# p-mc-grath/DMMFODS

Measured on AMD Instinct MI355X. Metric: training images/sec at 1280x1920 RGB+LiDAR, higher is better.
Workload: dtype f16; 1 GPU; C2 d121 early-fusion 6ch b4 1280x1920; key=c2, per_gpu_batch=4, global_batch=4, height=1280, width=1920, storage_dtype=fp16, accumulate=fp32, parallelism=dp1, weights=random-init (reference init, seed 123)

## Files before the change

dmmfods_amd/_lib.py:

```python
import ctypes as C
import os

_HERE = os.path.dirname(os.path.abspath(__file__))
LIB_PATH = os.environ.get("DMM_LIB_PATH") or os.path.join(_HERE, "libdmmfods_hip.so")

DMM_F32, DMM_F16, DMM_BF16 = 0, 1, 2
LOSS_BCE, LOSS_FOCAL = 0, 1
T_CONV, T_CONVT, T_BN_WEIGHT, T_BN_BIAS, T_BN_MEAN, T_BN_VAR, T_BN_TRACKED = range(7)
ERR_INVALID, ERR_SHAPE, ERR_HIP, ERR_STATE, ERR_NO_DEVICE = -1, -2, -3, -4, -5


class ModelDesc(C.Structure):
    _fields_ = [
        ("growth_rate", C.c_int32), ("num_blocks", C.c_int32), ("block_config", C.c_int32 * 8),
        ("num_init_features", C.c_int32), ("bn_size", C.c_int32), ("num_classes", C.c_int32),
        ("concat_before_block_num", C.c_int32), ("stream_1_in_channels", C.c_int32),
        ("stream_2_in_channels", C.c_int32), ("batch", C.c_int32), ("height", C.c_int32), ("width", C.c_int32),
        ("dtype", C.c_int32), ("loss_scale", C.c_float), ("bn_momentum", C.c_float), ("bn_eps", C.c_float),
        ("iou_threshold", C.c_float), ("use_mfma", C.c_int32),
    ]


class ConvDesc(C.Structure):
    _fields_ = [(n, C.c_int32) for n in (
        "dtype", "use_mfma", "B", "H", "W", "Cin", "Cout", "R", "S", "stride", "pad", "transposed", "mode", "bn_relu")]


class GuardState(C.Structure):
    _fields_ = [("scale", C.c_float), ("grad_scale", C.c_float), ("sumsq", C.c_double), ("grad_norm", C.c_float),
                ("found_inf", C.c_int32), ("applied_steps", C.c_int64), ("skipped_steps", C.c_int64),
                ("growth_tracker", C.c_int32), ("step_size", C.c_float), ("bc2_sqrt", C.c_float), ("clip_coef", C.c_float),
                ("reserved", C.c_int32 * 2)]


assert C.sizeof(GuardState) == 64

ADAM_MAX_CLASSES = 16


class AdamSegment(C.Structure):
    _fields_ = [("begin", C.c_int64), ("count", C.c_int64), ("cls", C.c_int32)]


class AdamClass(C.Structure):
    _fields_ = [("lr", C.c_float), ("beta1", C.c_float), ("beta2", C.c_float), ("eps", C.c_float), ("weight_decay", C.c_float),
                ("decoupled", C.c_int32), ("t0", C.c_int64)]


assert C.sizeof(AdamSegment) == 24 and C.sizeof(AdamClass) == 32


class DmmError(RuntimeError):
    pass


_lib = None


def lib():
    global _lib
    if _lib is not None:
        return _lib
    if not os.path.exists(LIB_PATH):
        raise ImportError(
            f"{LIB_PATH} is missing: build it with `python -c 'import __graft_entry__ as g; g.build()'` "
            "(or `make -C dmmfods_amd/csrc`).  dmmfods_amd has no CPU fallback.")
    import torch
    tl = os.path.join(os.path.dirname(torch.__file__), "lib", "libamdhip64.so")
    if os.path.exists(tl):
        C.CDLL(tl, mode=C.RTLD_GLOBAL)
    L = C.CDLL(LIB_PATH)
    vp, i32, i64, f32, sz = C.c_void_p, C.c_int32, C.c_int64, C.c_float, C.c_size_t
    L.dmm_last_error.restype = C.c_char_p
    L.dmm_version.restype = C.c_int
    L.dmm_last_impl.restype = C.c_int
    L.dmm_impl_name.restype = C.c_char_p
    L.dmm_impl_name.argtypes = [C.c_int]
    L.dmm_impl_mask.restype = C.c_uint
    L.dmm_impl_mask.argtypes = [C.c_int]
    L.dmm_set_option.restype = C.c_int
    L.dmm_set_option.argtypes = [C.c_char_p, C.c_int]
    L.dmm_plan_create.argtypes = [C.POINTER(ModelDesc), C.POINTER(vp)]
    L.dmm_plan_destroy.argtypes = [vp]
    L.dmm_plan_destroy.restype = C.c_int
    L.dmm_plan_num_tensors.argtypes = [vp]
    L.dmm_plan_tensor_info.argtypes = [vp, C.c_int, C.POINTER(C.c_char_p), C.POINTER(i32), C.POINTER(i32),
                                       C.POINTER(i64 * 4), C.POINTER(i64)]
    L.dmm_plan_num_params.argtypes = [vp]
    L.dmm_plan_num_params.restype = i64
    L.dmm_plan_num_buffer_elems.argtypes = [vp]
    L.dmm_plan_num_buffer_elems.restype = i64
    L.dmm_plan_workspace_bytes.argtypes = [vp]
    L.dmm_plan_workspace_bytes.restype = sz
    L.dmm_plan_forward_flops.argtypes = [vp]
    L.dmm_plan_forward_flops.restype = C.c_double
    L.dmm_plan_bind.argtypes = [vp, vp, sz, vp, vp, vp]
    L.dmm_plan_forward.argtypes = [vp, vp, vp, vp, C.c_int, vp]
    L.dmm_plan_loss_backward.argtypes = [vp, vp, vp, vp, vp]
    L.dmm_plan_backward.argtypes = [vp, vp, vp]
    L.dmm_plan_loss_metrics.argtypes = [vp, vp, vp, vp, vp]
    L.dmm_plan_set_loss.argtypes = [vp, C.c_int, vp, vp, C.c_int]
    L.dmm_loss_forward.argtypes = [C.c_int, C.c_int, vp, vp, vp, vp, vp, vp, C.c_int, C.c_int, C.c_int, C.c_int, vp]
    L.dmm_plan_num_grad_buckets.argtypes = [vp]
    L.dmm_plan_num_graph_replays.argtypes = [vp, C.c_int]
    L.dmm_plan_num_graph_replays.restype = C.c_longlong
    L.dmm_plan_grad_bucket.argtypes = [vp, C.c_int, C.POINTER(i64), C.POINTER(i64)]
    L.dmm_plan_grad_bucket_wait.argtypes = [vp, C.c_int, vp]
    L.dmm_plan_profile_begin.argtypes = [vp, C.c_int]
    L.dmm_plan_profile_filter.restype = C.c_int
    L.dmm_plan_profile_filter.argtypes = [vp, C.c_char_p]
    L.dmm_plan_profile_num_ops.argtypes = [vp, C.c_int]
    L.dmm_plan_profile_op.argtypes = [vp, C.c_int, C.c_int, C.POINTER(C.c_char_p), C.POINTER(C.c_double), C.POINTER(C.c_double)]
    L.dmm_plan_profile_collect.argtypes = [vp, C.c_int, C.POINTER(C.c_double), C.c_int, C.POINTER(C.c_int)]
    L.dmm_adam_step.argtypes = [vp, vp, vp, vp, i64, f32, f32, f32, f32, f32, i64, f32, vp]
    L.dmm_grad_guard_scratch_bytes.argtypes = [i64]
    L.dmm_grad_guard_scratch_bytes.restype = sz
    L.dmm_guard_state_init.argtypes = [vp, f32, i64, i32, vp]
    L.dmm_adam_step_guarded.argtypes = [vp, vp, vp, vp, i64, f32, f32, f32, f32, f32, f32, f32, f32, i32, vp, vp, vp]
    L.dmm_adam_step_guarded_ranges.argtypes = [vp, vp, vp, vp, C.POINTER(i64), C.POINTER(i64), C.POINTER(i64), C.c_int,
                                               f32, f32, f32, f32, f32, f32, f32, f32, i32, vp, vp, vp]
    L.dmm_plan_set_encoder_frozen.argtypes = [vp, C.c_int]
    L.dmm_adam_table_bytes.argtypes = [C.c_int, i64]
    L.dmm_adam_table_bytes.restype = sz
    L.dmm_adam_table_init.argtypes = [vp, C.POINTER(AdamSegment), C.c_int, i64, C.c_int, vp]
    L.dmm_adam_step_segmented.argtypes = [vp, vp, vp, vp, i64, vp, C.c_int, C.POINTER(AdamClass), C.c_int, i64, f32, vp]
    L.dmm_adam_step_guarded_segmented.argtypes = [vp, vp, vp, vp, i64, vp, C.c_int, C.POINTER(AdamClass), C.c_int, f32, f32, f32, i32,
                                                  vp, vp, vp]
    L.dmm_grad_sumsq.argtypes = [vp, i64, i64, C.c_int, vp, vp]
    L.dmm_plan_set_dynamic_loss_scale.argtypes = [vp, vp]
    L.dmm_plan_set_grad_accumulate.argtypes = [vp, C.c_int]
    L.dmm_conv_scratch_bytes.argtypes = [C.POINTER(ConvDesc)]
    L.dmm_conv_scratch_bytes.restype = sz
    L.dmm_conv_forward.argtypes = [C.POINTER(ConvDesc), vp, vp, vp, vp, vp, vp, vp, vp]
    L.dmm_conv_wgrad.argtypes = [C.POINTER(ConvDesc), vp, vp, vp, vp, vp, vp, vp]
    L.dmm_conv_dgrad.argtypes = [C.POINTER(ConvDesc), vp, vp, vp, vp, vp, vp, vp, vp, vp]
    L.dmm_conv_wgrad_ex.argtypes = [C.POINTER(ConvDesc), vp, vp, vp, vp, vp, vp, vp, C.c_int, vp, vp, vp]
    L.dmm_conv_dgrad_ex.argtypes = [C.POINTER(ConvDesc), vp, vp, vp, vp, vp, vp, vp, vp, vp, C.c_int, vp, vp, vp]
    L.dmm_conv1x1_backward_fused.argtypes = [C.POINTER(ConvDesc), vp, vp, vp, vp, vp, vp, vp, vp, vp, C.c_int, vp, vp, vp, vp]
    L.dmm_conv5_wgrad_stats.argtypes = [C.POINTER(ConvDesc), vp, vp, vp, vp, vp, vp, vp, vp, vp]
    _lib = L
    return L


EXPORTS = [
    "dmm_last_error", "dmm_version", "dmm_set_option", "dmm_plan_create", "dmm_plan_destroy", "dmm_plan_num_tensors",
    "dmm_plan_tensor_info", "dmm_plan_num_params", "dmm_plan_num_buffer_elems", "dmm_plan_workspace_bytes",
    "dmm_plan_forward_flops", "dmm_plan_bind", "dmm_plan_forward", "dmm_plan_loss_backward", "dmm_plan_backward",
    "dmm_plan_loss_metrics", "dmm_plan_num_graph_replays", "dmm_plan_set_loss", "dmm_loss_forward", "dmm_plan_num_grad_buckets", "dmm_plan_grad_bucket",
    "dmm_plan_grad_bucket_wait", "dmm_plan_profile_begin", "dmm_plan_profile_filter", "dmm_plan_profile_num_ops", "dmm_plan_profile_op",
    "dmm_plan_profile_collect", "dmm_adam_step", "dmm_conv_scratch_bytes", "dmm_conv_forward", "dmm_conv_wgrad",
    "dmm_conv_dgrad", "dmm_conv_wgrad_ex", "dmm_conv_dgrad_ex", "dmm_conv1x1_backward_fused", "dmm_conv5_wgrad_stats", "dmm_last_impl", "dmm_impl_name", "dmm_impl_mask",
    "dmm_grad_guard_scratch_bytes", "dmm_guard_state_init", "dmm_adam_step_guarded", "dmm_grad_sumsq", "dmm_plan_set_dynamic_loss_scale",
    "dmm_plan_set_grad_accumulate", "dmm_plan_set_encoder_frozen", "dmm_adam_step_guarded_ranges",
    "dmm_adam_table_bytes", "dmm_adam_table_init", "dmm_adam_step_segmented", "dmm_adam_step_guarded_segmented",
]


def check(rc):
    if rc == 0:
        return
    msg = lib().dmm_last_error().decode(errors="replace")
    if rc == ERR_SHAPE:
        raise ValueError(msg)
    if rc == ERR_INVALID and "fusion" in msg:
        raise AttributeError(msg)
    if rc == ERR_INVALID:
        raise ValueError(msg)
    raise DmmError(f"dmm status {rc}: {msg}")


def last_impl():
    L = lib()
    return L.dmm_impl_name(L.dmm_last_impl()).decode()


def impls_since_reset(reset=True):
    L = lib()
    m = L.dmm_impl_mask(1 if reset else 0)
    return {L.dmm_impl_name(i).decode() for i in range(32) if (m >> i) & 1}


def stream_ptr():
    import torch
    return C.c_void_p(torch.cuda.current_stream().cuda_stream)
```

dmmfods_amd/csrc/bw1.hip:

```cpp
#include <algorithm>
#include <cstdio>
#include <cstdlib>
#include <type_traits>

#include "common.h"
#include "dispatch.h"
#include "gather.h"
#include "isa.h"
#include "pointwise.h"

namespace dmm {

#ifndef B1_DBG
#define B1_DBG 0
#endif
#ifndef B1_LATE_PREFETCH
#define B1_LATE_PREFETCH 0
#endif
#ifndef B1_RAW_BAR
#define B1_RAW_BAR 0
#endif
#ifndef B1_NT
#define B1_NT 0
#endif
#ifndef B1_GOLD_EARLY
#define B1_GOLD_EARLY 0
#endif
constexpr int B1_TM = 64;
constexpr int B1_NB = 128;
constexpr int B1_CT = 128;
constexpr int B1_IMG = B1_TM * 256;
constexpr int B1_W = 4 * B1_CT * 64;
constexpr int B1_STAGE = B1_TM * B1_CT * 4;
static_assert(B1_STAGE == 2 * B1_IMG, "staging aliases the operand images exactly");
constexpr int B1_LDS = 2 * B1_IMG + B1_W + 2 * B1_CT * 8 + 6 * B1_CT * 4;

__device__ __forceinline__ int b1_swz(int row, int slot) { return ((((slot >> 2) ^ (row & 3)) << 2) | ((slot & 3) ^ ((row >> 2) & 3))); }

template <typename T, int PQ, bool ACC_, bool PART>
__global__ __launch_bounds__(NTHREADS, 2) void bw1_kernel(const Bw1Args g) {
  constexpr bool ACC = ACC_ && !(B1_DBG & 32);
  constexpr bool UNC = std::is_same<T, f16>::value;
  static_assert(sizeof(T) == 2, "16-bit storage");
  typedef typename TT<T>::vec V;
  constexpr int SLOT = 8;
  constexpr int NL = B1_TM * 16 / NTHREADS;
  const ConvArgs& a = g.c;
  const Seg& sg = a.seg[0];

  extern __shared__ __attribute__((aligned(16))) unsigned char smem[];
  unsigned char* Ai = smem;
  unsigned char* Gi = smem + B1_IMG;
  unsigned char* Wi = smem + 2 * B1_IMG;
  double* red = (double*)(smem + 2 * B1_IMG + B1_W);
  float* kc = (float*)(smem + 2 * B1_IMG + B1_W + 2 * B1_CT * 8);

  const int tid = threadIdx.x, lane = tid & 63, wave = tid >> 6;
  const int r = lane & 31, h = lane >> 5;
  const int xcd = blockIdx.x & 7, q = blockIdx.x >> 3;
  const int ct = g.xcd_group ? q % g.nct : (int)(blockIdx.x % g.nct);
  const int split = g.xcd_group ? (q / g.nct) * 8 + xcd : (int)(blockIdx.x / g.nct);
  const int c0 = ct * B1_CT;
  const int t_beg = split * g.tiles_per_wg, t_end = min(g.ntiles, t_beg + g.tiles_per_wg);
  if (t_beg >= t_end) return;

  const int cs = tid & 15, p0 = tid >> 4;
  const int cx = c0 + cs * SLOT;
  const bool cvalid = cx < a.N;
  if (tid < B1_CT) {
    const int c = c0 + tid;
    const bool v = c < a.N;
    kc[tid] = v ? a.bscale[c] : 0.f; kc[B1_CT + tid] = v ? a.bshift[c] : 0.f;
    kc[2 * B1_CT + tid] = v ? a.bmean[c] : 0.f; kc[3 * B1_CT + tid] = v ? a.binvstd[c] : 0.f;
    kc[4 * B1_CT + tid] = PQ == 2 ? sg.q[tid] : 0.f; kc[5 * B1_CT + tid] = PQ == 2 ? sg.r[tid] : 0.f;
  }
  const unsigned char* xbase = (const unsigned char*)a.bx;
  const unsigned char* gbase = (const unsigned char*)sg.src;
  const unsigned char* ybase = (const unsigned char*)sg.src2;
  unsigned char* obase = (unsigned char*)a.out;
  const unsigned xcol = (unsigned)(cvalid ? cx : 0) * 2u, gcol = (unsigned)(cs * SLOT) * 2u;
  const unsigned xpitch = (unsigned)a.ldbx * 2u, gpitch = (unsigned)sg.ld * 2u, ypitch = (unsigned)sg.ld2 * 2u, opitch = (unsigned)a.ldo * 2u;
  const int lds0 = p0 * 256 + (b1_swz(p0, cs) << 4);

  {
    const T* wp = (const T*)a.wpack;
#pragma unroll
    for (int j = 0; j < B1_W / 16 / NTHREADS; ++j) {
      const int piece = tid + NTHREADS * j;
      const int chunk = piece >> 9, rowc = (piece >> 2) & 127, slot = piece & 3;
      const int c = c0 + rowc;
      V v;
#pragma unroll
      for (int e = 0; e < SLOT; ++e) v[e] = (T)0;
      if (c < a.Npad) v = *(const V*)(wp + ((size_t)chunk * a.Npad + c) * 32 + slot * SLOT);
      *(V*)(Wi + chunk * (B1_CT * 64) + rowc * 64 + ((slot ^ ((rowc >> 2) & 3)) << 4)) = v;
    }
  }
  if (tid < 2 * B1_CT) red[tid] = 0.0;
  __syncthreads();

  V rx[NL], rg[NL], ry[PQ == 2 ? NL : 1];
  unsigned okp = 0;
  auto issue = [&](int tile) {
    okp = 0;
#pragma unroll
    for (int i = 0; i < NL; ++i) {
      const int m = tile * B1_TM + p0 + 16 * i;
      if (m < a.M) okp |= 1u << i;
      const unsigned mm = (B1_DBG & 16) ? 0u : (unsigned)min(m, a.M - 1);
      if (B1_NT & 1) rx[i] = __builtin_nontemporal_load((const V*)(xbase + (size_t)(mm * xpitch + xcol)));
      else rx[i] = *(const V*)(xbase + (size_t)(mm * xpitch + xcol));
      rg[i] = *(const V*)(gbase + (size_t)(mm * gpitch + gcol));
      if constexpr (PQ == 2) ry[i] = *(const V*)(ybase + (size_t)(mm * ypitch + gcol));
    }
  };

  const int dpx = 32 * (wave & 1) + r;
  const int dgoff = dpx * 256;
  const int dcb = 64 * (wave >> 1);
  const int bsw = (r >> 2) & 3;
  const int tg = lane >> 4, ti = lane & 15, tq = ti >> 2, tp = ti & 3;
  const int arow = 8 * (tg >> 1) + tq;
  auto tr_off = [&](int px, int colbyte) { return px * 256 + ((b1_swz(px, colbyte >> 4) << 4) | (colbyte & 15)); };
  const int acolb = (32 * wave + 16 * (tg & 1) + 4 * tp) * 2;
  const int aoff1 = tr_off(arow, acolb);
  int goff1[4];
#pragma unroll
  for (int j = 0; j < 4; ++j) goff1[j] = tr_off(arow, (32 * j + 16 * (tg & 1) + 4 * tp) * 2);
  auto second = [](int off) { return (off ^ 16) + 4 * 256; };

  f32x16 accw[4];
#pragma unroll
  for (int j = 0; j < 4; ++j)
#pragma unroll
    for (int i = 0; i < 16; ++i) accw[j][i] = 0.f;

  issue(t_beg);
  for (int tile = t_beg; tile < t_end; ++tile) {
    V xraw[NL], gold[ACC ? NL : 1];
    const bool full = (tile + 1) * B1_TM <= a.M;
    const unsigned okt = okp;
    auto stage = [&](auto full_tag) {
      constexpr bool FULL = decltype(full_tag)::value;
      V z;
#pragma unroll
      for (int e = 0; e < SLOT; ++e) z[e] = (T)0;
      {
        SlotK<SLOT> kx;
        kx.k0 = load_fv<SLOT>(kc + cs * SLOT); kx.k1 = load_fv<SLOT>(kc + B1_CT + cs * SLOT); kx.k2 = 0.f; kx.k3 = 0.f;
#pragma unroll
        for (int i = 0; i < NL; ++i) {
          xraw[i] = rx[i];
          const bool v = FULL || ((okt >> i) & 1) != 0;
          const V av_ = bn_relu_slot(rx[i], kx);
          *(V*)(Ai + lds0 + 4096 * i) = v ? av_ : z;
        }
      }
      {
        SlotK<SLOT> kg;
        kg.k0 = 0.f; kg.k1 = 0.f; kg.k2 = 0.f; kg.k3 = 0.f;
        if (PQ == 2) { kg.k0 = load_fv<SLOT>(kc + 4 * B1_CT + cs * SLOT); kg.k1 = load_fv<SLOT>(kc + 5 * B1_CT + cs * SLOT); }
#pragma unroll
        for (int i = 0; i < NL; ++i) {
          const bool v = FULL || ((okt >> i) & 1) != 0;
          V gv = rg[i];
          if constexpr (PQ == 2) gv = eff_grad_slot(rg[i], ry[i], kg);
          *(V*)(Gi + lds0 + 4096 * i) = v ? gv : z;
        }
      }
    };
    if (UNC && full) stage(std::true_type()); else stage(std::false_type());
    __syncthreads();
#if !B1_LATE_PREFETCH
    if (tile + 1 < t_end) issue(tile + 1);
#endif
#if B1_GOLD_EARLY
    if constexpr (ACC) {
#pragma unroll
      for (int i = 0; i < NL; ++i) {
        const unsigned mm = (unsigned)min(tile * B1_TM + p0 + 16 * i, a.M - 1);
        gold[i] = *(const V*)(obase + (size_t)(mm * opitch + xcol));
      }
    }
#endif

    f32x16 accd[2];
#pragma unroll
    for (int t = 0; t < 2; ++t)
#pragma unroll
      for (int i = 0; i < 16; ++i) accd[t][i] = 0.f;
    if (!(B1_DBG & 4))
#pragma unroll
    for (int ch = 0; ch < 4; ++ch)
#pragma unroll
      for (int s = 0; s < 2; ++s) {
        const int slot = ch * 4 + 2 * s + h;
        const V av = *(const V*)(Gi + dgoff + (b1_swz(dpx, slot) << 4));
#pragma unroll
        for (int t = 0; t < 2; ++t) {
          const V bv = *(const V*)(Wi + ch * (B1_CT * 64) + (dcb + 32 * t + r) * 64 + (((2 * s + h) ^ bsw) << 4));
          accd[t] = mma16(av, bv, accd[t]);
        }
      }
    if (!(B1_DBG & 2))
#pragma unroll
    for (int ms = 0; ms < B1_TM / 16; ++ms) {
      const V af = frag16<T>(lds_tr16(Ai + aoff1 + ms * 4096), lds_tr16(Ai + second(aoff1) + ms * 4096));
#pragma unroll
      for (int j = 0; j < 4; ++j) {
        const V gf = frag16<T>(lds_tr16(Gi + goff1[j] + ms * 4096), lds_tr16(Gi + second(goff1[j]) + ms * 4096));
        accw[j] = mma16(gf, af, accw[j]);
      }
    }
#if !B1_GOLD_EARLY
    if constexpr (ACC) {
#pragma unroll
      for (int i = 0; i < NL; ++i) {
        const unsigned mm = (unsigned)min(tile * B1_TM + p0 + 16 * i, a.M - 1);
        if (B1_NT & 1) gold[i] = __builtin_nontemporal_load((const V*)(obase + (size_t)(mm * opitch + xcol)));
        else gold[i] = *(const V*)(obase + (size_t)(mm * opitch + xcol));
      }
    }
#endif
#if B1_LATE_PREFETCH
    if (tile + 1 < t_end) issue(tile + 1);
#endif
#if B1_RAW_BAR
    lds_barrier();
#else
    __syncthreads();
#endif
    if (B1_DBG & 8) {
      float sa = 0.f;
#pragma unroll
      for (int t = 0; t < 2; ++t)
#pragma unroll
        for (int i = 0; i < 16; ++i) sa += accd[t][i];
      if (sa == 1.2345e33f) obase[0] = 1;
    } else {
    float* Cs = (float*)smem;
#pragma unroll
    for (int t = 0; t < 2; ++t)
#pragma unroll
      for (int i = 0; i < 16; ++i) {
        const int row = 32 * (wave & 1) + (i & 3) + 8 * (i >> 2) + 4 * h;
        Cs[row * B1_CT + ((dcb + 32 * t + r) ^ (h << 5))] = accd[t][i];
      }
#if B1_RAW_BAR
    lds_barrier();
#else
    __syncthreads();
#endif
    float s1[SLOT], s2[SLOT];
#pragma unroll
    for (int e = 0; e < SLOT; ++e) { s1[e] = 0.f; s2[e] = 0.f; }
    auto finish = [&](auto full_tag) {
      constexpr bool FULL = decltype(full_tag)::value;
      float sc[SLOT], sh[SLOT], mu[UNC ? 1 : SLOT], is[UNC ? 1 : SLOT];
      load_f32s<SLOT>(kc + cs * SLOT, sc); load_f32s<SLOT>(kc + B1_CT + cs * SLOT, sh);
      if constexpr (!UNC) { load_f32s<SLOT>(kc + 2 * B1_CT + cs * SLOT, mu); load_f32s<SLOT>(kc + 3 * B1_CT + cs * SLOT, is); }
#pragma unroll
      for (int i = 0; i < NL; ++i) {
        if (!FULL && !((okt >> i) & 1)) continue;
        const int p = p0 + 16 * i;
        float av[SLOT];
#pragma unroll
        for (int e = 0; e < SLOT; e += 4) {
          const f32x4 t4 = *(const f32x4*)(Cs + p * B1_CT + ((cs * SLOT + e) ^ (((p >> 2) & 1) << 5)));
          av[e] = t4[0]; av[e + 1] = t4[1]; av[e + 2] = t4[2]; av[e + 3] = t4[3];
        }
        const unsigned m = (unsigned)(tile * B1_TM + p);
        if constexpr (UNC) {
          const V ov = bnbwd_slot<ACC>(av, xraw[i], gold[ACC ? i : 0], sc, sh, s1, s2);
          if (B1_NT & 2) __builtin_nontemporal_store(ov, (V*)(obase + (size_t)(m * opitch + xcol)));
          else if (!(B1_DBG & 64) || av[0] == 1.2345e33f) *(V*)(obase + (size_t)(m * opitch + xcol)) = ov;
        } else {
          float xf[SLOT], gf[SLOT];
          vec_to_f32<T>(xraw[i], xf);
          if constexpr (ACC) vec_to_f32<T>(gold[i], gf);
#pragma unroll
          for (int e = 0; e < SLOT; ++e) {
            const float dz = (fmaf(xf[e], sc[e], sh[e]) > 0.f) ? av[e] : 0.f;
            s1[e] += dz;
            s2[e] = fmaf(dz, (xf[e] - mu[e]) * is[e], s2[e]);
            gf[e] = (ACC ? gf[e] : 0.f) + sc[e] * dz;
          }
          if (!(B1_DBG & 64) || gf[0] == 1.2345e33f) *(V*)(obase + (size_t)(m * opitch + xcol)) = f32_to_vec<T>(gf);
        }
      }
    };
    if (cvalid) { if (UNC && full) finish(std::true_type()); else finish(std::false_type()); }
    fold_to_lds<16, SLOT, B1_CT>(s1, s2, red, cs, cvalid, lane);
    }
#if B1_RAW_BAR
    lds_barrier();
#else
    __syncthreads();
#endif
  }

  if (tid < B1_CT && c0 + tid < a.N) {
    const size_t rep = (size_t)(blockIdx.x & (STAT_REPS - 1)) * a.stat_stride;
    const double S1 = red[fold_slot<16, SLOT>(0, tid)];
    double S2 = red[fold_slot<16, SLOT>(1, tid)];
    if constexpr (UNC) S2 = (S2 - (double)kc[2 * B1_CT + tid] * S1) * (double)kc[3 * B1_CT + tid];
    atomic_add_f64(a.red1 + rep + c0 + tid, S1);
    atomic_add_f64(a.red2 + rep + c0 + tid, S2);
  }
  const int c = c0 + 32 * wave + r;
  if constexpr (PART) {
    float* slot = g.part + ((size_t)split * g.nct + ct) * B1_SLOT_FLOATS + (size_t)wave * (B1_NB * 32);
#pragma unroll
    for (int j = 0; j < 4; ++j)
#pragma unroll
      for (int i = 0; i < 16; ++i) {
        const int n = 32 * j + (i & 3) + 8 * (i >> 2) + 4 * h;
        slot[n * 32 + r] = accw[j][i];
      }
  } else if (!(B1_DBG & 1) && c < g.wC) {
    const size_t chunk = (size_t)(c0 / 32 + wave);
#pragma unroll
    for (int j = 0; j < 4; ++j)
#pragma unroll
      for (int i = 0; i < 16; ++i) {
        const int n = 32 * j + (i & 3) + 8 * (i >> 2) + 4 * h;
        atomic_add_f32(g.dpack + (chunk * g.dNpad + n) * 32 + r, accw[j][i]);
      }
  }
  if (B1_DBG & 1) {
    float s = 0.f;
#pragma unroll
    for (int j = 0; j < 4; ++j)
#pragma unroll
      for (int i = 0; i < 16; ++i) s += accw[j][i];
    if (s == 1.2345e33f) g.dpack[0] = s;
  }
}

template <typename T, int PQ, bool ACC, bool PART>
static hipError_t launch_bw1_t(const Bw1Args& g, int nwg, hipStream_t st) {
  return launch_lds<bw1_kernel<T, PQ, ACC, PART>>(B1_LDS, nwg, NTHREADS, B1_LDS, st, g);
}

bool bw1_eligible(const WgradArgs& w, const ConvArgs& d, int dtype, unsigned deny) {
  if (((deny >> IMPL_BW1) & 1u) || dtype == DT_F32 || w.nseg != 1 || d.nseg != 1 || d.pool2) return false;
  const Seg& wx = w.seg[0];
  const Seg& wg = w.dy;
  const Seg& dg = d.seg[0];
  if (wx.mode != G_PLAIN || wx.istride != 1 || wx.ntaps != 1 || wx.taps[0] != 0 || wx.scale == nullptr || wx.C % 32) return false;
  if (wg.mode != G_PLAIN || wg.istride != 1 || wg.ntaps != 1 || wg.taps[0] != 0 || wg.scale != nullptr || wg.C != B1_NB) return false;
  if (dg.mode != G_PLAIN || dg.istride != 1 || dg.ntaps != 1 || dg.taps[0] != 0 || dg.scale != nullptr || dg.C != B1_NB || dg.Cpad != B1_NB) return false;
  if (dg.src != wg.src || dg.ld != wg.ld || dg.q != wg.q || dg.src2 != wg.src2) return false;
  if (w.N != B1_NB || w.Npad != B1_NB || w.M != d.M || d.N != wx.C || d.Npad % 32) return false;
  if (d.bx != wx.src || d.ldbx != wx.ld || d.bscale != wx.scale || d.bshift != wx.shift) return false;
  if (d.out == nullptr || d.ostride != 1 || d.Hout != d.Ho || d.Wout != d.Wo || wx.Hs != d.Ho || wx.Ws != d.Wo) return false;
  const double span = 2.0 * (double)d.M;
  if (span * d.ldbx >= 4294967296.0 || span * d.ldo >= 4294967296.0 || span * dg.ld >= 4294967296.0 || span * dg.ld2 >= 4294967296.0) return false;
  return true;
}

Bw1Geom bw1_geometry(const ConvArgs& a) {
  Bw1Geom q;
  q.nct = (a.N + B1_CT - 1) / B1_CT;
  q.ntiles = (a.M + B1_TM - 1) / B1_TM;
  constexpr int cus = DESIGN_CUS;
  static const int per_cu = lab_int("DMM_BW1_PER_CU", 2);
  int nsplit = std::max(1, (per_cu * cus + q.nct - 1) / q.nct);
  nsplit = std::min(nsplit, std::max(1, q.ntiles / 4));
  q.tiles_per_wg = (q.ntiles + nsplit - 1) / nsplit;
  q.nsplit = (q.ntiles + q.tiles_per_wg - 1) / q.tiles_per_wg;
  q.xcd_group = (q.nct > 1 && q.nsplit >= 32 && q.tiles_per_wg >= 8) ? 1 : 0;
  q.nwg = q.xcd_group ? ((q.nsplit + 7) / 8) * 8 * q.nct : q.nsplit * q.nct;
  return q;
}

static bool g_bw1_part = !lab_flag("DMM_NO_BW1_PART");

static bool bw1_uses_part(const Bw1Args& g, const Bw1Geom& q) {
  return g_bw1_part && g.part != nullptr && q.nsplit * q.nct <= g.part_slots && q.nsplit > 1;
}

hipError_t launch_bw1(const Bw1Args& g0, int dtype, hipStream_t st) {
  Bw1Args g = g0;
  const ConvArgs& a = g.c;
  if (a.M <= 0) return hipSuccess;
  const Bw1Geom q = bw1_geometry(a);
  note_impl(IMPL_BW1);
  g.nct = q.nct; g.ntiles = q.ntiles; g.tiles_per_wg = q.tiles_per_wg; g.xcd_group = q.xcd_group; g.nsplit = q.nsplit;
  const int nwg = q.nwg;
  const int pq = a.seg[0].q ? 2 : 0;
  const bool acc = a.accumulate != 0;
  const bool part = bw1_uses_part(g, q);
#define B1_GO(T) \
  (part ? (pq ? (acc ? launch_bw1_t<T, 2, true, true>(g, nwg, st) : launch_bw1_t<T, 2, false, true>(g, nwg, st))     \
              : (acc ? launch_bw1_t<T, 0, true, true>(g, nwg, st) : launch_bw1_t<T, 0, false, true>(g, nwg, st)))    \
        : (pq ? (acc ? launch_bw1_t<T, 2, true, false>(g, nwg, st) : launch_bw1_t<T, 2, false, false>(g, nwg, st))   \
              : (acc ? launch_bw1_t<T, 0, true, false>(g, nwg, st) : launch_bw1_t<T, 0, false, false>(g, nwg, st))))
  if (dtype == DT_F16) return B1_GO(f16);
  return B1_GO(bf16);
#undef B1_GO
}

__global__ __launch_bounds__(256) void bw1_reduce_kernel(const float* __restrict__ part, float* __restrict__ dpack, int nct, int nsplit, int nfloats) {
  const int e = (blockIdx.x * 256 + threadIdx.x) * 4;
  if (e >= nct * B1_SLOT_FLOATS) return;
  f32x4 s = {0.f, 0.f, 0.f, 0.f};
  const float* p = part + e;
  const size_t pitch = (size_t)nct * B1_SLOT_FLOATS;
  int k = 0;
  for (; k + 16 <= nsplit; k += 16) {
    f32x4 v[16];
#pragma unroll
    for (int u = 0; u < 16; ++u) v[u] = __builtin_nontemporal_load((const f32x4*)(p + (size_t)(k + u) * pitch));
#pragma unroll
    for (int u = 0; u < 16; u += 4) s += (v[u] + v[u + 1]) + (v[u + 2] + v[u + 3]);
  }
  for (; k + 4 <= nsplit; k += 4) {
    const f32x4 v0 = *(const f32x4*)(p + (size_t)k * pitch), v1 = *(const f32x4*)(p + (size_t)(k + 1) * pitch);
    const f32x4 v2 = *(const f32x4*)(p + (size_t)(k + 2) * pitch), v3 = *(const f32x4*)(p + (size_t)(k + 3) * pitch);
    s += (v0 + v1) + (v2 + v3);
  }
  for (; k < nsplit; ++k) s += *(const f32x4*)(p + (size_t)k * pitch);
  if (e < nfloats) *(f32x4*)(dpack + e) = s;
}

hipError_t launch_bw1_reduce(const Bw1Args& g, hipStream_t st) {
  const ConvArgs& a = g.c;
  if (a.M <= 0) return hipSuccess;
  const Bw1Geom q = bw1_geometry(a);
  if (!bw1_uses_part(g, q)) return hipSuccess;
  const int nfloats = ((g.wC + 31) / 32) * g.dNpad * 32;
  const int nthreads = q.nct * B1_SLOT_FLOATS / 4;
  hipLaunchKernelGGL(bw1_reduce_kernel, dim3((nthreads + 255) / 256), dim3(256), 0, st, g.part, g.dpack, q.nct, q.nsplit, nfloats);
  return hipGetLastError();
}

}
```

dmmfods_amd/csrc/capi.cpp:

```cpp
#include <algorithm>
#include <atomic>
#include <cmath>
#include <cstdio>
#include <cstdlib>
#include <cstring>
#include <stdexcept>
#include <chrono>
#include <mutex>
#include <string>
#include <utility>
#include <vector>
#include <unistd.h>

#include "dispatch.h"
#include "plan.h"

using namespace dmm;

void plan_build_tables(dmm_plan* p);
void plan_bind(dmm_plan* p, void* ws);
void plan_size(dmm_plan* p);

static thread_local std::string g_err;
static int fail(int code, const std::string& msg) {
  g_err = msg;
  return code;
}
#define HIPCHK(expr)                                                                                   \
  do {                                                                                                 \
    hipError_t e__ = (expr);                                                                           \
    if (e__ != hipSuccess) return fail(DMM_ERR_HIP, std::string(#expr) + ": " + hipGetErrorString(e__)); \
  } while (0)

static bool g_overlap_wgrad = getenv("DMM_NO_OVERLAP") == nullptr;
static int g_graph = getenv("DMM_GRAPH") ? std::max(1, atoi(getenv("DMM_GRAPH"))) : 0;
static unsigned long long g_option_epoch = 1;
static int g_bucket_mb = getenv("DMM_GRAD_BUCKET_MB") ? atoi(getenv("DMM_GRAD_BUCKET_MB")) : 25;
static std::atomic<unsigned> g_family_off{lab_family_off()};
static unsigned plan_deny(const dmm_plan* p) { return (p->sw.no_hf ? 1u << IMPL_HF : 0u) | g_family_off; }

namespace {
struct DevicePool {
  std::mutex mu;
  hipStream_t side = nullptr, pack = nullptr, capture = nullptr;
  std::vector<hipEvent_t> free_plain, free_timing;
  long events_made = 0;
};
constexpr int MAX_DEVICES = 64;
DevicePool* g_pools[MAX_DEVICES] = {};
std::mutex g_pools_mu;

DevicePool* pool_of(int device) {
  if (device < 0 || device >= MAX_DEVICES) return nullptr;
  std::lock_guard<std::mutex> l(g_pools_mu);
  if (g_pools[device] == nullptr) g_pools[device] = new DevicePool();
  return g_pools[device];
}
hipError_t pool_streams(DevicePool* dp, bool want_capture) {
  std::lock_guard<std::mutex> l(dp->mu);
  if (dp->side == nullptr) {
    int lo = 0, hi = 0;
    hipError_t e = hipDeviceGetStreamPriorityRange(&lo, &hi);
    if (e != hipSuccess) return e;
    hipStream_t s = nullptr, k = nullptr;
    if ((e = hipStreamCreateWithPriority(&s, hipStreamNonBlocking, lo)) != hipSuccess) return e;
    if ((e = hipStreamCreateWithPriority(&k, hipStreamNonBlocking, lo)) != hipSuccess) return e;
    dp->side = s; dp->pack = k;
  }
  if (want_capture && dp->capture == nullptr) {
    hipStream_t c = nullptr;
    const hipError_t e = hipStreamCreateWithFlags(&c, hipStreamNonBlocking);
    if (e != hipSuccess) return e;
    dp->capture = c;
  }
  return hipSuccess;
}
hipEvent_t pool_event(DevicePool* dp, bool timing) {
  std::lock_guard<std::mutex> l(dp->mu);
  auto& fl = timing ? dp->free_timing : dp->free_plain;
  if (!fl.empty()) { hipEvent_t e = fl.back(); fl.pop_back(); return e; }
  hipEvent_t e = nullptr;
  const hipError_t rc = timing ? hipEventCreate(&e) : hipEventCreateWithFlags(&e, hipEventDisableTiming);
  if (rc != hipSuccess) return nullptr;
  ++dp->events_made;
  return e;
}
void pool_return(DevicePool* dp, std::vector<void*>& evs, bool timing) {
  std::lock_guard<std::mutex> l(dp->mu);
  auto& fl = timing ? dp->free_timing : dp->free_plain;
  for (void* e : evs) if (e) fl.push_back((hipEvent_t)e);
  evs.clear();
}
void trace_destroy(const char* what) {
  static const bool on = getenv("DMM_TRACE_DESTROY") != nullptr;
  if (!on) return;
  char buf[160];
  const int n = snprintf(buf, sizeof(buf), "[dmm] destroy: %s\n", what);
  if (n > 0) { ssize_t w = write(2, buf, (size_t)std::min<int>(n, (int)sizeof(buf) - 1)); (void)w; }
}
}

extern "C" {

const char* dmm_last_error(void) { return g_err.c_str(); }
int dmm_version(void) { return 101; }

static const char* const kImplNames[IMPL_COUNT] = {"auto", "generic", "thin", "conv3", "cvp", "halo", "wg3", "wg5", "wgp", "pig", "bw1", "hf", "cf", "wgpw", "cvw"};
static const struct { const char* option; int family; } kFamilyOptions[] = {
    {"thin_logits", IMPL_THIN}, {"conv3", IMPL_CONV3}, {"wg3", IMPL_WG3}, {"wgp", IMPL_WGP},
    {"wg5", IMPL_WG5},          {"cvp", IMPL_CVP},     {"bw1", IMPL_BW1}, {"pig", IMPL_PIG},
};

int dmm_set_option(const char* name, int value) {
  if (!name) return fail(DMM_ERR_INVALID, "null argument");
  ++g_option_epoch;
  if (std::string(name) == "overlap_wgrad") { g_overlap_wgrad = value != 0; return DMM_OK; }
  if (std::string(name) == "graph") { g_graph = value; return DMM_OK; }
  for (const auto& o : kFamilyOptions)
    if (std::string(name) == o.option) {
      if (value != 0) g_family_off &= ~(1u << o.family);
      else g_family_off |= 1u << o.family;
      return DMM_OK;
    }
  if (std::string(name) == "grad_bucket_mb") {
    if (value < 0) return fail(DMM_ERR_INVALID, "grad_bucket_mb must be >= 0");
    g_bucket_mb = value;
    return DMM_OK;
  }
  return fail(DMM_ERR_INVALID, std::string("unknown option ") + name);
}

int dmm_plan_create(const dmm_model_desc* desc, dmm_plan** out) {
  if (!desc || !out) return fail(DMM_ERR_INVALID, "null argument");
  if (desc->num_blocks < 2 || desc->num_blocks > 8) return fail(DMM_ERR_INVALID, "num_blocks must be in [2, 8]");
  if (desc->dtype != DMM_F32 && desc->dtype != DMM_F16 && desc->dtype != DMM_BF16)
    return fail(DMM_ERR_INVALID, "dtype must be DMM_F32, DMM_F16 or DMM_BF16");
  if (desc->dtype == DMM_BF16 && !desc->use_mfma) return fail(DMM_ERR_INVALID, "DMM_BF16 has no scalar check kernels: use_mfma must be 1");
  if (desc->batch < 1) return fail(DMM_ERR_INVALID, "batch must be >= 1");
  if (!(desc->loss_scale > 0)) return fail(DMM_ERR_INVALID, "loss_scale must be > 0");
  dmm_plan* p = new dmm_plan();
  p->desc = *desc;
  p->sw = PlanSwitches::from_environment();
  p->bucket_bytes = (size_t)g_bucket_mb << 20;
  p->deny = plan_deny(p);
  try {
    plan_build_tables(p);
  } catch (const std::domain_error& e) {
    delete p;
    return fail(DMM_ERR_SHAPE, e.what());
  } catch (const std::exception& e) {
    delete p;
    return fail(DMM_ERR_INVALID, e.what());
  }
  *out = p;
  return DMM_OK;
}

int dmm_plan_destroy(dmm_plan* plan) {
  if (!plan) return DMM_OK;
  trace_destroy("begin");
  std::string first_err;
  auto note = [&](hipError_t e, const char* what) {
    if (e != hipSuccess && first_err.empty()) first_err = std::string(what) + ": " + hipGetErrorString(e);
  };
  DevicePool* dp = plan->device >= 0 ? pool_of(plan->device) : nullptr;
  if (dp != nullptr) {
    int cur = -1;
    const bool switched = hipGetDevice(&cur) == hipSuccess && cur != plan->device && hipSetDevice(plan->device) == hipSuccess;
    if (plan->used_side) {
      trace_destroy("synchronise the side stream");
      note(hipStreamSynchronize(dp->side), "hipStreamSynchronize(side stream)");
      trace_destroy("synchronise the pack stream");
      note(hipStreamSynchronize(dp->pack), "hipStreamSynchronize(pack stream)");
    }
    if (plan->used_capture && dp->capture) {
      trace_destroy("synchronise the capture stream");
      note(hipStreamSynchronize(dp->capture), "hipStreamSynchronize(capture stream)");
    }
    trace_destroy("graphs");
    for (auto& gc : plan->graphs) {
      for (auto& e : gc.entries) note(hipGraphExecDestroy((hipGraphExec_t)e.exec), "hipGraphExecDestroy");
      gc.entries.clear();
    }
    trace_destroy("events back to the pool");
    pool_return(dp, plan->fork_events, false);
    pool_return(dp, plan->join_events, false);
    pool_return(dp, plan->bucket_events, false);
    for (auto& which : plan->prof_events)
      for (auto& pass : which) pool_return(dp, pass, true);
    if (switched) (void)hipSetDevice(cur);
  }
  trace_destroy("delete");
  delete plan;
  trace_destroy("done");
  return first_err.empty() ? DMM_OK : fail(DMM_ERR_HIP, "dmm_plan_destroy: " + first_err);
}

int dmm_plan_num_tensors(const dmm_plan* plan) { return plan ? (int)plan->tensors.size() : 0; }

int dmm_plan_tensor_info(const dmm_plan* plan, int index, const char** name, int32_t* kind, int32_t* ndim, int64_t shape[4],
                         int64_t* arena_offset) {
  if (!plan || index < 0 || index >= (int)plan->tensors.size()) return fail(DMM_ERR_INVALID, "tensor index out of range");
  const TensorInfo& t = plan->tensors[index];
  if (name) *name = t.name.c_str();
  if (kind) *kind = t.kind;
  if (ndim) *ndim = t.ndim;
  if (shape) for (int i = 0; i < 4; ++i) shape[i] = t.shape[i];
  if (arena_offset) *arena_offset = t.off;
  return DMM_OK;
}

int64_t dmm_plan_num_params(const dmm_plan* plan) { return plan ? plan->nparams : 0; }
int64_t dmm_plan_num_buffer_elems(const dmm_plan* plan) { return plan ? plan->nbuf : 0; }
size_t dmm_plan_workspace_bytes(const dmm_plan* plan) { return plan ? plan->zero_bytes + plan->zero_bwd_bytes + plan->main_bytes : 0; }
double dmm_plan_forward_flops(const dmm_plan* plan) { return plan ? plan->fwd_flops : 0; }

int dmm_plan_bind(dmm_plan* plan, void* workspace, size_t workspace_bytes, float* params, float* grads, float* buffers) {
  if (!plan || !workspace || !params || !grads || !buffers) return fail(DMM_ERR_INVALID, "null argument");
  if (workspace_bytes < dmm_plan_workspace_bytes(plan)) return fail(DMM_ERR_INVALID, "workspace too small");
  if ((uintptr_t)workspace % 256) return fail(DMM_ERR_INVALID, "workspace must be 256-byte aligned");
  int ndev = 0;
  if (hipGetDeviceCount(&ndev) != hipSuccess || ndev == 0) return fail(DMM_ERR_NO_DEVICE, "no HIP device");
  int dev = 0;
  HIPCHK(hipGetDevice(&dev));
  if (plan->device >= 0 && plan->device != dev) return fail(DMM_ERR_STATE, "the plan is bound to another device");
  if (dev >= MAX_DEVICES) return fail(DMM_ERR_INVALID, "device index out of range");
  plan->device = dev;
  plan->params = params;
  plan->grads = grads;
  plan->buffers = buffers;
  plan->graphs[0].epoch = plan->graphs[1].epoch = 0;
  plan->bound = false;
  plan->deny = plan_deny(plan);
  try {
    plan_bind(plan, workspace);
  } catch (const dmm::plan_sizing_error& e) {
    return fail(DMM_ERR_STATE, e.what());
  } catch (const std::exception& e) {
    return fail(DMM_ERR_INVALID, e.what());
  }
  HIPCHK(hipDeviceSynchronize());
  plan->bound = true;
  return DMM_OK;
}

static std::string family_check(const Op& o, unsigned ran) {
  if ((o.kind == OP_IGEMM ? o.c.M : o.w.M) <= 0) return std::string();
  const bool recorded_ran = (ran >> o.impl) & 1u;
  const bool generic_ran = (ran >> IMPL_GENERIC) & 1u;
  const bool wgp_remainder = o.kind == OP_WGRAD && o.impl == IMPL_WGP && o.w.nseg == 2 && o.w.nphase == 0;
  if (recorded_ran && (o.impl == IMPL_GENERIC || !generic_ran || wgp_remainder)) return std::string();
  std::string names;
  for (int f = 1; f < IMPL_COUNT; ++f)
    if ((ran >> f) & 1u) names += (names.empty() ? "" : "+") + std::string(dmm_impl_name(f));
  return std::string("launch '") + o.label + "': the plan recorded family " + dmm_impl_name(o.impl) + ", " + (names.empty() ? "none" : names) + " ran";
}

static int run_ops(dmm_plan* p, std::vector<Op>& ops, hipStream_t st, int prof_which = -1, size_t begin = 0, size_t end = 0, bool capturing = false) {
  if (end == 0 || end > ops.size()) end = ops.size();
  const size_t ev_offset = 0;
  const int dt = p->desc.dtype;
  const bool mfma = p->desc.use_mfma != 0;
  std::vector<void*>* evs = nullptr;
  if (prof_which >= 0 && p->prof_max_passes > 0 && p->prof_pass[prof_which] < p->prof_max_passes) {
    auto& sets = p->prof_events[prof_which];
    const int pass = p->prof_pass[prof_which]++;
    if ((int)sets.size() <= pass) sets.resize(pass + 1);
    evs = &sets[pass];
    const size_t need = 2 * (ops.size() + ev_offset);
    DevicePool* pdp = pool_of(p->device);
    while (evs->size() < need) {
      hipEvent_t e = pdp ? pool_event(pdp, true) : nullptr;
      if (e == nullptr) return fail(DMM_ERR_HIP, "hipEventCreate failed");
      evs->push_back((void*)e);
    }
  }
  const bool accumulate = p->grad_accumulate;
  const std::string& filt = p->prof_filter;
  auto selected = [&](const Op& o) { return evs != nullptr && (filt.empty() || strncmp(o.label, filt.c_str(), filt.size()) == 0); };
  const bool overlap = g_overlap_wgrad && !capturing && (evs == nullptr || !filt.empty());
  constexpr int nside = 1;
  size_t nfork = 0;
  bool forked = false;
  DevicePool* dp = pool_of(p->device);
  hipStream_t side_st = nullptr, pack_st = nullptr;
  if (overlap) {
    if (dp == nullptr || pool_streams(dp, false) != hipSuccess) return fail(DMM_ERR_HIP, "side stream");
    side_st = dp->side; pack_st = dp->pack;
    while ((int)p->join_events.size() < nside + 1) {
      hipEvent_t je = pool_event(dp, false);
      if (je == nullptr) return fail(DMM_ERR_HIP, "hipEventCreate failed");
      p->join_events.push_back((void*)je);
    }
    p->used_side = true;
  }
  bool pack_pending = false;
  auto join_pack = [&]() {
    if (pack_pending) {
      hipStreamWaitEvent(st, (hipEvent_t)p->join_events[nside], 0);
      pack_pending = false;
    }
  };
  auto join_side = [&]() {
    if (forked) {
      for (int k = 0; k < nside; ++k) {
        hipEventRecord((hipEvent_t)p->join_events[k], side_st);
        hipStreamWaitEvent(st, (hipEvent_t)p->join_events[k], 0);
      }
      forked = false;
    }
  };
  auto join = [&]() { join_side(); join_pack(); };
  static const bool host_prof = lab_flag("DMM_HOST_PROF");
  static double hp_launch[32] = {0}, hp_fork[32] = {0};
  static long hp_n[32] = {0}, hp_lists = 0;
  auto now = [] { return std::chrono::duration<double, std::micro>(std::chrono::steady_clock::now().time_since_epoch()).count(); };
  for (size_t i = begin; i < end; ++i) {
    Op& o = ops[i];
    hipError_t e = hipSuccess;
    const double hp_t0 = host_prof ? now() : 0.0;
    double hp_t1 = hp_t0;
    hipStream_t lst = st;
    if (overlap && o.leaf == 3 && forked) {
      lst = side_st;
    } else if (overlap && !o.chain && (o.kind == OP_WGRAD || o.leaf)) {
      if (nfork >= p->fork_events.size()) {
        hipEvent_t fe = pool_event(dp, false);
        if (fe == nullptr) { join(); return fail(DMM_ERR_HIP, "hipEventCreate failed"); }
        p->fork_events.push_back((void*)fe);
      }
      lst = o.leaf == 2 ? pack_st : side_st;
      hipEvent_t fe = (hipEvent_t)p->fork_events[nfork++];
      hipEventRecord(fe, st);
      hipStreamWaitEvent(lst, fe, 0);
      if (o.leaf == 2) pack_pending = true; else forked = true;
      if (host_prof) hp_t1 = now();
    }
    const bool sel = selected(o);
    if (sel) hipEventRecord((hipEvent_t)(*evs)[2 * (ev_offset + i)], lst);
    const bool fam_check = (o.kind == OP_IGEMM || o.kind == OP_WGRAD) && o.impl != IMPL_AUTO;
    const unsigned mask_before = g_impl_mask;
    if (fam_check) g_impl_mask = 0;
    switch (o.kind) {
      case OP_MEMSET: if (!(accumulate && o.ms.p == (void*)p->grads)) e = hipMemsetAsync(o.ms.p, 0, o.ms.bytes, lst); break;
      case OP_COPY: e = hipMemcpyAsync(o.cp.dst, o.cp.src, o.cp.bytes, hipMemcpyDeviceToDevice, lst); break;
      case OP_CONVERT: e = launch_convert_input(o.cv, dt, lst); break;
      case OP_IGEMM: e = launch_igemm(o.c, dt, o.epi, mfma, lst, o.impl); break;
      case OP_WGRAD: e = launch_wgrad(o.w, dt, mfma, lst, o.impl); break;
      case OP_BW1: e = launch_bw1(o.b1, dt, lst); break;
      case OP_BW1RED: e = launch_bw1_reduce(o.b1, lst); break;
      case OP_RAWFIN: e = launch_wg5_rawfin(o.rf, lst); break;
      case OP_FIN64: e = launch_wg5_fin64(o.f64, lst); break;
      case OP_JOIN: if (o.epi == 1) join_pack(); else join_side(); break;
      case OP_BNFIN: e = launch_bn_finalize(o.bf, lst); break;
      case OP_BNBWD:
        if (accumulate) { BnBwdFinalizeArgs bb = o.bb; bb.accumulate = 1; e = launch_bn_bwd_finalize(bb, lst); }
        else e = launch_bn_bwd_finalize(o.bb, lst);
        break;
      case OP_POOL: e = launch_maxpool_fwd(o.mp, dt, lst); break;
      case OP_POOLBWD: e = launch_maxpool_bwd(o.mpb, dt, lst); break;
      case OP_BCE: e = launch_bce_metrics(o.bce, dt, lst); break;
      case OP_PACK: e = launch_pack(o.pk.descs, o.pk.prefix, o.pk.ndesc, o.pk.total_rows, dt, lst, o.pk.tdescs, o.pk.tiles, o.pk.nt1, o.pk.nt9); break;
      case OP_APPLYCORR: e = launch_apply_corr(o.ac, dt, lst); break;
      case OP_UNPACK: e = launch_unpack(o.pk.descs, o.pk.prefix, o.pk.ndesc, o.pk.total_rows, dt, o.pk.grad_scale, lst, o.pk.tdescs, o.pk.tiles, o.pk.nt1, o.pk.nt9, accumulate); break;
      default: join(); return fail(DMM_ERR_STATE, "unknown op");
    }
    if (host_prof && o.kind < 32) { const double t2 = now(); hp_fork[o.kind] += hp_t1 - hp_t0; hp_launch[o.kind] += t2 - hp_t1; hp_n[o.kind]++; }
    if (e != hipSuccess) join();
    if (e != hipSuccess && fam_check) g_impl_mask |= mask_before;
    if (e != hipSuccess) return fail(DMM_ERR_HIP, "op " + std::to_string(i) + " kind " + std::to_string(o.kind) + ": " + hipGetErrorString(e));
    if (fam_check) {
      const unsigned ran = g_impl_mask;
      g_impl_mask = mask_before | ran;
      const std::string why = family_check(o, ran);
      if (!why.empty()) { join(); return fail(DMM_ERR_STATE, why); }
    }
    if (sel) hipEventRecord((hipEvent_t)(*evs)[2 * (ev_offset + i) + 1], lst);
    if (pack_pending && o.leaf == 2) hipEventRecord((hipEvent_t)p->join_events[nside], lst);
    if (o.signal >= 0 && !capturing) {
      while ((int)p->bucket_events.size() <= o.signal) {
        hipEvent_t be = dp ? pool_event(dp, false) : nullptr;
        if (be == nullptr) { join(); return fail(DMM_ERR_HIP, "hipEventCreate failed"); }
        p->bucket_events.push_back((void*)be);
      }
      hipEventRecord((hipEvent_t)p->bucket_events[o.signal], lst);
    }
  }
  join();
  if (host_prof && ++hp_lists == 40) {
    double tot = 0;
    for (int k = 0; k < 32; ++k) tot += hp_launch[k] + hp_fork[k];
    fprintf(stderr, "[host] 40 lists: %.2f ms of enqueue calls per list pair\n", tot / 20 / 1e3);
    for (int k = 0; k < 32; ++k)
      if (hp_n[k]) fprintf(stderr, "[host] op kind %2d: %6ld calls per pair, launch %.2f us each, fork events %.2f us each\n", k, hp_n[k] / 20,
                           hp_launch[k] / hp_n[k], hp_fork[k] / hp_n[k]);
  }
  return DMM_OK;
}

static int record_bucket_events(dmm_plan* p, const std::vector<Op>& ops, hipStream_t st) {
  for (const Op& o : ops) {
    if (o.signal < 0) continue;
    while ((int)p->bucket_events.size() <= o.signal) {
      DevicePool* dp = pool_of(p->device);
      hipEvent_t be = dp ? pool_event(dp, false) : nullptr;
      if (be == nullptr) return fail(DMM_ERR_HIP, "hipEventCreate failed");
      p->bucket_events.push_back((void*)be);
    }
    HIPCHK(hipEventRecord((hipEvent_t)p->bucket_events[o.signal], st));
  }
  return DMM_OK;
}

static int launch_list(dmm_plan* p, int which, std::vector<Op>& ops, size_t seg_begin, size_t seg_end, hipStream_t st) {
  dmm_plan::GraphCache& gc = p->graphs[which];
  const bool profiling = p->prof_max_passes > 0 && p->prof_pass[which] < p->prof_max_passes;
  if (gc.epoch != g_option_epoch) {
    for (auto& e : gc.entries) hipGraphExecDestroy((hipGraphExec_t)e.exec);
    gc.entries.clear();
    gc.nseen = 0;
    gc.epoch = g_option_epoch;
  }
  const bool want = g_graph && !(g_graph == 2 && which == 1) && !p->graph_failed && !profiling && !(which == 1 && p->dp_used) && seg_end > seg_begin + 8;
  if (!want) return run_ops(p, ops, st, which);
  if (gc.entries.empty() && gc.nseen > 0) {
    DevicePool* dp = pool_of(p->device);
    if (dp == nullptr || pool_streams(dp, true) != hipSuccess) return fail(DMM_ERR_HIP, "capture stream");
    hipStream_t cs = dp->capture;
    p->used_capture = true;
    hipGraph_t graph = nullptr;
    hipGraphExec_t exec = nullptr;
    bool ok = hipStreamBeginCapture(cs, hipStreamCaptureModeThreadLocal) == hipSuccess;
    if (ok) {
      const int rc = run_ops(p, ops, cs, -1, seg_begin, seg_end, true);
      const bool ended = hipStreamEndCapture(cs, &graph) == hipSuccess && graph != nullptr;
      ok = rc == DMM_OK && ended;
      if (ok) ok = hipGraphInstantiate(&exec, graph, nullptr, nullptr, 0) == hipSuccess;
      if (graph) hipGraphDestroy(graph);
    }
    gc.captures++;
    static const bool gtrace = lab_flag("DMM_GRAPH_TRACE");
    if (gtrace) fprintf(stderr, "[dmm] graph capture of list %d, launches [%zu, %zu): %s\n", which, seg_begin, seg_end, ok ? "ok" : "FAILED");
    if (!ok) {
      (void)hipGetLastError();
      p->graph_failed = true;
    } else {
      dmm_plan::GraphEntry e;
      for (int i = 0; i < 4; ++i) e.key[i] = nullptr;
      e.exec = (void*)exec; e.stamp = 0;
      gc.entries.push_back(e);
    }
  }
  gc.nseen = 1;
  if (gc.entries.empty()) return run_ops(p, ops, st, which);
  int rc = seg_begin > 0 ? run_ops(p, ops, st, -1, 0, seg_begin) : DMM_OK;
  if (rc) return rc;
  HIPCHK(hipGraphLaunch((hipGraphExec_t)gc.entries[0].exec, st));
  p->graph_replays[which]++;
  if (seg_end < ops.size()) { rc = run_ops(p, ops, st, -1, seg_end, ops.size()); if (rc) return rc; }
  return which == 1 ? record_bucket_events(p, ops, st) : DMM_OK;
}

int dmm_plan_forward(dmm_plan* plan, const float* stream_1, const float* stream_2, float* logits_out, int training, void* stream) {
  if (!plan || !plan->bound) return fail(DMM_ERR_STATE, "plan not bound");
  if (!stream_1 || !logits_out) return fail(DMM_ERR_INVALID, "null argument");
  if (plan->desc.stream_2_in_channels > 0 && !stream_2) return fail(DMM_ERR_INVALID, "stream_2 required");
  std::vector<Op>& ops = training ? plan->fwd_train : plan->fwd_eval;
  for (int idx : (training ? plan->convert_ops_train : plan->convert_ops_eval)) {
    Op& o = ops[idx];
    if (o.epi == 0) { o.cv.src1 = stream_1; o.cv.src2 = nullptr; }
    else if (o.epi == 1) { o.cv.src1 = stream_1; o.cv.src2 = stream_2; }
    else { o.cv.src1 = stream_2; o.cv.src2 = nullptr; }
  }
  ops[training ? plan->logits_op_train : plan->logits_op_eval].c.logits = logits_out;
  if (!training) return run_ops(plan, ops, (hipStream_t)stream, -1);
  size_t seg_begin = 0;
  for (size_t i = 0; i < ops.size(); ++i) if (ops[i].kind == OP_JOIN) seg_begin = i + 1;
  if (seg_begin == 0) for (int idx : plan->convert_ops_train) seg_begin = std::max(seg_begin, (size_t)idx + 1);
  return launch_list(plan, 0, ops, seg_begin, (size_t)plan->logits_op_train, (hipStream_t)stream);
}

static void set_loss_fields(const dmm_plan* plan, BceArgs& a) {
  a.kind = plan->loss_kind;
  for (int i = 0; i < 8; ++i) { a.alpha[i] = plan->loss_alpha[i]; a.gamma[i] = plan->loss_gamma[i]; }
}

int dmm_plan_set_loss(dmm_plan* plan, int kind, const float* alpha, const float* gamma, int nclass) {
  if (!plan) return fail(DMM_ERR_INVALID, "null plan");
  if (kind != DMM_LOSS_BCE && kind != DMM_LOSS_FOCAL) return fail(DMM_ERR_INVALID, "loss kind must be DMM_LOSS_BCE or DMM_LOSS_FOCAL");
  if (kind == DMM_LOSS_FOCAL) {
    if (!alpha || !gamma || nclass != plan->desc.num_classes) return fail(DMM_ERR_INVALID, "focal loss needs num_classes alpha / gamma values");
    for (int i = 0; i < nclass; ++i) { plan->loss_alpha[i] = alpha[i]; plan->loss_gamma[i] = gamma[i]; }
  }
  plan->loss_kind = kind;
  return DMM_OK;
}

int dmm_loss_forward(int kind, int from_prob, const float* alpha, const float* gamma, const float* input, const float* target,
                     float* loss_out, float* dinput_out, int batch, int nclass, int height, int width, void* stream) {
  if (!input || !target || (!loss_out && !dinput_out)) return fail(DMM_ERR_INVALID, "null argument");
  if (kind != DMM_LOSS_BCE && kind != DMM_LOSS_FOCAL) return fail(DMM_ERR_INVALID, "loss kind must be DMM_LOSS_BCE or DMM_LOSS_FOCAL");
  if (nclass < 1 || nclass > 8 || batch < 1 || height < 1 || width < 1) return fail(DMM_ERR_INVALID, "1..8 classes (dim 1) supported");
  if (kind == DMM_LOSS_FOCAL && (!alpha || !gamma)) return fail(DMM_ERR_INVALID, "focal loss needs alpha / gamma");
  BceArgs a;
  memset(&a, 0, sizeof(a));
  a.logits = input; a.target = target; a.loss_out = loss_out; a.dx_out = dinput_out;
  a.B = batch; a.NC = nclass; a.H = height; a.W = width;
  a.thr = 0.f; a.loss_scale = 1.f; a.kind = kind; a.from_prob = from_prob ? 1 : 0;
  for (int i = 0; i < nclass; ++i) { a.alpha[i] = alpha ? alpha[i] : 1.f; a.gamma[i] = gamma ? gamma[i] : 2.f; }
  HIPCHK(launch_bce_metrics(a, DT_F32, (hipStream_t)stream));
  return DMM_OK;
}

int dmm_plan_loss_backward(dmm_plan* plan, const float* logits, const float* target, double* metrics_out, void* stream) {
  if (!plan || !plan->bound) return fail(DMM_ERR_STATE, "plan not bound");
  if (!logits || !target) return fail(DMM_ERR_INVALID, "null argument");
  Op& b = plan->bwd[plan->bce_op];
  b.bce.logits = logits;
  b.bce.target = target;
  set_loss_fields(plan, b.bce);
  b.bce.dyn_scale = plan->dyn_scale;
  int rc = launch_list(plan, 1, plan->bwd, (size_t)plan->bce_op + 1, plan->bwd.size(), (hipStream_t)stream);
  if (rc) return rc;
  if (metrics_out) HIPCHK(hipMemcpyAsync(metrics_out, plan->metrics, plan->metrics_bytes, hipMemcpyDeviceToDevice, (hipStream_t)stream));
  return DMM_OK;
}

int dmm_plan_backward(dmm_plan* plan, const float* dlogits, void* stream) {
  if (!plan || !plan->bound) return fail(DMM_ERR_STATE, "plan not bound");
  if (!dlogits) return fail(DMM_ERR_INVALID, "null argument");
  hipStream_t st = (hipStream_t)stream;
  const BceArgs& b = plan->bwd[plan->bce_op].bce;
  ConvertArgs cv;
  memset(&cv, 0, sizeof(cv));
  cv.src1 = dlogits; cv.C1 = b.NC; cv.dst = b.dlogits; cv.B = b.B; cv.H = b.H; cv.W = b.W;
  cv.scale = plan->desc.loss_scale;
  cv.dyn_scale = plan->dyn_scale;
  int rc = run_ops(plan, plan->bwd, st, -1, 0, (size_t)plan->bce_op);
  if (rc) return rc;
  HIPCHK(launch_convert_input(cv, plan->desc.dtype, st));
  return run_ops(plan, plan->bwd, st, -1, (size_t)plan->bce_op + 1, 0);
}

long long dmm_plan_num_graph_replays(const dmm_plan* plan, int which) {
  return (plan && which >= 0 && which <= 1) ? plan->graph_replays[which] : 0;
}

int dmm_plan_num_grad_buckets(const dmm_plan* plan) { return plan ? (int)plan->buckets.size() : 0; }

int dmm_plan_grad_bucket(const dmm_plan* plan, int index, int64_t* offset, int64_t* count) {
  if (!plan || index < 0 || index >= (int)plan->buckets.size()) return fail(DMM_ERR_INVALID, "bucket index out of range");
  if (offset) *offset = plan->buckets[index].off;
  if (count) *count = plan->buckets[index].n;
  return DMM_OK;
}

int dmm_plan_grad_bucket_wait(dmm_plan* plan, int index, void* stream) {
  if (!plan || index < 0 || index >= (int)plan->buckets.size()) return fail(DMM_ERR_INVALID, "bucket index out of range");
  const GradBucket& b = plan->buckets[index];
  plan->dp_used = true;
  for (int ev : {b.ev_main, b.ev_side}) {
    if (ev < 0) continue;
    if (ev >= (int)plan->bucket_events.size()) return fail(DMM_ERR_STATE, "no backward pass has been enqueued on this plan yet");
    HIPCHK(hipStreamWaitEvent((hipStream_t)stream, (hipEvent_t)plan->bucket_events[ev], 0));
  }
  return DMM_OK;
}

int dmm_plan_profile_begin(dmm_plan* plan, int max_passes) {
  if (!plan) return fail(DMM_ERR_INVALID, "null plan");
  plan->prof_max_passes = max_passes;
  plan->prof_pass[0] = plan->prof_pass[1] = 0;
  return DMM_OK;
}

int dmm_plan_profile_filter(dmm_plan* plan, const char* label_prefix) {
  if (!plan) return fail(DMM_ERR_INVALID, "null plan");
  plan->prof_filter = label_prefix ? label_prefix : "";
  return DMM_OK;
}

int dmm_plan_profile_num_ops(const dmm_plan* plan, int which) {
  if (!plan || which < 0 || which > 1) return 0;
  return (int)(which == 0 ? plan->fwd_train.size() : plan->bwd.size());
}

int dmm_plan_profile_op(const dmm_plan* plan, int which, int index, const char** label, double* flops, double* bytes) {
  if (!plan || which < 0 || which > 1) return fail(DMM_ERR_INVALID, "bad argument");
  const std::vector<Op>& ops = which == 0 ? plan->fwd_train : plan->bwd;
  if (index < 0 || index >= (int)ops.size()) return fail(DMM_ERR_INVALID, "op index out of range");
  if (label) *label = ops[index].label;
  if (flops) *flops = ops[index].flops;
  if (bytes) *bytes = ops[index].bytes;
  return DMM_OK;
}

int dmm_plan_profile_collect(dmm_plan* plan, int which, double* ms_sum, int n, int* passes) {
  if (!plan || which < 0 || which > 1 || !ms_sum) return fail(DMM_ERR_INVALID, "bad argument");
  const int nops = dmm_plan_profile_num_ops(plan, which);
  if (n < nops) return fail(DMM_ERR_INVALID, "buffer too small");
  for (int i = 0; i < nops; ++i) ms_sum[i] = 0;
  int np = 0;
  for (auto& evs : plan->prof_events[which]) {
    if ((int)evs.size() < 2 * nops || np >= plan->prof_pass[which]) continue;
    const std::vector<Op>& ops = which == 0 ? plan->fwd_train : plan->bwd;
    const std::string& filt = plan->prof_filter;
    for (int i = 0; i < nops; ++i) {
      if (!filt.empty() && strncmp(ops[i].label, filt.c_str(), filt.size()) != 0) continue;
      float ms = 0;
      if (hipEventElapsedTime(&ms, (hipEvent_t)evs[2 * i], (hipEvent_t)evs[2 * i + 1]) != hipSuccess) return fail(DMM_ERR_HIP, "hipEventElapsedTime failed");
      ms_sum[i] += ms;
    }
    ++np;
  }
  if (passes) *passes = np;
  return DMM_OK;
}

int dmm_plan_loss_metrics(dmm_plan* plan, const float* logits, const float* target, double* metrics_out, void* stream) {
  if (!plan || !plan->bound) return fail(DMM_ERR_STATE, "plan not bound");
  if (!logits || !target || !metrics_out) return fail(DMM_ERR_INVALID, "null argument");
  hipStream_t st = (hipStream_t)stream;
  HIPCHK(hipMemsetAsync(plan->metrics, 0, plan->metrics_bytes, st));
  Op o = plan->bce_only;
  o.bce.logits = logits;
  o.bce.target = target;
  set_loss_fields(plan, o.bce);
  HIPCHK(launch_bce_metrics(o.bce, plan->desc.dtype, st));
  HIPCHK(hipMemcpyAsync(metrics_out, plan->metrics, plan->metrics_bytes, hipMemcpyDeviceToDevice, st));
  return DMM_OK;
}

int dmm_adam_step(float* params, const float* grads, float* exp_avg, float* exp_avg_sq, int64_t n, float lr, float beta1, float beta2,
                  float eps, float weight_decay, int64_t step, float grad_scale, void* stream) {
  if (!params || !grads || !exp_avg || !exp_avg_sq || n < 0 || step < 1) return fail(DMM_ERR_INVALID, "bad Adam argument");
  AdamArgs a;
  a.p = params; a.g = grads; a.m = exp_avg; a.v = exp_avg_sq; a.n = (size_t)n;
  a.beta1 = beta1; a.beta2 = beta2; a.eps = eps; a.weight_decay = weight_decay;
  const double bc1 = 1.0 - std::pow((double)beta1, (double)step), bc2 = 1.0 - std::pow((double)beta2, (double)step);
  a.step_size = (float)(lr / bc1);
  a.bc2_sqrt = (float)std::sqrt(bc2);
  a.grad_scale = grad_scale;
  HIPCHK(launch_adam(a, (hipStream_t)stream));
  return DMM_OK;
}

int dmm_plan_set_dynamic_loss_scale(dmm_plan* plan, const float* scale_dev) {
  if (!plan) return fail(DMM_ERR_INVALID, "null plan");
  if (((uintptr_t)scale_dev & 3) != 0) return fail(DMM_ERR_INVALID, "dynamic loss scale pointer must be 4-byte aligned");
  plan->dyn_scale = scale_dev;
  if (plan->bound && plan->bce_op >= 0) plan->bwd[plan->bce_op].bce.dyn_scale = scale_dev;
  return DMM_OK;
}

int dmm_plan_set_grad_accumulate(dmm_plan* plan, int accumulate) {
  if (!plan) return fail(DMM_ERR_INVALID, "null plan");
  const bool on = accumulate != 0;
  if (on == plan->grad_accumulate) return DMM_OK;
  plan->grad_accumulate = on;
  plan->graphs[1].epoch = 0;
  return DMM_OK;
}

int dmm_plan_set_encoder_frozen(dmm_plan* plan, int frozen) {
  if (!plan) return fail(DMM_ERR_INVALID, "null plan");
  if (plan->bound) return fail(DMM_ERR_STATE, "dmm_plan_set_encoder_frozen: the plan is bound (set the mode between dmm_plan_create and dmm_plan_bind)");
  const bool on = frozen != 0;
  if (on == plan->encoder_frozen) return DMM_OK;
  plan->encoder_frozen = on;
  plan->deny = plan_deny(plan);
  try {
    plan_size(plan);
  } catch (const std::exception& e) {
    plan->encoder_frozen = !on;
    try { plan_size(plan); } catch (...) {}
    return fail(DMM_ERR_INVALID, e.what());
  }
  return DMM_OK;
}

size_t dmm_grad_guard_scratch_bytes(int64_t n) {
  (void)n;
  return (size_t)GUARD_PARTIALS * sizeof(double);
}

int dmm_guard_state_init(dmm_guard_state* dev, float init_scale, int64_t applied_steps, int32_t growth_tracker, void* stream) {
  if (!dev) return fail(DMM_ERR_INVALID, "null guard state");
  if (((uintptr_t)dev & 7) != 0) return fail(DMM_ERR_INVALID, "guard state must be 8-byte aligned");
  if (!(init_scale > 0.f) || !std::isfinite(init_scale)) return fail(DMM_ERR_INVALID, "init_scale must be a finite number > 0");
  if (applied_steps < 0 || growth_tracker < 0) return fail(DMM_ERR_INVALID, "applied_steps and growth_tracker must be >= 0");
  HIPCHK(launch_guard_init(dev, init_scale, applied_steps, growth_tracker, (hipStream_t)stream));
  return DMM_OK;
}

int dmm_grad_sumsq(const float* grads, int64_t offset, int64_t count, int accumulate, void* scratch, void* stream) {
  if (!grads || !scratch) return fail(DMM_ERR_INVALID, "null argument");
  if (offset < 0 || count < 0) return fail(DMM_ERR_INVALID, "offset and count must be >= 0");
  if ((((uintptr_t)grads) & 3) != 0 || (((uintptr_t)scratch) & 7) != 0) return fail(DMM_ERR_INVALID, "misaligned gradient or scratch pointer");
  GradSumsqArgs r;
  r.g = grads + offset; r.n = (size_t)count; r.partials = (double*)scratch; r.accumulate = accumulate ? 1 : 0;
  HIPCHK(launch_grad_sumsq(r, (hipStream_t)stream));
  return DMM_OK;
}

int dmm_adam_step_guarded(float* params, const float* grads, float* exp_avg, float* exp_avg_sq, int64_t n, float lr, float beta1,
                          float beta2, float eps, float weight_decay, float max_norm, float growth_factor, float backoff_factor,
                          int32_t growth_interval, dmm_guard_state* state, void* scratch, void* stream) {
  if (!params || !grads || !exp_avg || !exp_avg_sq || !state || !scratch) return fail(DMM_ERR_INVALID, "null argument of the guarded Adam step");
  if (n < 0) return fail(DMM_ERR_INVALID, "n must be >= 0");
  if ((((uintptr_t)grads) & 3) != 0 || (((uintptr_t)state) & 7) != 0 || (((uintptr_t)scratch) & 7) != 0)
    return fail(DMM_ERR_INVALID, "misaligned gradient, state or scratch pointer");
  if (!(growth_factor >= 1.f) || !std::isfinite(growth_factor)) return fail(DMM_ERR_INVALID, "growth_factor must be a finite number >= 1");
  if (!(backoff_factor > 0.f) || !(backoff_factor <= 1.f)) return fail(DMM_ERR_INVALID, "backoff_factor must lie in (0, 1]");
  if (growth_interval < 0) return fail(DMM_ERR_INVALID, "growth_interval must be >= 0");
  if (std::isnan(max_norm)) return fail(DMM_ERR_INVALID, "max_norm is NaN");
  if (!(beta1 >= 0.f && beta1 < 1.f) || !(beta2 >= 0.f && beta2 < 1.f)) return fail(DMM_ERR_INVALID, "betas must lie in [0, 1)");
  hipStream_t st = (hipStream_t)stream;
  GradSumsqArgs r;
  r.g = grads; r.n = (size_t)n; r.partials = (double*)scratch; r.accumulate = 0;
  HIPCHK(launch_grad_sumsq(r, st));
  GuardFinalizeArgs f;
  f.partials = (const double*)scratch; f.state = state; f.lr = lr; f.beta1 = beta1; f.beta2 = beta2; f.max_norm = max_norm;
  f.growth_factor = growth_factor; f.backoff_factor = backoff_factor; f.growth_interval = growth_interval;
  HIPCHK(launch_guard_finalize(f, st));
  AdamArgs a;
  a.p = params; a.g = grads; a.m = exp_avg; a.v = exp_avg_sq; a.n = (size_t)n;
  a.beta1 = beta1; a.beta2 = beta2; a.eps = eps; a.weight_decay = weight_decay;
  a.step_size = 0.f; a.bc2_sqrt = 1.f; a.grad_scale = 0.f;
  HIPCHK(launch_adam_guarded(a, state, st));
  return DMM_OK;
}

int dmm_adam_step_guarded_ranges(float* params, const float* grads, float* exp_avg, float* exp_avg_sq, const int64_t* offsets,
                                 const int64_t* counts, const int64_t* t0, int nranges, float lr, float beta1, float beta2, float eps,
                                 float weight_decay, float max_norm, float growth_factor, float backoff_factor, int32_t growth_interval,
                                 dmm_guard_state* state, void* scratch, void* stream) {
  if (!params || !grads || !exp_avg || !exp_avg_sq || !offsets || !counts || !t0 || !state || !scratch)
    return fail(DMM_ERR_INVALID, "null argument of the guarded Adam step over ranges");
  if (nranges < 1) return fail(DMM_ERR_INVALID, "nranges must be >= 1");
  if ((((uintptr_t)grads) & 3) != 0 || (((uintptr_t)state) & 7) != 0 || (((uintptr_t)scratch) & 7) != 0)
    return fail(DMM_ERR_INVALID, "misaligned gradient, state or scratch pointer");
  for (int i = 0; i < nranges; ++i) {
    if (offsets[i] < 0 || counts[i] < 0) return fail(DMM_ERR_INVALID, "range " + std::to_string(i) + ": offset and count must be >= 0");
    if (t0[i] < 0) return fail(DMM_ERR_INVALID, "range " + std::to_string(i) + ": t0 must be >= 0");
    if (offsets[i] > INT64_MAX - counts[i]) return fail(DMM_ERR_INVALID, "range " + std::to_string(i) + ": offset + count overflows");
    for (int k = 0; k < i; ++k)
      if (offsets[i] < offsets[k] + counts[k] && offsets[k] < offsets[i] + counts[i])
        return fail(DMM_ERR_INVALID, "ranges " + std::to_string(k) + " and " + std::to_string(i) + " overlap");
  }
  if (!(growth_factor >= 1.f) || !std::isfinite(growth_factor)) return fail(DMM_ERR_INVALID, "growth_factor must be a finite number >= 1");
  if (!(backoff_factor > 0.f) || !(backoff_factor <= 1.f)) return fail(DMM_ERR_INVALID, "backoff_factor must lie in (0, 1]");
  if (growth_interval < 0) return fail(DMM_ERR_INVALID, "growth_interval must be >= 0");
  if (std::isnan(max_norm)) return fail(DMM_ERR_INVALID, "max_norm is NaN");
  if (!(beta1 >= 0.f && beta1 < 1.f) || !(beta2 >= 0.f && beta2 < 1.f)) return fail(DMM_ERR_INVALID, "betas must lie in [0, 1)");
  hipStream_t st = (hipStream_t)stream;
  for (int i = 0; i < nranges; ++i) {
    GradSumsqArgs r;
    r.g = grads + offsets[i]; r.n = (size_t)counts[i]; r.partials = (double*)scratch; r.accumulate = i > 0 ? 1 : 0;
    HIPCHK(launch_grad_sumsq(r, st));
  }
  GuardFinalizeArgs f;
  f.partials = (const double*)scratch; f.state = state; f.lr = lr; f.beta1 = beta1; f.beta2 = beta2; f.max_norm = max_norm;
  f.growth_factor = growth_factor; f.backoff_factor = backoff_factor; f.growth_interval = growth_interval;
  HIPCHK(launch_guard_finalize(f, st));
  for (int i = 0; i < nranges; ++i) {
    AdamArgs a;
    a.p = params + offsets[i]; a.g = grads + offsets[i]; a.m = exp_avg + offsets[i]; a.v = exp_avg_sq + offsets[i]; a.n = (size_t)counts[i];
    a.beta1 = beta1; a.beta2 = beta2; a.eps = eps; a.weight_decay = weight_decay;
    a.step_size = 0.f; a.bc2_sqrt = 1.f; a.grad_scale = 0.f;
    if (t0[i] == 0) HIPCHK(launch_adam_guarded(a, state, st));
    else HIPCHK(launch_adam_guarded_from(a, state, lr, t0[i], st));
  }
  return DMM_OK;
}

namespace {
hipError_t upload(void* dst, const void* src, size_t bytes, hipStream_t st);
struct AdamTableHost {
  int nsegs = 0, nclasses = 0;
  int64_t n = 0;
  std::vector<std::pair<int64_t, int64_t>> runs;
};
std::mutex g_adam_tables_mu;
std::vector<std::pair<const void*, AdamTableHost>> g_adam_tables;

size_t adam_table_chunks(int64_t n) { return (size_t)((n + ADAM_SEG_CHUNK - 1) / ADAM_SEG_CHUNK); }

bool bad_scalar(float x) { return std::isnan(x) || x < 0.f; }

int adam_seg_check(const char* who, const float* params, const float* grads, const float* exp_avg, const float* exp_avg_sq, int64_t n,
                   const void* table_dev, int nsegs, const dmm_adam_class* classes, int nclasses, AdamTableHost* host) {
  const std::string w(who);
  if (!params || !grads || !exp_avg || !exp_avg_sq || !table_dev || !classes) return fail(DMM_ERR_INVALID, w + ": null argument");
  if ((((uintptr_t)params | (uintptr_t)grads | (uintptr_t)exp_avg | (uintptr_t)exp_avg_sq) & 3) != 0 || ((uintptr_t)table_dev & 7) != 0)
    return fail(DMM_ERR_INVALID, w + ": misaligned arena (4 bytes) or table (8 bytes) pointer");
  if (n < 1) return fail(DMM_ERR_INVALID, w + ": n must be >= 1");
  if (nsegs < 1) return fail(DMM_ERR_INVALID, w + ": nsegs must be >= 1");
  if (nclasses < 1 || nclasses > ADAM_MAX_CLASSES)
    return fail(DMM_ERR_INVALID, w + ": nclasses must lie in [1, " + std::to_string(ADAM_MAX_CLASSES) + "]");
  for (int c = 0; c < nclasses; ++c) {
    const dmm_adam_class& k = classes[c];
    const std::string cw = w + ": class " + std::to_string(c) + ": ";
    if (!(k.beta1 >= 0.f && k.beta1 < 1.f) || !(k.beta2 >= 0.f && k.beta2 < 1.f)) return fail(DMM_ERR_INVALID, cw + "betas must lie in [0, 1)");
    if (bad_scalar(k.lr)) return fail(DMM_ERR_INVALID, cw + "lr must be >= 0 and not NaN");
    if (bad_scalar(k.eps)) return fail(DMM_ERR_INVALID, cw + "eps must be >= 0 and not NaN");
    if (bad_scalar(k.weight_decay)) return fail(DMM_ERR_INVALID, cw + "weight_decay must be >= 0 and not NaN");
    if (k.t0 < 0) return fail(DMM_ERR_INVALID, cw + "t0 must be >= 0");
  }
  std::lock_guard<std::mutex> l(g_adam_tables_mu);
  for (const auto& e : g_adam_tables)
    if (e.first == table_dev) {
      if (e.second.nsegs != nsegs || e.second.n != n)
        return fail(DMM_ERR_INVALID, w + ": table_dev was initialised for nsegs = " + std::to_string(e.second.nsegs) + ", n = " + std::to_string(e.second.n));
      if (e.second.nclasses != nclasses)
        return fail(DMM_ERR_INVALID, w + ": table_dev was initialised for nclasses = " + std::to_string(e.second.nclasses));
      *host = e.second;
      return DMM_OK;
    }
  return fail(DMM_ERR_INVALID, w + ": table_dev was not initialised by dmm_adam_table_init");
}

void adam_seg_args(AdamSegArgs& a, float* params, const float* grads, float* exp_avg, float* exp_avg_sq, int64_t n, const void* table_dev,
                   int nsegs, const dmm_adam_class* classes, int nclasses) {
  a.p = params; a.g = grads; a.m = exp_avg; a.v = exp_avg_sq; a.n = (size_t)n;
  a.segs = (const AdamSegDev*)table_dev;
  a.first = (const int*)((const uint8_t*)table_dev + (size_t)nsegs * sizeof(AdamSegDev));
  a.nsegs = nsegs; a.nchunks = (int)adam_table_chunks(n); a.nclasses = nclasses;
  a.vec_ok = (((uintptr_t)params | (uintptr_t)grads | (uintptr_t)exp_avg | (uintptr_t)exp_avg_sq) & 15) == 0 ? 1 : 0;
  a.grad_scale = 0.f; a.state = nullptr;
  for (int c = 0; c < ADAM_MAX_CLASSES; ++c) {
    AdamSegClass& k = a.cls[c];
    k = AdamSegClass{};
    k.bc2_sqrt = 1.f;
    if (c >= nclasses) continue;
    const dmm_adam_class& s = classes[c];
    k.lr = s.lr; k.beta1 = s.beta1; k.beta2 = s.beta2; k.eps = s.eps; k.t0 = s.t0;
    k.decoupled = s.decoupled != 0 ? 1 : 0;
    k.weight_decay = k.decoupled ? 0.f : s.weight_decay;
    k.decay = k.decoupled ? (float)(1.0 - (double)s.lr * (double)s.weight_decay) : 1.f;
  }
}
}

size_t dmm_adam_table_bytes(int nsegs, int64_t n) {
  if (nsegs < 1 || n < 1 || n > (int64_t)INT32_MAX * ADAM_SEG_CHUNK) return 0;
  return (size_t)nsegs * sizeof(AdamSegDev) + adam_table_chunks(n) * sizeof(int);
}

int dmm_adam_table_init(void* table_dev, const dmm_adam_segment* segs, int nsegs, int64_t n, int nclasses, void* stream) {
  if (!table_dev || !segs) return fail(DMM_ERR_INVALID, "dmm_adam_table_init: null argument");
  if (((uintptr_t)table_dev & 7) != 0) return fail(DMM_ERR_INVALID, "dmm_adam_table_init: misaligned table pointer (8 bytes)");
  if (nsegs < 1) return fail(DMM_ERR_INVALID, "dmm_adam_table_init: nsegs must be >= 1");
  if (n < 1 || n > (int64_t)INT32_MAX * ADAM_SEG_CHUNK) return fail(DMM_ERR_INVALID, "dmm_adam_table_init: n must be >= 1 (and below 2^41)");
  if (nclasses < 1 || nclasses > ADAM_MAX_CLASSES)
    return fail(DMM_ERR_INVALID, "dmm_adam_table_init: nclasses must lie in [1, " + std::to_string(ADAM_MAX_CLASSES) + "]");
  for (int i = 0; i < nsegs; ++i) {
    const dmm_adam_segment& s = segs[i];
    const std::string w = "dmm_adam_table_init: segment " + std::to_string(i);
    if (s.count < 1) return fail(DMM_ERR_INVALID, w + ": count must be >= 1");
    if (s.begin < 0 || s.begin >= n || s.count > n - s.begin) return fail(DMM_ERR_INVALID, w + " lies outside [0, n)");
    if (s.cls < 0 || s.cls >= nclasses) return fail(DMM_ERR_INVALID, w + ": cls outside [0, nclasses)");
    if (i > 0 && s.begin < segs[i - 1].begin + segs[i - 1].count)
      return fail(DMM_ERR_INVALID, w + " is unsorted or overlaps segment " + std::to_string(i - 1));
  }
  const size_t nchunks = adam_table_chunks(n), bytes = dmm_adam_table_bytes(nsegs, n);
  std::vector<uint8_t> buf(bytes);
  AdamSegDev* sd = (AdamSegDev*)buf.data();
  int* first = (int*)(buf.data() + (size_t)nsegs * sizeof(AdamSegDev));
  AdamTableHost host;
  host.nsegs = nsegs; host.nclasses = nclasses; host.n = n;
  for (int i = 0; i < nsegs; ++i) {
    sd[i].begin = segs[i].begin; sd[i].end = segs[i].begin + segs[i].count; sd[i].cls = segs[i].cls; sd[i].pad = 0;
    if (!host.runs.empty() && host.runs.back().first + host.runs.back().second == segs[i].begin) host.runs.back().second += segs[i].count;
    else host.runs.emplace_back(segs[i].begin, segs[i].count);
  }
  int s = 0;
  for (size_t ch = 0; ch < nchunks; ++ch) {
    while (s < nsegs && sd[s].end <= (long long)(ch * ADAM_SEG_CHUNK)) ++s;
    first[ch] = s;
  }
  HIPCHK(upload(table_dev, buf.data(), bytes, (hipStream_t)stream));
  std::lock_guard<std::mutex> l(g_adam_tables_mu);
  for (auto& e : g_adam_tables)
    if (e.first == table_dev) { e.second = std::move(host); return DMM_OK; }
  g_adam_tables.emplace_back(table_dev, std::move(host));
  return DMM_OK;
}

int dmm_adam_step_segmented(float* params, const float* grads, float* exp_avg, float* exp_avg_sq, int64_t n, const void* table_dev,
                            int nsegs, const dmm_adam_class* classes, int nclasses, int64_t step, float grad_scale, void* stream) {
  if (step < 1) return fail(DMM_ERR_INVALID, "dmm_adam_step_segmented: step must be >= 1");
  AdamTableHost host;
  if (int rc = adam_seg_check("dmm_adam_step_segmented", params, grads, exp_avg, exp_avg_sq, n, table_dev, nsegs, classes, nclasses, &host)) return rc;
  AdamSegArgs a;
  adam_seg_args(a, params, grads, exp_avg, exp_avg_sq, n, table_dev, nsegs, classes, nclasses);
  a.grad_scale = grad_scale;
  for (int c = 0; c < nclasses; ++c) {
    AdamSegClass& k = a.cls[c];
    const int64_t t = step - k.t0;
    k.active = t >= 1 ? 1 : 0;
    if (!k.active) continue;
    const double bc1 = 1.0 - std::pow((double)k.beta1, (double)t), bc2 = 1.0 - std::pow((double)k.beta2, (double)t);
    k.step_size = (float)(k.lr / bc1);
    k.bc2_sqrt = (float)std::sqrt(bc2);
  }
  HIPCHK(launch_adam_segmented(a, (hipStream_t)stream));
  return DMM_OK;
}

int dmm_adam_step_guarded_segmented(float* params, const float* grads, float* exp_avg, float* exp_avg_sq, int64_t n,
                                    const void* table_dev, int nsegs, const dmm_adam_class* classes, int nclasses, float max_norm,
                                    float growth_factor, float backoff_factor, int32_t growth_interval, dmm_guard_state* state,
                                    void* scratch, void* stream) {
  const char* who = "dmm_adam_step_guarded_segmented";
  if (!state || !scratch) return fail(DMM_ERR_INVALID, std::string(who) + ": null state or scratch");
  if ((((uintptr_t)state) & 7) != 0 || (((uintptr_t)scratch) & 7) != 0) return fail(DMM_ERR_INVALID, std::string(who) + ": misaligned state or scratch pointer");
  if (!(growth_factor >= 1.f) || !std::isfinite(growth_factor)) return fail(DMM_ERR_INVALID, "growth_factor must be a finite number >= 1");
  if (!(backoff_factor > 0.f) || !(backoff_factor <= 1.f)) return fail(DMM_ERR_INVALID, "backoff_factor must lie in (0, 1]");
  if (growth_interval < 0) return fail(DMM_ERR_INVALID, "growth_interval must be >= 0");
  if (std::isnan(max_norm)) return fail(DMM_ERR_INVALID, "max_norm is NaN");
  AdamTableHost host;
  if (int rc = adam_seg_check(who, params, grads, exp_avg, exp_avg_sq, n, table_dev, nsegs, classes, nclasses, &host)) return rc;
  hipStream_t st = (hipStream_t)stream;
  for (size_t i = 0; i < host.runs.size(); ++i) {
    GradSumsqArgs r;
    r.g = grads + host.runs[i].first; r.n = (size_t)host.runs[i].second; r.partials = (double*)scratch; r.accumulate = i > 0 ? 1 : 0;
    HIPCHK(launch_grad_sumsq(r, st));
  }
  GuardFinalizeArgs f;
  f.partials = (const double*)scratch; f.state = state; f.lr = classes[0].lr; f.beta1 = classes[0].beta1; f.beta2 = classes[0].beta2;
  f.max_norm = max_norm; f.growth_factor = growth_factor; f.backoff_factor = backoff_factor; f.growth_interval = growth_interval;
  HIPCHK(launch_guard_finalize(f, st));
  AdamSegArgs a;
  adam_seg_args(a, params, grads, exp_avg, exp_avg_sq, n, table_dev, nsegs, classes, nclasses);
  a.state = state;
  HIPCHK(launch_adam_segmented(a, st));
  return DMM_OK;
}

namespace {
hipError_t upload(void* dst, const void* src, size_t bytes, hipStream_t st) {
  const hipError_t e = hipStreamSynchronize(st);
  return e != hipSuccess ? e : hipMemcpy(dst, src, bytes, hipMemcpyHostToDevice);
}
struct OneConv {
  int esz, SLOT, BK;
  int Ho, Wo, Hout, Wout, ostride, istride;
  std::vector<std::vector<Tap>> phase_taps;
  std::vector<std::pair<int, int>> phase_xy;
  int Cst;
};
int rup(int v, int m) { return (v + m - 1) / m * m; }

bool geometry(const dmm_conv_desc* d, OneConv& g) {
  g.esz = (int)dtype_size(d->dtype);
  g.SLOT = 16 / g.esz;
  g.BK = 4 * g.SLOT;
  g.Cst = d->Cin;
  g.ostride = 1;
  g.istride = 1;
  if (d->Cin % 8 || d->Cout % 8 == 7) return false;
  if (d->transposed) {
    g.Ho = d->H; g.Wo = d->W; g.Hout = 2 * d->H; g.Wout = 2 * d->W; g.ostride = 2;
    for (int py = 0; py < 2; ++py)
      for (int px = 0; px < 2; ++px) { g.phase_taps.push_back(taps_convT_phase(py, px)); g.phase_xy.push_back({py, px}); }
    return true;
  }
  if (d->mode == 2) { g.Ho = d->H / 2; g.Wo = d->W / 2; g.phase_taps.push_back(taps_conv(1, 1, 0)); }
  else if (d->mode == 1) { g.Ho = 2 * d->H; g.Wo = 2 * d->W; g.phase_taps.push_back(taps_conv(d->R, d->S, d->pad)); }
  else {
    g.Ho = (d->H + 2 * d->pad - d->R) / d->stride + 1;
    g.Wo = (d->W + 2 * d->pad - d->S) / d->stride + 1;
    g.istride = d->stride;
    g.phase_taps.push_back(taps_conv(d->R, d->S, d->pad));
  }
  g.Hout = g.Ho; g.Wout = g.Wo;
  g.phase_xy.push_back({0, 0});
  return true;
}

struct Scratch {
  uint8_t* base;
  size_t off = 0;
  void* take(size_t bytes) {
    off = (off + 255) / 256 * 256;
    void* p = base ? base + off : nullptr;
    off += bytes;
    return p;
  }
};

size_t layout_fwd(const dmm_conv_desc* d, const OneConv& g, uint8_t* scratch, const float* w, float* dw, std::vector<PackDesc>& packs,
                  PackDesc** dev_descs, int** dev_prefix, std::vector<int>& prefix, int& total_rows) {
  Scratch S{scratch};
  *dev_descs = (PackDesc*)S.take(8 * sizeof(PackDesc));
  *dev_prefix = (int*)S.take(8 * sizeof(int));
  total_rows = 0;
  const long long RS = (long long)d->R * d->S;
  for (size_t ph = 0; ph < g.phase_taps.size(); ++ph) {
    PackDesc pd;
    memset(&pd, 0, sizeof(pd));
    pd.w = w; pd.gw = dw;
    pd.N = d->Cout; pd.Npad = rup(d->Cout, 32); pd.nseg = 1;
    if (!d->transposed) { pd.sn = d->Cin * RS; pd.sk = RS; } else { pd.sn = RS; pd.sk = (long long)d->Cout * RS; }
    pd.st = 1;
    fill_pack_seg(pd.seg[0], g.phase_taps[ph], d->Cin, g.Cst, 0, g.BK);
    const size_t elems = (size_t)pd.seg[0].nchunks * pd.Npad * g.BK;
    pd.dst = S.take(elems * g.esz);
    pd.dpack = (float*)S.take(elems * sizeof(float));
    prefix.push_back(total_rows);
    total_rows += pd.seg[0].nchunks * pd.Npad;
    packs.push_back(pd);
  }
  return S.off;
}
}

size_t dmm_conv_scratch_bytes(const dmm_conv_desc* d) {
  OneConv g;
  if (!d || !geometry(d, g)) return 0;
  std::vector<PackDesc> packs;
  std::vector<int> prefix;
  PackDesc* dd; int* dp; int tr;
  size_t fwd = layout_fwd(d, g, nullptr, nullptr, nullptr, packs, &dd, &dp, prefix, tr);
  const size_t dg = (size_t)((d->R * d->S * rup(d->Cout, 8) + g.BK - 1) / g.BK + 16) * rup(d->Cin, 128) * g.BK * g.esz;
  return fwd + dg + 2 * dg + (size_t)rup(d->Cout, 8) * 8 + 8192 + (size_t)W5_SBUF64_FLOATS * sizeof(float);
}

static void fill_one_seg(Seg& s, const dmm_conv_desc* d, const OneConv& g, const void* x, const float* scale, const float* shift,
                         const std::vector<Tap>& taps) {
  memset(&s, 0, sizeof(s));
  s.src = x; s.ld = g.Cst; s.Hs = d->H; s.Ws = d->W; s.C = g.Cst; s.Cpad = g.Cst;
  s.mode = d->transposed ? 0 : d->mode;
  s.istride = g.istride;
  if (d->bn_relu) { s.scale = scale; s.shift = shift; }
  fill_seg_taps(s, taps, g.BK);
}

int dmm_last_impl(void) { return g_last_impl; }
unsigned dmm_impl_mask(int reset) { const unsigned m = g_impl_mask; if (reset) g_impl_mask = 0; return m; }
const char* dmm_impl_name(int impl) { return impl >= 0 && impl < IMPL_COUNT ? kImplNames[impl] : "?"; }

int dmm_conv_forward(const dmm_conv_desc* d, const void* x, const float* w, const float* scale, const float* shift, void* y,
                     double* stats, void* scratch, void* stream) {
  OneConv g;
  if (!d || !geometry(d, g)) return fail(DMM_ERR_INVALID, "unsupported conv descriptor");
  hipStream_t st = (hipStream_t)stream;
  std::vector<PackDesc> packs;
  std::vector<int> prefix;
  PackDesc* dd; int* dp; int total_rows;
  layout_fwd(d, g, (uint8_t*)scratch, w, nullptr, packs, &dd, &dp, prefix, total_rows);
  HIPCHK(upload(dd, packs.data(), packs.size() * sizeof(PackDesc), st));
  HIPCHK(upload(dp, prefix.data(), prefix.size() * sizeof(int), st));
  HIPCHK(hipStreamSynchronize(st));
  HIPCHK(launch_pack(dd, dp, (int)packs.size(), total_rows, d->dtype, st));
  if (stats) HIPCHK(hipMemsetAsync(stats, 0, 2 * d->Cout * sizeof(double), st));
  for (size_t ph = 0; ph < packs.size(); ++ph) {
    ConvArgs a;
    memset(&a, 0, sizeof(a));
    a.nseg = 1;
    fill_one_seg(a.seg[0], d, g, x, scale, shift, g.phase_taps[ph]);
    a.B = d->B; a.Ho = g.Ho; a.Wo = g.Wo; a.M = d->B * g.Ho * g.Wo;
    a.wpack = packs[ph].dst; a.N = d->Cout; a.Npad = packs[ph].Npad;
    a.out = y; a.ldo = d->Cout; a.Hout = g.Hout; a.Wout = g.Wout; a.ostride = g.ostride;
    a.py = g.phase_xy[ph].first; a.px = g.phase_xy[ph].second;
    if (stats) { a.stat_sum = stats; a.stat_sq = stats + d->Cout; }
    HIPCHK(launch_igemm(a, d->dtype, EPI_STORE, d->use_mfma != 0, st, IMPL_AUTO, g_family_off));
  }
  return DMM_OK;
}

static void set_eff_grad(Seg& s, const void* yfwd, int ldy, const float* q, const float* r, const float* zeros) {
  if (q == nullptr) return;
  s.src2 = yfwd; s.ld2 = ldy; s.q = q; s.r = r; s.ql = zeros; s.rl = zeros;
}

static PackDesc dgrad_pack_desc(const dmm_conv_desc* d, const OneConv& g, const std::vector<Tap>& taps, const float* w, int npad) {
  PackDesc pd;
  memset(&pd, 0, sizeof(pd));
  const long long RS = (long long)d->R * d->S;
  pd.w = w;
  pd.N = d->Cin; pd.Npad = npad; pd.nseg = 1;
  if (!d->transposed) { pd.sn = RS; pd.sk = d->Cin * RS; } else { pd.sn = (long long)d->Cout * RS; pd.sk = RS; }
  pd.st = 1;
  fill_pack_seg(pd.seg[0], taps, d->Cout, rup(d->Cout, 8), 0, g.BK);
  return pd;
}

int dmm_conv_wgrad_ex(const dmm_conv_desc* d, const void* x, const void* dy, const float* scale, const float* shift, const void* yfwd,
                      const float* q, const float* r, int transposed_form, float* dw, void* scratch, void* stream) {
  OneConv g;
  if (!d || !geometry(d, g)) return fail(DMM_ERR_INVALID, "unsupported conv descriptor");
  if ((q != nullptr) != (r != nullptr) || (q != nullptr && yfwd == nullptr)) return fail(DMM_ERR_INVALID, "q, r and yfwd come together");
  hipStream_t st = (hipStream_t)stream;
  const size_t wn = (size_t)d->Cin * d->Cout * d->R * d->S;
  if (transposed_form) {
    if (d->transposed || d->mode != 0 || d->stride != 1 || d->R * d->S <= 1 || !d->bn_relu)
      return fail(DMM_ERR_INVALID, "the transposed form serves unit-stride multi-tap convolutions behind BN+ReLU");
    const std::vector<Tap> taps = taps_conv_dgrad(d->R, d->S, d->pad);
    const int cs = g.Cst;
    const int npad = rup(cs, cs >= 384 || cs % 128 == 0 ? 128 : (cs >= 64 ? 64 : 32));
    Scratch S{(uint8_t*)scratch};
    PackDesc* dd = (PackDesc*)S.take(sizeof(PackDesc));
    int* dp = (int*)S.take(sizeof(int));
    float* zeros = (float*)S.take((size_t)rup(d->Cout, 8) * sizeof(float) + 64);
    PackDesc pd = dgrad_pack_desc(d, g, taps, dw, npad);
    const size_t elems = (size_t)pd.seg[0].nchunks * pd.Npad * g.BK;
    pd.dpack = (float*)S.take(elems * sizeof(float));
    pd.gw = dw;
    if (S.off > dmm_conv_scratch_bytes(d)) return fail(DMM_ERR_INVALID, "scratch too small");
    HIPCHK(hipMemsetAsync(scratch, 0, S.off, st));
    int zero = 0;
    HIPCHK(upload(dd, &pd, sizeof(pd), st));
    HIPCHK(upload(dp, &zero, sizeof(int), st));
    HIPCHK(hipStreamSynchronize(st));
    WgradArgs a;
    memset(&a, 0, sizeof(a));
    a.nseg = 1;
    Seg& sq = a.seg[0];
    sq.src = dy; sq.ld = d->Cout; sq.Hs = g.Hout; sq.Ws = g.Wout; sq.C = rup(d->Cout, 8); sq.Cpad = sq.C; sq.mode = G_PLAIN; sq.istride = 1;
    set_eff_grad(sq, yfwd, d->Cout, q, r, zeros);
    fill_seg_taps(sq, taps, g.BK);
    a.B = d->B; a.Ho = g.Ho; a.Wo = g.Wo; a.M = d->B * g.Ho * g.Wo;
    fill_one_seg(a.dy, d, g, x, scale, shift, taps_conv(1, 1, 0));
    a.dy.istride = 1;
    a.N = g.Cst; a.Npad = pd.Npad;
    a.dpack = (float*)pd.dpack;
    void* part = nullptr;
    Resolved wg3;
    const unsigned deny = g_family_off;
    if (d->use_mfma && !((deny >> IMPL_WG3) & 1u) && wg3_resolve(a, d->dtype, wg3)) {
      HIPCHK(hipMallocAsync(&part, (size_t)W3_MAX_SLOTS * W3_SLOT_FLOATS * sizeof(float), st));
      a.part = (float*)part;
      a.part_slots = W3_MAX_SLOTS;
    }
    const hipError_t e1 = launch_wgrad(a, d->dtype, d->use_mfma != 0, st, IMPL_AUTO, deny);
    if (part != nullptr) hipFreeAsync(part, st);
    HIPCHK(e1);
    HIPCHK(hipMemsetAsync(dw, 0, wn * sizeof(float), st));
    HIPCHK(launch_unpack(dd, dp, 1, pd.seg[0].nchunks * pd.Npad, d->dtype, 1.0f, st));
    return DMM_OK;
  }
  std::vector<PackDesc> packs;
  std::vector<int> prefix;
  PackDesc* dd; int* dp; int total_rows;
  const size_t used = layout_fwd(d, g, (uint8_t*)scratch, dw , dw, packs, &dd, &dp, prefix, total_rows);
  Scratch S{(uint8_t*)scratch, used};
  float* zeros = (float*)S.take((size_t)rup(d->Cout, 8) * sizeof(float) + 64);
  if (S.off > dmm_conv_scratch_bytes(d)) return fail(DMM_ERR_INVALID, "scratch too small");
  HIPCHK(hipMemsetAsync(scratch, 0, S.off, st));
  HIPCHK(upload(dd, packs.data(), packs.size() * sizeof(PackDesc), st));
  HIPCHK(upload(dp, prefix.data(), prefix.size() * sizeof(int), st));
  HIPCHK(hipStreamSynchronize(st));
  for (size_t ph = 0; ph < packs.size(); ++ph) {
    WgradArgs a;
    memset(&a, 0, sizeof(a));
    a.nseg = 1;
    fill_one_seg(a.seg[0], d, g, x, scale, shift, g.phase_taps[ph]);
    a.B = d->B; a.Ho = g.Ho; a.Wo = g.Wo; a.M = d->B * g.Ho * g.Wo;
    a.dy.src = dy; a.dy.ld = d->Cout; a.dy.Hs = g.Hout; a.dy.Ws = g.Wout; a.dy.C = rup(d->Cout, 8); a.dy.Cpad = a.dy.C;
    a.dy.mode = G_PLAIN; a.dy.istride = g.ostride; a.dy.ntaps = 1; a.dy.nchunks = 1;
    a.dy.taps[0] = (short)((g.phase_xy[ph].first & 0xff) | ((g.phase_xy[ph].second & 0xff) << 8));
    set_eff_grad(a.dy, yfwd, d->Cout, q, r, zeros);
    a.N = d->Cout; a.Npad = packs[ph].Npad;
    a.dpack = (float*)packs[ph].dpack;
    HIPCHK(launch_wgrad(a, d->dtype, d->use_mfma != 0, st, IMPL_AUTO, g_family_off));
  }
  HIPCHK(hipMemsetAsync(dw, 0, wn * sizeof(float), st));
  HIPCHK(launch_unpack(dd, dp, (int)packs.size(), total_rows, d->dtype, 1.0f, st));
  return DMM_OK;
}

int dmm_conv5_wgrad_stats(const dmm_conv_desc* d, const void* x, const void* dy, const float* w, const float* scale, const float* shift,
                          float* dw, double* red, void* scratch, void* stream) {
  OneConv g;
  if (!d || !geometry(d, g)) return fail(DMM_ERR_INVALID, "unsupported conv descriptor");
  if (d->transposed || d->mode != 0 || d->stride != 1 || d->R != 5 || d->S != 5 || d->pad != 2 || !d->bn_relu || d->Cin != 64 || d->Cout > 4 ||
      d->dtype == DMM_F32 || !d->use_mfma)
    return fail(DMM_ERR_INVALID, "serves the 5x5 convolution of 64 channels onto <= 4 behind BN+ReLU in 16-bit storage");
  hipStream_t st = (hipStream_t)stream;
  const size_t wn = (size_t)d->Cin * d->Cout * 25;
  const std::vector<Tap> taps = taps_conv_dgrad(5, 5, 2);
  Scratch S{(uint8_t*)scratch};
  PackDesc* dd = (PackDesc*)S.take(sizeof(PackDesc));
  int* dp = (int*)S.take(sizeof(int));
  PackDesc pd = dgrad_pack_desc(d, g, taps, dw, 64);
  const size_t elems = (size_t)pd.seg[0].nchunks * pd.Npad * g.BK;
  pd.dpack = (float*)S.take(elems * sizeof(float));
  pd.gw = dw;
  float* sbuf = (float*)S.take((size_t)W5_SBUF64_FLOATS * sizeof(float));
  if (S.off > dmm_conv_scratch_bytes(d)) return fail(DMM_ERR_INVALID, "scratch too small");
  HIPCHK(hipMemsetAsync(scratch, 0, S.off, st));
  HIPCHK(hipMemsetAsync(red, 0, 2 * (size_t)d->Cin * sizeof(double), st));
  int zero = 0;
  HIPCHK(upload(dd, &pd, sizeof(pd), st));
  HIPCHK(upload(dp, &zero, sizeof(int), st));
  HIPCHK(hipStreamSynchronize(st));
  WgradArgs a;
  memset(&a, 0, sizeof(a));
  a.nseg = 1;
  Seg& sq = a.seg[0];
  sq.src = dy; sq.ld = d->Cout; sq.Hs = g.Hout; sq.Ws = g.Wout; sq.C = rup(d->Cout, 8); sq.Cpad = sq.C; sq.mode = G_PLAIN; sq.istride = 1;
  fill_seg_taps(sq, taps, g.BK);
  a.B = d->B; a.Ho = g.Ho; a.Wo = g.Wo; a.M = d->B * g.Ho * g.Wo;
  fill_one_seg(a.dy, d, g, x, scale, shift, taps_conv(1, 1, 0));
  a.dy.istride = 1;
  a.N = g.Cst; a.Npad = pd.Npad;
  a.dpack = (float*)pd.dpack;
  a.sbuf = sbuf;
  a.t_mean = shift + d->Cin; a.t_invstd = shift + 2 * d->Cin;
  HIPCHK(launch_wgrad(a, d->dtype, true, st, IMPL_AUTO, g_family_off));
  if (g_last_impl != IMPL_WG5) return fail(DMM_ERR_STATE, "the factor form is wg5.hip's");
  Fin64Args f;
  memset(&f, 0, sizeof(f));
  f.sbuf = sbuf; f.dpack = a.dpack; f.Npad = a.Npad;
  f.w = w; f.Kin = d->Cin; f.nreal = d->Cout; f.dtype = d->dtype;
  for (int t = 0; t < 25; ++t) f.tapw[t] = (unsigned char)(pd.seg[0].tapw[t] & 0xff);
  f.scale = scale; f.shift = shift; f.mean = shift + d->Cin; f.invstd = shift + 2 * d->Cin;
  f.red1 = red; f.red2 = red + d->Cin;
  HIPCHK(launch_wg5_fin64(f, st));
  HIPCHK(hipMemsetAsync(dw, 0, wn * sizeof(float), st));
  HIPCHK(launch_unpack(dd, dp, 1, pd.seg[0].nchunks * pd.Npad, d->dtype, 1.0f, st));
  return DMM_OK;
}

int dmm_conv_wgrad(const dmm_conv_desc* d, const void* x, const void* dy, const float* scale, const float* shift, float* dw, void* scratch,
                   void* stream) {
  return dmm_conv_wgrad_ex(d, x, dy, scale, shift, nullptr, nullptr, nullptr, 0, dw, scratch, stream);
}

static int build_dgrad(const dmm_conv_desc* d, const OneConv& g, const void* x, const void* dy, const float* w, const float* scale,
                       const float* shift, const void* yfwd, const float* q, const float* r, void* gx, int accumulate, double* red,
                       Scratch& S, int npad, ConvArgs& a, hipStream_t st) {
  std::vector<Tap> taps;
  int istride = 1, rH = d->H, rW = d->W, pool2 = 0, ostride = 1;
  if (d->transposed) { taps = taps_convT_dgrad(); istride = 2; }
  else if (d->mode == 2) { taps = taps_conv(1, 1, 0); rH = d->H / 2; rW = d->W / 2; pool2 = 1; ostride = 2; }
  else if (d->mode == 1) { taps = taps_up2_merged_dgrad(); istride = 2; }
  else taps = taps_conv_dgrad(d->R, d->S, d->pad);
  PackDesc* dd = (PackDesc*)S.take(sizeof(PackDesc));
  int* dp = (int*)S.take(sizeof(int));
  float* zeros = (float*)S.take((size_t)rup(d->Cout, 8) * sizeof(float) + 64);
  PackDesc pd = dgrad_pack_desc(d, g, taps, w, npad);
  pd.dst = S.take((size_t)pd.seg[0].nchunks * pd.Npad * g.BK * g.esz);
  if (S.off > dmm_conv_scratch_bytes(d)) return fail(DMM_ERR_INVALID, "scratch too small");
  int zero = 0;
  HIPCHK(hipMemsetAsync(zeros, 0, (size_t)rup(d->Cout, 8) * sizeof(float) + 64, st));
  HIPCHK(upload(dd, &pd, sizeof(pd), st));
  HIPCHK(upload(dp, &zero, sizeof(int), st));
  HIPCHK(hipStreamSynchronize(st));
  HIPCHK(launch_pack(dd, dp, 1, pd.seg[0].nchunks * pd.Npad, d->dtype, st));
  HIPCHK(hipMemsetAsync(red, 0, 2 * d->Cin * sizeof(double), st));
  memset(&a, 0, sizeof(a));
  a.nseg = 1;
  Seg& s = a.seg[0];
  const int kc = rup(d->Cout, 8);
  s.src = dy; s.ld = d->Cout; s.Hs = g.Hout; s.Ws = g.Wout; s.C = kc; s.Cpad = kc; s.mode = G_PLAIN; s.istride = istride;
  set_eff_grad(s, yfwd, d->Cout, q, r, zeros);
  fill_seg_taps(s, taps, g.BK);
  a.B = d->B; a.Ho = rH; a.Wo = rW; a.M = d->B * rH * rW;
  a.wpack = pd.dst; a.N = d->Cin; a.Npad = pd.Npad;
  a.out = gx; a.ldo = d->Cin; a.Hout = d->H; a.Wout = d->W; a.ostride = ostride;
  a.bx = x; a.ldbx = d->Cin; a.bscale = scale; a.bshift = shift;
  a.bmean = shift + d->Cin; a.binvstd = shift + 2 * d->Cin;
  a.red1 = red; a.red2 = red + d->Cin;
  a.accumulate = accumulate ? 1 : 0; a.pool2 = pool2;
  return DMM_OK;
}

int dmm_conv_dgrad_ex(const dmm_conv_desc* d, const void* x, const void* dy, const float* w, const float* scale, const float* shift,
                      const void* yfwd, const float* q, const float* r, void* gx, int accumulate, double* red, void* scratch,
                      void* stream) {
  OneConv g;
  if (!d || !geometry(d, g) || !d->bn_relu) return fail(DMM_ERR_INVALID, "unsupported conv descriptor (dgrad needs bn_relu)");
  if (d->mode == 0 && !d->transposed && d->stride != 1) return fail(DMM_ERR_INVALID, "strided conv dgrad is not on the hot path");
  if ((q != nullptr) != (r != nullptr) || (q != nullptr && yfwd == nullptr)) return fail(DMM_ERR_INVALID, "q, r and yfwd come together");
  hipStream_t st = (hipStream_t)stream;
  Scratch S{(uint8_t*)scratch};
  ConvArgs a;
  const int cs = g.Cst;
  const int npad = rup(cs, cs >= 384 || cs % 128 == 0 ? 128 : (cs >= 64 ? 64 : 32));
  const int rc = build_dgrad(d, g, x, dy, w, scale, shift, yfwd, q, r, gx, accumulate, red, S, npad, a, st);
  if (rc) return rc;
  HIPCHK(launch_igemm(a, d->dtype, EPI_BNBWD, d->use_mfma != 0, st, IMPL_AUTO, g_family_off));
  return DMM_OK;
}

int dmm_conv_dgrad(const dmm_conv_desc* d, const void* x, const void* dy, const float* w, const float* scale, const float* shift, void* gx,
                   double* red, void* scratch, void* stream) {
  return dmm_conv_dgrad_ex(d, x, dy, w, scale, shift, nullptr, nullptr, nullptr, gx, 0, red, scratch, stream);
}

int dmm_conv1x1_backward_fused(const dmm_conv_desc* d, const void* x, const void* dy, const float* w, const float* scale,
                               const float* shift, const void* yfwd, const float* q, const float* r, void* gx, int accumulate,
                               float* dw, double* red, void* scratch, void* stream) {
  OneConv g;
  if (!d || !geometry(d, g) || !d->bn_relu || d->R != 1 || d->S != 1 || d->stride != 1 || d->transposed || d->mode != 0)
    return fail(DMM_ERR_INVALID, "the fused backward serves 1x1 unit-stride convolutions behind BN+ReLU");
  if ((q != nullptr) != (r != nullptr) || (q != nullptr && yfwd == nullptr)) return fail(DMM_ERR_INVALID, "q, r and yfwd come together");
  hipStream_t st = (hipStream_t)stream;
  std::vector<PackDesc> packs;
  std::vector<int> prefix;
  PackDesc* dd; int* dp; int total_rows;
  const size_t used = layout_fwd(d, g, (uint8_t*)scratch, dw, dw, packs, &dd, &dp, prefix, total_rows);
  HIPCHK(hipMemsetAsync(scratch, 0, used, st));
  HIPCHK(upload(dd, packs.data(), packs.size() * sizeof(PackDesc), st));
  HIPCHK(upload(dp, prefix.data(), prefix.size() * sizeof(int), st));
  Scratch S{(uint8_t*)scratch, used};
  Bw1Args b;
  memset(&b, 0, sizeof(b));
  const int cs = g.Cst;
  const int npad = rup(cs, cs >= 384 || cs % 128 == 0 ? 128 : (cs >= 64 ? 64 : 32));
  const int rc = build_dgrad(d, g, x, dy, w, scale, shift, yfwd, q, r, gx, accumulate, red, S, npad, b.c, st);
  if (rc) return rc;
  WgradArgs wa;
  memset(&wa, 0, sizeof(wa));
  wa.nseg = 1;
  fill_one_seg(wa.seg[0], d, g, x, scale, shift, g.phase_taps[0]);
  wa.B = d->B; wa.Ho = g.Ho; wa.Wo = g.Wo; wa.M = d->B * g.Ho * g.Wo;
  wa.dy = b.c.seg[0];
  wa.N = d->Cout; wa.Npad = packs[0].Npad;
  wa.dpack = (float*)packs[0].dpack;
  if (!bw1_eligible(wa, b.c, d->dtype, g_family_off)) return fail(DMM_ERR_INVALID, "not a pair bw1.hip fuses (16-bit storage, 128 output channels, Cin % 32 == 0)");
  b.dpack = wa.dpack; b.dNpad = wa.Npad; b.wC = wa.seg[0].C;
  {
    const Bw1Geom q = bw1_geometry(b.c);
    b.part_slots = q.nsplit * q.nct;
    void* part = nullptr;
    HIPCHK(hipMallocAsync(&part, (size_t)b.part_slots * B1_SLOT_FLOATS * sizeof(float), st));
    b.part = (float*)part;
    const hipError_t e1 = launch_bw1(b, d->dtype, st);
    const hipError_t e2 = e1 == hipSuccess ? launch_bw1_reduce(b, st) : e1;
    hipFreeAsync(part, st);
    HIPCHK(e2);
  }
  const size_t wn = (size_t)d->Cin * d->Cout;
  HIPCHK(hipMemsetAsync(dw, 0, wn * sizeof(float), st));
  HIPCHK(launch_unpack(dd, dp, (int)packs.size(), total_rows, d->dtype, 1.0f, st));
  return DMM_OK;
}

}
```

dmmfods_amd/csrc/plan.h:

```cpp
#pragma once
#include <cstring>
#include <stdexcept>
#include <string>
#include <vector>

#include "../../include/dmmfods_hip.h"
#include "common.h"
#include "pointwise.h"

namespace dmm {

struct plan_sizing_error : std::runtime_error { using std::runtime_error::runtime_error; };

struct TensorInfo {
  std::string name;
  int kind, ndim;
  int64_t shape[4];
  int64_t off;
};

struct Tap {
  int dy, dx;
  unsigned tapw;
};

std::vector<Tap> taps_conv(int R, int S, int pad);
std::vector<Tap> taps_conv_dgrad(int R, int S, int pad);
std::vector<Tap> taps_convT_phase(int py, int px);
std::vector<Tap> taps_convT_dgrad();
std::vector<Tap> taps_up2_merged_dgrad();
std::vector<Tap> taps_up2_phase(int e, int f);
std::vector<Tap> taps_conv_phase_s2(int e, int f);
void fill_seg_taps(Seg& s, const std::vector<Tap>& taps, int BK);
void fill_pack_seg(PackSeg& p, const std::vector<Tap>& taps, int Creal, int Cpad, int koff, int BK);

enum OpKind { OP_MEMSET = 0, OP_CONVERT, OP_IGEMM, OP_WGRAD, OP_BNFIN, OP_BNBWD, OP_POOL, OP_POOLBWD, OP_BCE, OP_PACK, OP_UNPACK,
              OP_COPY, OP_APPLYCORR, OP_BW1, OP_JOIN, OP_BW1RED, OP_RAWFIN, OP_FIN64 };

struct MemsetArgs { void* p; size_t bytes; };
struct CopyArgs { void* dst; const void* src; size_t bytes; };
struct PackArgs {
  const PackDesc* descs; const int* prefix; int ndesc, total_rows; float grad_scale;
  const PackDesc* tdescs; const PackTile* tiles; int nt1, nt9;
};

struct Op {
  int kind;
  int epi;
  int leaf;
  int chain;
  int signal;
  int impl;
  double flops;
  double bytes;
  char label[56];
  union {
    MemsetArgs ms;
    CopyArgs cp;
    ConvertArgs cv;
    ConvArgs c;
    WgradArgs w;
    BnFinalizeArgs bf;
    BnBwdFinalizeArgs bb;
    MaxpoolArgs mp;
    MaxpoolBwdArgs mpb;
    BceArgs bce;
    PackArgs pk;
    ApplyCorrArgs ac;
    Bw1Args b1;
    RawFinArgs rf;
    Fin64Args f64;
  };
  Op() { memset(static_cast<void*>(this), 0, sizeof(*this)); signal = -1; impl = IMPL_AUTO; }
};

}

struct GradBucket {
  int64_t off = 0, n = 0;
  int ev_main = -1, ev_side = -1;
  int ready = -1;
};

struct PlanSwitches {
  bool no_pack_tiles = false, no_hf = false, no_c3_merge = false, no_cvp_merge = false, no_wgp_merge = false, no_two_pass = false,
       no_eff_compact = false, no_s2_interleave = false, no_raw_stats = false, no_r1_stats = false;
  int pack_cut = 0;
  static PlanSwitches from_environment();
};

struct dmm_plan {
  dmm_model_desc desc;
  PlanSwitches sw;
  unsigned deny = 0;
  std::vector<dmm::TensorInfo> tensors;
  int64_t nparams = 0, nbuf = 0;
  size_t zero_bytes = 0, zero_bwd_bytes = 0, main_bytes = 0;
  double fwd_flops = 0;
  bool bound = false;
  void* ws = nullptr;
  float *params = nullptr, *grads = nullptr, *buffers = nullptr;
  std::vector<dmm::Op> fwd_train, fwd_eval, bwd;
  std::vector<int> convert_ops_train, convert_ops_eval;
  int logits_op_train = -1, logits_op_eval = -1;
  int bce_op = -1, bce_only_valid = 0;
  dmm::Op bce_only;
  int loss_kind = 0;
  float loss_alpha[8] = {1, 1, 1, 1, 1, 1, 1, 1}, loss_gamma[8] = {2, 2, 2, 2, 2, 2, 2, 2};
  bool grad_accumulate = false;
  bool encoder_frozen = false;
  const float* dyn_scale = nullptr;
  double* metrics = nullptr;
  size_t metrics_bytes = 0;
  std::vector<dmm::PackDesc> packs;
  std::vector<int> pack_prefix;
  std::vector<dmm::PackDesc> unpacks;
  std::vector<int> unpack_prefix;
  std::vector<dmm::PackTile> pack_tiles, unpack_tiles;
  size_t bucket_bytes = 0;
  std::vector<GradBucket> buckets;
  std::vector<void*> bucket_events;
  int prof_max_passes = 0;
  int prof_pass[2] = {0, 0};
  std::vector<std::vector<void*>> prof_events[2];
  std::string prof_filter;
  int device = -1;
  bool used_side = false, used_capture = false;
  std::vector<void*> join_events;
  std::vector<void*> fork_events;
  struct GraphEntry { const void* key[4]; void* exec; unsigned long long stamp; };
  struct GraphCache {
    std::vector<GraphEntry> entries;
    const void* seen[4][4] = {};
    int nseen = 0;
    int captures = 0;
    unsigned long long epoch = 0;
  };
  GraphCache graphs[2];
  bool graph_failed = false;
  bool dp_used = false;
  unsigned long long graph_clock = 0;
  long long graph_replays[2] = {0, 0};
};
```

dmmfods_amd/csrc/pointwise.h:

```cpp
#pragma once
#include "../../include/dmmfods_hip.h"
#include "common.h"

namespace dmm {

struct ConvertArgs {
  const float* src1;
  const float* src2;
  int C1, C2;
  void* dst;
  int B, H, W;
  double* stat_sum;
  double* stat_sq;
  float scale;
  const float* dyn_scale;
};

struct BnFinalizeArgs {
  const double* sum;
  const double* sq;
  int stat_stride;
  double count;
  double count_unbiased;
  const float* gamma;
  const float* beta;
  float* running_mean;
  float* running_var;
  float* scale;
  float* shift;
  float* mean;
  float* invstd;
  int C;
  int training;
  float momentum, eps;
};

struct BnBwdFinalizeArgs {
  const double* red1;
  const double* red2;
  int stat_stride;
  const float* mean;
  const float* invstd;
  const float* scale;
  float* dgamma;
  float* dbeta;
  double* qd;
  double* rd;
  float* q;
  float* r;
  float* ql;
  float* rl;
  double count;
  float grad_scale;
  int C;
  int accumulate;
};

struct MaxpoolArgs {
  const void* y0;
  int ld0, H0, W0, B, C;
  const float* scale;
  const float* shift;
  void* out;
  int ldo, Hp, Wp;
  unsigned char* argmax;
  double* stat_sum;
  double* stat_sq;
  int stat_stride;
};

struct MaxpoolBwdArgs {
  const void* y0;
  int ld0, H0, W0, B, C;
  const float* scale;
  const float* shift;
  const void* gpool;
  const void* xpool;
  const float* q;
  const float* r;
  const float* ql;
  const float* rl;
  const float* mean;
  const float* invstd;
  int ldg, Hp, Wp;
  const unsigned char* argmax;
  void* gy0;
  double* red1;
  double* red2;
  int stat_stride;
};

struct BceArgs {
  const float* logits;
  const float* target;
  void* dlogits;
  double* out;
  int B, NC, H, W;
  float thr, loss_scale;
  int kind, from_prob;
  float alpha[8], gamma[8];
  float* loss_out;
  float* dx_out;
  int metrics;
  const float* dyn_scale;
};

struct ApplyCorrArgs {
  void* g;
  const void* y;
  const float* q;
  const float* r;
  const float* ql;
  const float* rl;
  size_t npix;
  int C, ldg, ldy;
};

struct AdamArgs {
  float* p;
  const float* g;
  float* m;
  float* v;
  size_t n;
  float beta1, beta2, eps, weight_decay, step_size, bc2_sqrt, grad_scale;
};

constexpr int GUARD_PARTIALS = 512;
struct GradSumsqArgs {
  const float* g;
  size_t n;
  double* partials;
  int accumulate;
};
constexpr int ADAM_MAX_CLASSES = DMM_ADAM_MAX_CLASSES;
constexpr int ADAM_SEG_CHUNK = 1024;
constexpr int ADAM_SEG_MAX_GRID = 2048;
struct AdamSegDev {
  long long begin, end;
  int cls, pad;
};
struct AdamSegClass {
  float lr, beta1, beta2, eps;
  float weight_decay;
  float decay;
  float step_size, bc2_sqrt;
  long long t0;
  int decoupled;
  int active;
};
struct AdamSegArgs {
  float* p;
  const float* g;
  float* m;
  float* v;
  size_t n;
  const AdamSegDev* segs;
  const int* first;
  int nsegs, nchunks, nclasses;
  int vec_ok;
  float grad_scale;
  const dmm_guard_state* state;
  AdamSegClass cls[ADAM_MAX_CLASSES];
};
struct GuardFinalizeArgs {
  const double* partials;
  dmm_guard_state* state;
  float lr, beta1, beta2;
  float max_norm;
  float growth_factor, backoff_factor;
  int growth_interval;
};

struct PackSeg {
  int Creal, Cpad, ntaps, nchunks, koff;
  unsigned tapw[MAX_TAPS];
};

struct PackDesc {
  const float* w;
  void* dst;
  float* gw;
  const float* dpack;
  int N, Npad, nseg;
  int shared_master;
  long long sn, sk, st;
  PackSeg seg[2];
  int rs;
  int tiled;
};
struct PackTile { int desc, nsib, n0, cg; };

struct Bw1Args {
  ConvArgs c;
  float* dpack;
  int dNpad, wC;
  float* part;
  int part_slots;
  int nct, ntiles, tiles_per_wg, xcd_group, nsplit;
};
struct Bw1Geom { int nct, ntiles, tiles_per_wg, nsplit, xcd_group, nwg; };
Bw1Geom bw1_geometry(const ConvArgs& a);
constexpr int B1_SLOT_FLOATS = 4 * 128 * 32;
bool bw1_eligible(const WgradArgs& w, const ConvArgs& d, int dtype, unsigned deny);
hipError_t launch_bw1(const Bw1Args& g, int dtype, hipStream_t st);
hipError_t launch_bw1_reduce(const Bw1Args& g, hipStream_t st);
hipError_t launch_igemm(const ConvArgs& a, int dtype, int epi, bool mfma, hipStream_t st, int impl = IMPL_AUTO, unsigned deny = 0);
hipError_t launch_wgrad(WgradArgs a, int dtype, bool mfma, hipStream_t st, int impl = IMPL_AUTO, unsigned deny = 0);
int igemm_pick(const ConvArgs& a, int dtype, int epi, bool mfma, unsigned deny);
int wgrad_pick(const WgradArgs& a, int dtype, bool mfma, unsigned deny);
hipError_t launch_wg5_rawfin(const RawFinArgs& a, hipStream_t st);
hipError_t launch_wg5_fin64(const Fin64Args& a, hipStream_t st);
hipError_t launch_convert_input(const ConvertArgs& a, int dtype, hipStream_t st);
hipError_t launch_bn_finalize(const BnFinalizeArgs& a, hipStream_t st);
hipError_t launch_bn_bwd_finalize(const BnBwdFinalizeArgs& a, hipStream_t st);
hipError_t launch_maxpool_fwd(const MaxpoolArgs& a, int dtype, hipStream_t st);
hipError_t launch_maxpool_bwd(const MaxpoolBwdArgs& a, int dtype, hipStream_t st);
hipError_t launch_bce_metrics(const BceArgs& a, int dtype, hipStream_t st);
hipError_t launch_adam(const AdamArgs& a, hipStream_t st);
hipError_t launch_grad_sumsq(const GradSumsqArgs& a, hipStream_t st);
hipError_t launch_guard_finalize(const GuardFinalizeArgs& a, hipStream_t st);
hipError_t launch_adam_guarded(const AdamArgs& a, const dmm_guard_state* state, hipStream_t st);
hipError_t launch_adam_guarded_from(const AdamArgs& a, const dmm_guard_state* state, float lr, int64_t t0, hipStream_t st);
hipError_t launch_adam_segmented(const AdamSegArgs& a, hipStream_t st);
hipError_t launch_guard_init(dmm_guard_state* dev, float scale, int64_t applied, int32_t tracker, hipStream_t st);
hipError_t launch_apply_corr(const ApplyCorrArgs& a, int dtype, hipStream_t st);
hipError_t launch_pack(const PackDesc* descs_dev, const int* prefix_dev, int ndesc, int total_rows, int dtype, hipStream_t st,
                       const PackDesc* tile_descs = nullptr, const PackTile* tiles_dev = nullptr, int nt1 = 0, int nt9 = 0);
hipError_t launch_unpack(const PackDesc* descs_dev, const int* prefix_dev, int ndesc, int total_rows, int dtype, float grad_scale,
                         hipStream_t st, const PackDesc* tile_descs = nullptr, const PackTile* tiles_dev = nullptr, int nt1 = 0, int nt9 = 0,
                         bool accumulate = false);

#if defined(__HIPCC__)
template <bool COH>
__device__ __forceinline__ double stat_load(const double* p) {
  if constexpr (COH) return __hip_atomic_load(p, __ATOMIC_RELAXED, __HIP_MEMORY_SCOPE_AGENT);
  else return *p;
}

template <bool COH>
__device__ __forceinline__ void bn_finalize_channel(const BnFinalizeArgs& a, int c) {
  float mean, var;
  if (a.training) {
    double su = stat_load<COH>(a.sum + c), sq = stat_load<COH>(a.sq + c);
    if (a.stat_stride)
      for (int k = 1; k < STAT_REPS; ++k) { su += stat_load<COH>(a.sum + c + (size_t)k * a.stat_stride); sq += stat_load<COH>(a.sq + c + (size_t)k * a.stat_stride); }
    const double m = su / a.count;
    double v = sq / a.count - m * m;
    if (v < 0) v = 0;
    mean = (float)m;
    var = (float)v;
    const double unb = a.count_unbiased > 1 ? v * (a.count_unbiased / (a.count_unbiased - 1.0)) : v;
    a.running_mean[c] = (1.f - a.momentum) * a.running_mean[c] + a.momentum * mean;
    a.running_var[c] = (1.f - a.momentum) * a.running_var[c] + a.momentum * (float)unb;
  } else {
    mean = a.running_mean[c];
    var = a.running_var[c];
  }
  const float invstd = 1.0f / sqrtf(var + a.eps);
  const float s = a.gamma[c] * invstd;
  a.scale[c] = s;
  a.shift[c] = a.beta[c] - mean * s;
  a.mean[c] = mean;
  a.invstd[c] = invstd;
}

template <bool COH>
__device__ __forceinline__ void bn_bwd_finalize_channel(const BnBwdFinalizeArgs& a, int c) {
  double S1 = stat_load<COH>(a.red1 + c), S2 = stat_load<COH>(a.red2 + c);
  if (a.stat_stride)
    for (int k = 1; k < STAT_REPS; ++k) { S1 += stat_load<COH>(a.red1 + c + (size_t)k * a.stat_stride); S2 += stat_load<COH>(a.red2 + c + (size_t)k * a.stat_stride); }
  const double mu = a.mean[c], is = a.invstd[c];
  const double dotp = S2;
  const float dg = (float)(dotp * a.grad_scale), db = (float)(S1 * a.grad_scale);
  if (a.accumulate) {
    a.dgamma[c] += dg;
    a.dbeta[c] += db;
  } else {
    a.dgamma[c] = dg;
    a.dbeta[c] = db;
  }
  if (a.qd != nullptr) {
    const double s = a.scale[c];
    const double c1 = S1 / a.count, c2 = dotp / a.count;
    const double q = a.qd[c] + (-s * c1 + s * c2 * mu * is);
    const double r = a.rd[c] + (-s * c2 * is);
    a.qd[c] = q;
    a.rd[c] = r;
    const float qh = (float)q, rh = (float)r;
    a.q[c] = qh; a.ql[c] = (float)(q - (double)qh);
    a.r[c] = rh; a.rl[c] = (float)(r - (double)rh);
  }
}

#endif

}
```

dmmfods_amd/csrc/wg3.hip:

```cpp
#include <algorithm>
#include <cmath>
#include <cstdlib>

#include "common.h"
#include "dispatch.h"
#include "gather.h"
#include "isa.h"
#include "pointwise.h"

#ifndef WG3_DBG
#define WG3_DBG 0
#endif
namespace dmm {

constexpr int W3_TH = 8, W3_TW = 16, W3_HH = 10, W3_HW = 18;
constexpr int W3_CA = 128, W3_CY = 32;
constexpr int W3_A_BYTES = BM * W3_CA * 2;
constexpr int W3_Y_BYTES = W3_HH * W3_HW * W3_CY * 2;
constexpr int W3_IMG = W3_A_BYTES + W3_Y_BYTES;
constexpr int W3_LDS = 2 * W3_IMG;
constexpr int W3_NT = 512;

struct Wg3Args {
  WgradArgs w;
  int tiles_y, tiles_x, ntiles, tiles_per_wg;
  float* part;
};

template <typename T, int NA, int NY, int PQ, int MODE>
__device__ __forceinline__ void w3_sync(typename TT<T>::vec (&ra)[NA], typename TT<T>::vec (&ry)[NY], typename TT<T>::vec (&ry2)[PQ == 2 ? NY : 1]) {
  static_assert(NA == 8 && NY == 3, "DMM_V8 / DMM_V3 below");
  if constexpr (PQ == 2) {
    if constexpr (MODE == 2) DMM_VM_HOLD(DMM_V8(ra), DMM_V3(ry), DMM_V3(ry2));
    else DMM_VM_WAIT(MODE == 0 ? NA + 2 * NY : 0, DMM_V8(ra), DMM_V3(ry), DMM_V3(ry2));
  } else {
    if constexpr (MODE == 2) DMM_VM_HOLD(DMM_V8(ra), DMM_V3(ry));
    else DMM_VM_WAIT(MODE == 0 ? NA + NY : 0, DMM_V8(ra), DMM_V3(ry));
  }
}

template <typename T, int PQ>
__global__ __launch_bounds__(W3_NT, 1) void wg3_kernel(const Wg3Args g) {
  static_assert(sizeof(T) == 2, "16-bit storage");
  typedef typename TT<T>::vec V;
  constexpr int SLOT = 8;
  constexpr int NL = 256;
  constexpr int NA = BM * (W3_CA / SLOT) / NL;
  constexpr int NY = (W3_HH * W3_HW * (W3_CY / SLOT) + NL - 1) / NL;
  const WgradArgs& a = g.w;
  const Seg& sy_ = a.seg[0];
  const Seg& sa = a.dy;

  extern __shared__ __attribute__((aligned(16))) unsigned char smem[];
  const int tid = threadIdx.x, lane = tid & 63, wave = tid >> 6;
  const int t_beg = blockIdx.x * g.tiles_per_wg, t_end = min(g.ntiles, t_beg + g.tiles_per_wg);
  if (t_beg >= t_end) return;
  const int nt = t_end - t_beg;

  if (wave >= 4) {
    const int lt = tid - NL;
    const int ca = lt & 15, pa0 = lt >> 4;
    const int cy = lt & 3, hy0 = lt >> 2;
    SlotK<SLOT> ka, ky;
    ka.k0 = load_fv<SLOT>(sa.scale + ca * SLOT); ka.k1 = load_fv<SLOT>(sa.shift + ca * SLOT); ka.k2 = 0.f; ka.k3 = 0.f;
    ky.k0 = 0.f; ky.k1 = 0.f; ky.k2 = 0.f; ky.k3 = 0.f;
    if (PQ == 2) { ky.k0 = load_fv<SLOT>(sy_.q + cy * SLOT); ky.k1 = load_fv<SLOT>(sy_.r + cy * SLOT); }
    const T* asrc = (const T*)sa.src + ca * SLOT;
    const T* ysrc = (const T*)sy_.src + cy * SLOT;
    const T* ysrc2 = (const T*)sy_.src2 + cy * SLOT;
    int hyy[NY], hxx[NY];
#pragma unroll
    for (int i = 0; i < NY; ++i) {
      const int hp = min(hy0 + 64 * i, W3_HH * W3_HW - 1);
      hyy[i] = hp / W3_HW - 1; hxx[i] = hp % W3_HW - 1;
    }
    struct LSet {
      V ra[NA], ry[NY], ry2[PQ == 2 ? NY : 1];
      unsigned oka, oky;
    };
    const int tiles_img = g.tiles_y * g.tiles_x;
    int cb = t_beg / tiles_img, cty, ctx, cleft = nt;
    { const int tr = t_beg - cb * tiles_img; cty = tr / g.tiles_x; ctx = tr - cty * g.tiles_x; }
    auto issue = [&](LSet& R) {
      const int y0 = cty * W3_TH, x0 = ctx * W3_TW;
      R.oka = 0; R.oky = 0;
      const int xa = x0 + pa0;
      const size_t arow = (size_t)cb * sa.Hs;
#pragma unroll
      for (int i = 0; i < NA; ++i) {
        const int y = y0 + i;
        if (y < a.Ho && xa < a.Wo) R.oka |= 1u << i;
        const size_t pix = (arow + min(y, sa.Hs - 1)) * sa.Ws + min(xa, sa.Ws - 1);
        if (!(WG3_DBG & 4)) gload16(R.ra[i], asrc + pix * sa.ld);
      }
      const size_t yrow = (size_t)cb * sy_.Hs;
#pragma unroll
      for (int i = 0; i < NY; ++i) {
        const int y = y0 + hyy[i], x = x0 + hxx[i];
        if (hy0 + 64 * i < W3_HH * W3_HW && (unsigned)y < (unsigned)sy_.Hs && (unsigned)x < (unsigned)sy_.Ws) R.oky |= 1u << i;
        const size_t pix = (yrow + min(max(y, 0), sy_.Hs - 1)) * sy_.Ws + min(max(x, 0), sy_.Ws - 1);
        if (!(WG3_DBG & 4)) gload16(R.ry[i], ysrc + pix * sy_.ld);
        if constexpr (PQ == 2) { if (!(WG3_DBG & 4)) gload16(R.ry2[i], ysrc2 + pix * sy_.ld2); }
      }
      if (--cleft > 0) {
        if (++ctx == g.tiles_x) { ctx = 0; if (++cty == g.tiles_y) { cty = 0; ++cb; } }
      }
    };
    auto store = [&](LSet& R, int set, bool wait = true) {
      if (wait && !(WG3_DBG & 4)) w3_sync<T, NA, NY, PQ, 0>(R.ra, R.ry, R.ry2);
      unsigned char* As = smem + set * W3_IMG;
      unsigned char* Ys = As + W3_A_BYTES;
      V z;
#pragma unroll
      for (int e = 0; e < SLOT; ++e) z[e] = (T)0;
#pragma unroll
      for (int i = 0; i < NA; ++i) {
        const int p = pa0 + 16 * i;
        const V v = bn_relu_slot(R.ra[i], ka);
        *(V*)(As + p * 256 + ((ca * 16) ^ ((p & 3) << 6))) = ((R.oka >> i) & 1) ? v : z;
      }
#pragma unroll
      for (int i = 0; i < NY; ++i) {
        const int hp = hy0 + 64 * i;
        if (hp < W3_HH * W3_HW) {
          V v = R.ry[i];
          if constexpr (PQ == 2) v = eff_grad_slot(R.ry[i], R.ry2[i], ky);
          *(V*)(Ys + hp * 64 + cy * 16) = ((R.oky >> i) & 1) ? v : z;
        }
      }
    };
#pragma unroll
    for (int e = 0; e < SLOT; ++e) {
      asm volatile("" : "+v"(ka.k0[e]), "+v"(ka.k1[e]));
      if constexpr (PQ == 2) asm volatile("" : "+v"(ky.k0[e]), "+v"(ky.k1[e]));
    }
    LSet R0, R1;
    issue(R0);
    issue(R1);
    for (int k = 0; k + 1 < nt; k += 2) {
      store(R0, 0);
      lds_barrier();
      issue(R0);
      store(R1, 1);
      lds_barrier();
      issue(R1);
    }
    if (!(WG3_DBG & 4)) {
      w3_sync<T, NA, NY, PQ, 1>(R0.ra, R0.ry, R0.ry2);
      w3_sync<T, NA, NY, PQ, 2>(R1.ra, R1.ry, R1.ry2);
    }
    if (nt & 1) {
      store(R0, 0, false);
      lds_barrier();
    }
    return;
  }

  f32x16 acc[9];
#pragma unroll
  for (int t = 0; t < 9; ++t)
#pragma unroll
    for (int i = 0; i < 16; ++i) acc[t][i] = 0.f;

  const int tg = lane >> 4, ti = lane & 15, tq = ti >> 2, tp = ti & 3;
  const int acol = ((32 * wave + 16 * (tg & 1) + 4 * tp) * 2) ^ (tq << 6);
  const int arow = 8 * (tg >> 1) + tq;
  const int ycol = (16 * (tg & 1) + 4 * tp) * 2;
  int yoff[9];
#pragma unroll
  for (int t = 0; t < 9; ++t) {
    const int tw = sy_.taps[t];
    const int dy = (int)(signed char)(tw & 0xff), dx = (int)(signed char)((tw >> 8) & 0xff);
    yoff[t] = ((1 + dy) * W3_HW + (arow + 1 + dx)) * 64 + ycol;
  }
  for (int k = 0; k < nt; ++k) {
    lds_barrier();
    const unsigned char* As = smem + (k & 1) * W3_IMG;
    const unsigned char* Ys = As + W3_A_BYTES;
    if (!(WG3_DBG & 2)) {
#pragma unroll 2
      for (int ms = 0; ms < W3_TH; ++ms) {
        const unsigned char* ap = As + (16 * ms + arow) * 256 + acol;
        const V af = frag16<T>(lds_tr16(ap), lds_tr16(ap + 4 * 256));
        const unsigned char* yp = Ys + ms * (W3_HW * 64);
#pragma unroll
        for (int t = 0; t < 9; ++t) {
          const V bf = frag16<T>(lds_tr16(yp + yoff[t]), lds_tr16(yp + yoff[t] + 4 * 64));
          acc[t] = mma16(af, bf, acc[t]);
        }
      }
    }
  }

  const int r = lane & 31, h = lane >> 5;
  if (g.part != nullptr) {
    f32x4* slot = (f32x4*)(g.part + (size_t)blockIdx.x * W3_SLOT_FLOATS);
#pragma unroll
    for (int t = 0; t < 9; ++t)
#pragma unroll
      for (int j = 0; j < 4; ++j) {
        const f32x4 v = {acc[t][4 * j], acc[t][4 * j + 1], acc[t][4 * j + 2], acc[t][4 * j + 3]};
        if (!(WG3_DBG & 1) || v[0] == 1.2345e33f) slot[((t * 4 + wave) * 4 + j) * 64 + lane] = v;
      }
  } else {
#pragma unroll
    for (int t = 0; t < 9; ++t)
#pragma unroll
      for (int i = 0; i < 16; ++i) {
        const int c = 32 * wave + (i & 3) + 8 * (i >> 2) + 4 * h;
        if (!(WG3_DBG & 1) || acc[t][i] == 1.2345e33f) atomic_add_f32(a.dpack + ((size_t)t * a.Npad + c) * 32 + r, acc[t][i]);
      }
  }
}

constexpr int W3_RG = 8;
__global__ __launch_bounds__(256) void wg3_reduce_kernel(const float* __restrict__ part, float* __restrict__ dpack, int nslots) {
  __shared__ f32x4 red[W3_RG][32];
  const int o = threadIdx.x & 31, sg = threadIdx.x >> 5;
  const int f = blockIdx.x * 32 + o;
  const float* p = part + (size_t)f * 4;
  f32x4 s = {0.f, 0.f, 0.f, 0.f};
  int k = sg;
  for (; k + 3 * W3_RG < nslots; k += 4 * W3_RG) {
    const f32x4 v0 = __builtin_nontemporal_load((const f32x4*)(p + (size_t)k * W3_SLOT_FLOATS));
    const f32x4 v1 = __builtin_nontemporal_load((const f32x4*)(p + (size_t)(k + W3_RG) * W3_SLOT_FLOATS));
    const f32x4 v2 = __builtin_nontemporal_load((const f32x4*)(p + (size_t)(k + 2 * W3_RG) * W3_SLOT_FLOATS));
    const f32x4 v3 = __builtin_nontemporal_load((const f32x4*)(p + (size_t)(k + 3 * W3_RG) * W3_SLOT_FLOATS));
    s += (v0 + v1) + (v2 + v3);
  }
  for (; k < nslots; k += W3_RG) s += __builtin_nontemporal_load((const f32x4*)(p + (size_t)k * W3_SLOT_FLOATS));
  red[sg][o] = s;
  __syncthreads();
  if (sg == 0) {
    f32x4 t4 = red[0][o];
#pragma unroll
    for (int g2 = 1; g2 < W3_RG; ++g2) t4 += red[g2][o];
    const int l = f & 63, j = (f >> 6) & 3, w = (f >> 8) & 3, t = f >> 10;
    float* d = dpack + ((size_t)t * W3_CA + 32 * w + 8 * j + 4 * (l >> 5)) * 32 + (l & 31);
#pragma unroll
    for (int q = 0; q < 4; ++q) d[q * 32] += t4[q];
  }
}

struct Wg3Launch {
  Wg3Args g;
  LdsLauncher<Wg3Args> run;
};

bool wg3_resolve(const WgradArgs& a, int dtype, Resolved& r) {
  if (dtype == DT_F32 || a.nseg != 1) return false;
  const Seg& q = a.seg[0];
  const Seg& p = a.dy;
  if (q.mode != G_PLAIN || q.istride != 1 || q.ntaps != 9 || q.C != W3_CY || q.Cpad != W3_CY || q.Hs != a.Ho || q.Ws != a.Wo || q.scale != nullptr)
    return false;
  if (p.mode != G_PLAIN || p.istride != 1 || p.ntaps != 1 || p.taps[0] != 0 || p.C != W3_CA || p.Hs != a.Ho || p.Ws != a.Wo || p.scale == nullptr)
    return false;
  if (a.N != W3_CA || a.Npad != W3_CA) return false;
  bool seen[9] = {false, false, false, false, false, false, false, false, false};
  for (int t = 0; t < 9; ++t) {
    const int dy = (int)(signed char)(q.taps[t] & 0xff), dx = (int)(signed char)((q.taps[t] >> 8) & 0xff);
    if (dy < -1 || dy > 1 || dx < -1 || dx > 1 || seen[(dy + 1) * 3 + dx + 1]) return false;
    seen[(dy + 1) * 3 + dx + 1] = true;
  }
  Wg3Launch& l = r.put<Wg3Launch>();
  Wg3Args& g = l.g;
  g.w = a;
  g.tiles_y = (a.Ho + W3_TH - 1) / W3_TH;
  g.tiles_x = (a.Wo + W3_TW - 1) / W3_TW;
  g.ntiles = a.B * g.tiles_y * g.tiles_x;
  if (dtype == DT_F16) l.run = q.q ? launch_lds<wg3_kernel<f16, 2>, Wg3Args> : launch_lds<wg3_kernel<f16, 0>, Wg3Args>;
  else l.run = q.q ? launch_lds<wg3_kernel<bf16, 2>, Wg3Args> : launch_lds<wg3_kernel<bf16, 0>, Wg3Args>;
  return true;
}

hipError_t wg3_launch(const Resolved& r, hipStream_t st) {
  const Wg3Launch& l = r.get<Wg3Launch>();
  Wg3Args g = l.g;
  const WgradArgs& a = g.w;
  static const int cus = device_cus();
  static const bool use_slots = lab_int("DMM_WG3_SLOTS", 1) != 0;
  static const int wgs_cap = lab_int("DMM_WG3_WGS", 0);
  g.part = (use_slots && a.part != nullptr) ? a.part : nullptr;
  int nwg = g.part ? std::min(cus, a.part_slots) : (int)std::lround(std::sqrt(12.0 * g.ntiles));
  if (wgs_cap > 0) nwg = std::min(nwg, wgs_cap);
  nwg = std::max(1, std::min(std::min(nwg, cus), g.ntiles));
  g.tiles_per_wg = (g.ntiles + nwg - 1) / nwg;
  nwg = (g.ntiles + g.tiles_per_wg - 1) / g.tiles_per_wg;
  hipError_t e = l.run(W3_LDS, nwg, W3_NT, W3_LDS, st, g);
  if (e == hipSuccess && g.part != nullptr) {
    hipLaunchKernelGGL(wg3_reduce_kernel, dim3(W3_SLOT_FLOATS / 4 / 32), dim3(256), 0, st, g.part, g.w.dpack, nwg);
    e = hipGetLastError();
  }
  return e;
}

}
```

include/dmmfods_hip.h:

```cpp
#ifndef DMMFODS_HIP_H
#define DMMFODS_HIP_H
#include <stddef.h>
#include <stdint.h>

#ifdef __cplusplus
extern "C" {
#endif

typedef enum {
  DMM_OK = 0,
  DMM_ERR_INVALID = -1,
  DMM_ERR_SHAPE = -2,
  DMM_ERR_HIP = -3,
  DMM_ERR_STATE = -4,
  DMM_ERR_NO_DEVICE = -5
} dmm_status;

enum { DMM_F32 = 0, DMM_F16 = 1, DMM_BF16 = 2 };

enum { DMM_T_CONV = 0, DMM_T_CONVT = 1, DMM_T_BN_WEIGHT = 2, DMM_T_BN_BIAS = 3, DMM_T_BN_MEAN = 4, DMM_T_BN_VAR = 5,
       DMM_T_BN_TRACKED = 6 };

typedef struct {
  int32_t growth_rate;
  int32_t num_blocks;
  int32_t block_config[8];
  int32_t num_init_features;
  int32_t bn_size;
  int32_t num_classes;
  int32_t concat_before_block_num;
  int32_t stream_1_in_channels;
  int32_t stream_2_in_channels;
  int32_t batch, height, width;
  int32_t dtype;
  float loss_scale;
  float bn_momentum, bn_eps;
  float iou_threshold;
  int32_t use_mfma;
} dmm_model_desc;

typedef struct dmm_plan dmm_plan;

const char* dmm_last_error(void);
int dmm_version(void);
int dmm_set_option(const char* name, int value);

int dmm_plan_create(const dmm_model_desc* desc, dmm_plan** out);
int dmm_plan_destroy(dmm_plan* plan);

int dmm_plan_num_tensors(const dmm_plan* plan);
int dmm_plan_tensor_info(const dmm_plan* plan, int index, const char** name, int32_t* kind, int32_t* ndim,
                         int64_t shape[4], int64_t* arena_offset);
int64_t dmm_plan_num_params(const dmm_plan* plan);
int64_t dmm_plan_num_buffer_elems(const dmm_plan* plan);
size_t dmm_plan_workspace_bytes(const dmm_plan* plan);
double dmm_plan_forward_flops(const dmm_plan* plan);

int dmm_plan_bind(dmm_plan* plan, void* workspace, size_t workspace_bytes, float* params, float* grads, float* buffers);

int dmm_plan_forward(dmm_plan* plan, const float* stream_1, const float* stream_2, float* logits_out, int training,
                     void* stream);

int dmm_plan_loss_backward(dmm_plan* plan, const float* logits, const float* target, double* metrics_out, void* stream);

enum { DMM_LOSS_BCE = 0, DMM_LOSS_FOCAL = 1 };
int dmm_plan_set_loss(dmm_plan* plan, int kind, const float* alpha, const float* gamma, int nclass);

int dmm_loss_forward(int kind, int from_prob, const float* alpha, const float* gamma, const float* input, const float* target,
                     float* loss_out, float* dinput_out, int batch, int nclass, int height, int width, void* stream);

int dmm_plan_backward(dmm_plan* plan, const float* dlogits, void* stream);

int dmm_plan_set_grad_accumulate(dmm_plan* plan, int accumulate);

int dmm_plan_set_encoder_frozen(dmm_plan* plan, int frozen);

int dmm_plan_num_grad_buckets(const dmm_plan* plan);
int dmm_plan_grad_bucket(const dmm_plan* plan, int index, int64_t* offset, int64_t* count);
int dmm_plan_grad_bucket_wait(dmm_plan* plan, int index, void* stream);

int dmm_plan_profile_begin(dmm_plan* plan, int max_passes);
int dmm_plan_profile_filter(dmm_plan* plan, const char* label_prefix);
int dmm_plan_profile_num_ops(const dmm_plan* plan, int which);
int dmm_plan_profile_op(const dmm_plan* plan, int which, int index, const char** label, double* flops, double* bytes);
int dmm_plan_profile_collect(dmm_plan* plan, int which, double* ms_sum, int n, int* passes);

int dmm_plan_loss_metrics(dmm_plan* plan, const float* logits, const float* target, double* metrics_out, void* stream);

long long dmm_plan_num_graph_replays(const dmm_plan* plan, int which);

int dmm_adam_step(float* params, const float* grads, float* exp_avg, float* exp_avg_sq, int64_t n, float lr, float beta1,
                  float beta2, float eps, float weight_decay, int64_t step, float grad_scale, void* stream);

typedef struct dmm_guard_state {
  float scale;
  float grad_scale;
  double sumsq;
  float grad_norm;
  int32_t found_inf;
  int64_t applied_steps;
  int64_t skipped_steps;
  int32_t growth_tracker;
  float step_size;
  float bc2_sqrt;
  float clip_coef;
  int32_t reserved[2];
} dmm_guard_state;

size_t dmm_grad_guard_scratch_bytes(int64_t n);
int dmm_guard_state_init(dmm_guard_state* dev, float init_scale, int64_t applied_steps, int32_t growth_tracker, void* stream);
int dmm_adam_step_guarded(float* params, const float* grads, float* exp_avg, float* exp_avg_sq, int64_t n, float lr, float beta1,
                          float beta2, float eps, float weight_decay, float max_norm, float growth_factor, float backoff_factor,
                          int32_t growth_interval, dmm_guard_state* state, void* scratch, void* stream);
int dmm_adam_step_guarded_ranges(float* params, const float* grads, float* exp_avg, float* exp_avg_sq, const int64_t* offsets,
                                 const int64_t* counts, const int64_t* t0, int nranges, float lr, float beta1, float beta2, float eps,
                                 float weight_decay, float max_norm, float growth_factor, float backoff_factor, int32_t growth_interval,
                                 dmm_guard_state* state, void* scratch, void* stream);
int dmm_grad_sumsq(const float* grads, int64_t offset, int64_t count, int accumulate, void* scratch, void* stream);
#define DMM_ADAM_MAX_CLASSES 16
typedef struct dmm_adam_segment {
  int64_t begin, count;
  int32_t cls;
} dmm_adam_segment;
typedef struct dmm_adam_class {
  float lr, beta1, beta2, eps, weight_decay;
  int32_t decoupled;
  int64_t t0;
} dmm_adam_class;
size_t dmm_adam_table_bytes(int nsegs, int64_t n);
int dmm_adam_table_init(void* table_dev, const dmm_adam_segment* segs, int nsegs, int64_t n, int nclasses, void* stream);
int dmm_adam_step_segmented(float* params, const float* grads, float* exp_avg, float* exp_avg_sq, int64_t n, const void* table_dev,
                            int nsegs, const dmm_adam_class* classes, int nclasses, int64_t step, float grad_scale, void* stream);
int dmm_adam_step_guarded_segmented(float* params, const float* grads, float* exp_avg, float* exp_avg_sq, int64_t n,
                                    const void* table_dev, int nsegs, const dmm_adam_class* classes, int nclasses, float max_norm,
                                    float growth_factor, float backoff_factor, int32_t growth_interval, dmm_guard_state* state,
                                    void* scratch, void* stream);
int dmm_plan_set_dynamic_loss_scale(dmm_plan* plan, const float* scale_dev);

typedef struct {
  int32_t dtype, use_mfma;
  int32_t B, H, W;
  int32_t Cin, Cout;
  int32_t R, S, stride, pad;
  int32_t transposed;
  int32_t mode;
  int32_t bn_relu;
} dmm_conv_desc;

size_t dmm_conv_scratch_bytes(const dmm_conv_desc* d);
int dmm_conv_forward(const dmm_conv_desc* d, const void* x, const float* w, const float* scale, const float* shift, void* y,
                     double* stats, void* scratch, void* stream);
int dmm_conv_wgrad(const dmm_conv_desc* d, const void* x, const void* dy, const float* scale, const float* shift, float* dw,
                   void* scratch, void* stream);
int dmm_conv_dgrad(const dmm_conv_desc* d, const void* x, const void* dy, const float* w, const float* scale, const float* shift,
                   void* gx, double* red, void* scratch, void* stream);


int dmm_conv_wgrad_ex(const dmm_conv_desc* d, const void* x, const void* dy, const float* scale, const float* shift, const void* yfwd,
                      const float* q, const float* r, int transposed_form, float* dw, void* scratch, void* stream);
int dmm_conv_dgrad_ex(const dmm_conv_desc* d, const void* x, const void* dy, const float* w, const float* scale, const float* shift,
                      const void* yfwd, const float* q, const float* r, void* gx, int accumulate, double* red, void* scratch,
                      void* stream);
int dmm_conv5_wgrad_stats(const dmm_conv_desc* d, const void* x, const void* dy, const float* w, const float* scale, const float* shift,
                          float* dw, double* red, void* scratch, void* stream);
int dmm_conv1x1_backward_fused(const dmm_conv_desc* d, const void* x, const void* dy, const float* w, const float* scale,
                               const float* shift, const void* yfwd, const float* q, const float* r, void* gx, int accumulate,
                               float* dw, double* red, void* scratch, void* stream);

int dmm_last_impl(void);
const char* dmm_impl_name(int impl);
unsigned dmm_impl_mask(int reset);

#ifdef __cplusplus
}
#endif
#endif
```

Measured before the change: 160.1 img/s.

## Batch consecutive WG3 weight-gradient and BW1 reduce launches into grouped kernels

Adds grouped kernels that take a table of several WG3 weight-gradient convolutions, or several BW1 split-reduce jobs, and run them in one launch. A shared tile budget is split across members in proportion to their tile counts. The backward op runner gathers eligible ops, flushes them at dependency points and issues them as one grouped launch plus one grouped reduce. This is on by default on the main stream. It cuts per-kernel launch overhead and small-kernel underutilisation, at the cost of more complex scheduling and changed overlap with the side stream.

```diff
diff --git a/dmmfods_amd/_lib.py b/dmmfods_amd/_lib.py
--- a/dmmfods_amd/_lib.py
+++ b/dmmfods_amd/_lib.py
@@ -138,6 +138,10 @@
     L.dmm_conv_dgrad_ex.argtypes = [C.POINTER(ConvDesc), vp, vp, vp, vp, vp, vp, vp, vp, vp, C.c_int, vp, vp, vp]
     L.dmm_conv1x1_backward_fused.argtypes = [C.POINTER(ConvDesc), vp, vp, vp, vp, vp, vp, vp, vp, vp, C.c_int, vp, vp, vp, vp]
     L.dmm_conv5_wgrad_stats.argtypes = [C.POINTER(ConvDesc), vp, vp, vp, vp, vp, vp, vp, vp, vp]
+    L.dmm_plan_wgrad_batch_counts.argtypes = [vp, C.POINTER(C.c_longlong * 4)]
+    L.dmm_conv_wgrad_grouped.argtypes = [C.POINTER(ConvDesc), C.c_int, vp, vp, vp, vp, vp, vp, vp, vp, vp, C.c_int, C.POINTER(C.c_int), vp]
+    L.dmm_bw1_reduce_grouped.argtypes = [C.c_int, vp, vp, C.POINTER(C.c_int), C.POINTER(C.c_int), C.POINTER(C.c_int), C.c_int,
+                                         C.POINTER(C.c_int), vp]
     _lib = L
     return L
 
@@ -153,6 +157,7 @@
     "dmm_grad_guard_scratch_bytes", "dmm_guard_state_init", "dmm_adam_step_guarded", "dmm_grad_sumsq", "dmm_plan_set_dynamic_loss_scale",
     "dmm_plan_set_grad_accumulate", "dmm_plan_set_encoder_frozen", "dmm_adam_step_guarded_ranges",
     "dmm_adam_table_bytes", "dmm_adam_table_init", "dmm_adam_step_segmented", "dmm_adam_step_guarded_segmented",
+    "dmm_plan_wgrad_batch_counts", "dmm_conv_wgrad_grouped", "dmm_bw1_reduce_grouped",
 ]
 
 
diff --git a/dmmfods_amd/csrc/bw1.hip b/dmmfods_amd/csrc/bw1.hip
--- a/dmmfods_amd/csrc/bw1.hip
+++ b/dmmfods_amd/csrc/bw1.hip
@@ -1,5 +1,6 @@
 #include <algorithm>
 #include <cstdio>
+#include <cstring>
 #include <cstdlib>
 #include <type_traits>
 
@@ -401,7 +402,7 @@
 #undef B1_GO
 }
 
-__global__ __launch_bounds__(256) void bw1_reduce_kernel(const float* __restrict__ part, float* __restrict__ dpack, int nct, int nsplit, int nfloats) {
+__device__ __forceinline__ void bw1_reduce_slots(const float* __restrict__ part, float* __restrict__ dpack, int nct, int nsplit, int nfloats) {
   const int e = (blockIdx.x * 256 + threadIdx.x) * 4;
   if (e >= nct * B1_SLOT_FLOATS) return;
   f32x4 s = {0.f, 0.f, 0.f, 0.f};
@@ -423,15 +424,55 @@
   for (; k < nsplit; ++k) s += *(const f32x4*)(p + (size_t)k * pitch);
   if (e < nfloats) *(f32x4*)(dpack + e) = s;
 }
+__global__ __launch_bounds__(256) void bw1_reduce_kernel(const float* __restrict__ part, float* __restrict__ dpack, int nct, int nsplit, int nfloats) {
+  bw1_reduce_slots(part, dpack, nct, nsplit, nfloats);
+}
+struct Bw1RedGroupArgs { Bw1RedMember m[B1_RED_GROUP_MAX]; };
+static_assert(sizeof(Bw1RedMember) % 8 == 0, "members are read with aligned scalar loads");
+__global__ __launch_bounds__(256) void bw1_reduce_group_kernel(const Bw1RedGroupArgs g) {
+  const Bw1RedMember& m = g.m[blockIdx.y];
+  bw1_reduce_slots(m.part, m.dpack, m.nct, m.nsplit, m.nfloats);
+}
+
+static bool bw1_reduce_member(const Bw1Args& g, Bw1RedMember& m) {
+  const ConvArgs& a = g.c;
+  if (a.M <= 0) return false;
+  const Bw1Geom q = bw1_geometry(a);
+  if (!bw1_uses_part(g, q)) return false;
+  m.part = g.part; m.dpack = g.dpack; m.nct = q.nct; m.nsplit = q.nsplit;
+  m.nfloats = ((g.wC + 31) / 32) * g.dNpad * 32;
+  return true;
+}
+
+hipError_t launch_bw1_reduce_member(const Bw1RedMember& m, hipStream_t st) {
+  const int nthreads = m.nct * B1_SLOT_FLOATS / 4;
+  hipLaunchKernelGGL(bw1_reduce_kernel, dim3((nthreads + 255) / 256), dim3(256), 0, st, m.part, m.dpack, m.nct, m.nsplit, m.nfloats);
+  return hipGetLastError();
+}
 
 hipError_t launch_bw1_reduce(const Bw1Args& g, hipStream_t st) {
-  const ConvArgs& a = g.c;
-  if (a.M <= 0) return hipSuccess;
-  const Bw1Geom q = bw1_geometry(a);
-  if (!bw1_uses_part(g, q)) return hipSuccess;
-  const int nfloats = ((g.wC + 31) / 32) * g.dNpad * 32;
-  const int nthreads = q.nct * B1_SLOT_FLOATS / 4;
-  hipLaunchKernelGGL(bw1_reduce_kernel, dim3((nthreads + 255) / 256), dim3(256), 0, st, g.part, g.dpack, q.nct, q.nsplit, nfloats);
+  Bw1RedMember m;
+  if (!bw1_reduce_member(g, m)) return hipSuccess;
+  return launch_bw1_reduce_member(m, st);
+}
+
+bool bw1_reduce_group_add(Bw1RedGroup& G, const Bw1Args& g) {
+  Bw1RedMember m;
+  if (!bw1_reduce_member(g, m)) return true;
+  if (G.n >= B1_RED_GROUP_MAX) return false;
+  G.m[G.n++] = m;
+  return true;
+}
+
+hipError_t bw1_reduce_group_launch(Bw1RedGroup& G, hipStream_t st) {
+  if (G.n <= 0) return hipSuccess;
+  Bw1RedGroupArgs a;
+  memset(&a, 0, sizeof(a));
+  int nct = 0;
+  for (int i = 0; i < G.n; ++i) { a.m[i] = G.m[i]; nct = std::max(nct, G.m[i].nct); }
+  const int n = G.n;
+  G.n = 0;
+  hipLaunchKernelGGL(bw1_reduce_group_kernel, dim3((nct * (B1_SLOT_FLOATS / 4) + 255) / 256, n), dim3(256), 0, st, a);
   return hipGetLastError();
 }
 
diff --git a/dmmfods_amd/csrc/capi.cpp b/dmmfods_amd/csrc/capi.cpp
--- a/dmmfods_amd/csrc/capi.cpp
+++ b/dmmfods_amd/csrc/capi.cpp
@@ -35,6 +35,7 @@
 static bool g_overlap_wgrad = getenv("DMM_NO_OVERLAP") == nullptr;
 static int g_graph = getenv("DMM_GRAPH") ? std::max(1, atoi(getenv("DMM_GRAPH"))) : 0;
 static unsigned long long g_option_epoch = 1;
+static int g_batch_wgrad = 1;
 static int g_bucket_mb = getenv("DMM_GRAD_BUCKET_MB") ? atoi(getenv("DMM_GRAD_BUCKET_MB")) : 25;
 static std::atomic<unsigned> g_family_off{lab_family_off()};
 static unsigned plan_deny(const dmm_plan* p) { return (p->sw.no_hf ? 1u << IMPL_HF : 0u) | g_family_off; }
@@ -116,6 +117,11 @@
   ++g_option_epoch;
   if (std::string(name) == "overlap_wgrad") { g_overlap_wgrad = value != 0; return DMM_OK; }
   if (std::string(name) == "graph") { g_graph = value; return DMM_OK; }
+  if (std::string(name) == "batch_wgrad") {
+    if (value < 0 || value > 2) return fail(DMM_ERR_INVALID, "batch_wgrad must be 0, 1 or 2");
+    g_batch_wgrad = value;
+    return DMM_OK;
+  }
   for (const auto& o : kFamilyOptions)
     if (std::string(name) == o.option) {
       if (value != 0) g_family_off &= ~(1u << o.family);
@@ -311,6 +317,32 @@
     }
   };
   auto join = [&]() { join_side(); join_pack(); };
+  const bool batch = g_batch_wgrad != 0;
+  static const long long w3_batch_tiles = lab_int("DMM_WG3_BATCH_TILES", 0);
+  Wg3Group w3g;
+  Bw1RedGroup rdg;
+  std::vector<size_t> w3_members, rd_members;
+  const bool batch_main = g_batch_wgrad == 1;
+  hipStream_t batch_st = (overlap && !batch_main) ? side_st : st;
+  auto flush_members = [&](std::vector<size_t>& members, auto&& launch) -> hipError_t {
+    if (members.empty()) return hipSuccess;
+    for (size_t k = 0; k + 1 < members.size(); ++k)
+      if (selected(ops[members[k]])) {
+        hipEventRecord((hipEvent_t)(*evs)[2 * (ev_offset + members[k])], batch_st);
+        hipEventRecord((hipEvent_t)(*evs)[2 * (ev_offset + members[k]) + 1], batch_st);
+      }
+    const size_t last = members.back();
+    const bool sel_last = selected(ops[last]);
+    members.clear();
+    if (sel_last) hipEventRecord((hipEvent_t)(*evs)[2 * (ev_offset + last)], batch_st);
+    const hipError_t fe = launch();
+    if (sel_last) hipEventRecord((hipEvent_t)(*evs)[2 * (ev_offset + last) + 1], batch_st);
+    return fe;
+  };
+  auto flush_w3 = [&]() { return flush_members(w3_members, [&] { ++p->batch_counts[0]; return wg3_group_launch(w3g, batch_st); }); };
+  auto flush_rd = [&]() { return flush_members(rd_members, [&] { ++p->batch_counts[2]; return bw1_reduce_group_launch(rdg, batch_st); }); };
+  auto flush_all = [&]() { const hipError_t e1 = flush_w3(), e2 = flush_rd(); return e1 != hipSuccess ? e1 : e2; };
+  auto flush_failed = [&](hipError_t fe) { join(); return fail(DMM_ERR_HIP, std::string("grouped weight-gradient launch: ") + hipGetErrorString(fe)); };
   static const bool host_prof = lab_flag("DMM_HOST_PROF");
   static double hp_launch[32] = {0}, hp_fork[32] = {0};
   static long hp_n[32] = {0}, hp_lists = 0;
@@ -320,9 +352,30 @@
     hipError_t e = hipSuccess;
     const double hp_t0 = host_prof ? now() : 0.0;
     double hp_t1 = hp_t0;
+    const bool forks = !o.chain && o.leaf != 2 && o.leaf != 3 && (o.kind == OP_WGRAD || o.leaf);
+    bool as_w3 = false, as_rd = false;
+    if (batch && forks && o.signal < 0) {
+      if (o.kind == OP_WGRAD && o.impl == IMPL_WG3 && mfma) {
+        as_w3 = wg3_group_add(w3g, o.w, dt);
+        if (!as_w3 && w3g.n > 0) {
+          if ((e = flush_w3()) != hipSuccess) return flush_failed(e);
+          as_w3 = wg3_group_add(w3g, o.w, dt);
+        }
+      } else if (o.kind == OP_BW1RED) {
+        as_rd = bw1_reduce_group_add(rdg, o.b1);
+        if (!as_rd) {
+          if ((e = flush_rd()) != hipSuccess) return flush_failed(e);
+          as_rd = bw1_reduce_group_add(rdg, o.b1);
+        }
+      }
+    }
+    const bool rd_added = as_rd && rdg.n > (int)rd_members.size();
+    if (!as_w3 && !as_rd && (forks || o.leaf == 3 || o.signal >= 0 || (o.kind == OP_JOIN && o.epi != 1)))
+      if ((e = flush_all()) != hipSuccess) return flush_failed(e);
     hipStream_t lst = st;
     if (overlap && o.leaf == 3 && forked) {
       lst = side_st;
+    } else if (batch_main && forks && ((o.kind == OP_WGRAD && o.impl == IMPL_WG3) || o.kind == OP_BW1RED)) {
     } else if (overlap && !o.chain && (o.kind == OP_WGRAD || o.leaf)) {
       if (nfork >= p->fork_events.size()) {
         hipEvent_t fe = pool_event(dp, false);
@@ -336,7 +389,7 @@
       if (o.leaf == 2) pack_pending = true; else forked = true;
       if (host_prof) hp_t1 = now();
     }
-    const bool sel = selected(o);
+    const bool sel = selected(o) && !as_w3 && !rd_added;
     if (sel) hipEventRecord((hipEvent_t)(*evs)[2 * (ev_offset + i)], lst);
     const bool fam_check = (o.kind == OP_IGEMM || o.kind == OP_WGRAD) && o.impl != IMPL_AUTO;
     const unsigned mask_before = g_impl_mask;
@@ -346,9 +399,17 @@
       case OP_COPY: e = hipMemcpyAsync(o.cp.dst, o.cp.src, o.cp.bytes, hipMemcpyDeviceToDevice, lst); break;
       case OP_CONVERT: e = launch_convert_input(o.cv, dt, lst); break;
       case OP_IGEMM: e = launch_igemm(o.c, dt, o.epi, mfma, lst, o.impl); break;
-      case OP_WGRAD: e = launch_wgrad(o.w, dt, mfma, lst, o.impl); break;
+      case OP_WGRAD:
+        if (as_w3) { note_impl(IMPL_WG3); w3_members.push_back(i); ++p->batch_counts[1]; break; }
+        if (o.impl == IMPL_WG3 && o.w.M > 0) { ++p->batch_counts[0]; ++p->batch_counts[1]; }
+        e = launch_wgrad(o.w, dt, mfma, lst, o.impl);
+        break;
       case OP_BW1: e = launch_bw1(o.b1, dt, lst); break;
-      case OP_BW1RED: e = launch_bw1_reduce(o.b1, lst); break;
+      case OP_BW1RED:
+        if (as_rd) { if (rd_added) { rd_members.push_back(i); ++p->batch_counts[3]; } break; }
+        { Bw1RedGroup one; if (bw1_reduce_group_add(one, o.b1) && one.n > 0) { ++p->batch_counts[2]; ++p->batch_counts[3]; } }
+        e = launch_bw1_reduce(o.b1, lst);
+        break;
       case OP_RAWFIN: e = launch_wg5_rawfin(o.rf, lst); break;
       case OP_FIN64: e = launch_wg5_fin64(o.f64, lst); break;
       case OP_JOIN: if (o.epi == 1) join_pack(); else join_side(); break;
@@ -376,6 +437,7 @@
       if (!why.empty()) { join(); return fail(DMM_ERR_STATE, why); }
     }
     if (sel) hipEventRecord((hipEvent_t)(*evs)[2 * (ev_offset + i) + 1], lst);
+    if (as_w3 && w3_batch_tiles > 0 && w3g.tiles >= w3_batch_tiles && (e = flush_w3()) != hipSuccess) return flush_failed(e);
     if (pack_pending && o.leaf == 2) hipEventRecord((hipEvent_t)p->join_events[nside], lst);
     if (o.signal >= 0 && !capturing) {
       while ((int)p->bucket_events.size() <= o.signal) {
@@ -385,6 +447,10 @@
       }
       hipEventRecord((hipEvent_t)p->bucket_events[o.signal], lst);
     }
+  }
+  {
+    const hipError_t fe = flush_all();
+    if (fe != hipSuccess) return flush_failed(fe);
   }
   join();
   if (host_prof && ++hp_lists == 40) {
@@ -540,6 +606,12 @@
   if (rc) return rc;
   HIPCHK(launch_convert_input(cv, plan->desc.dtype, st));
   return run_ops(plan, plan->bwd, st, -1, (size_t)plan->bce_op + 1, 0);
+}
+
+int dmm_plan_wgrad_batch_counts(const dmm_plan* plan, long long counts[4]) {
+  if (!plan || !counts) return fail(DMM_ERR_INVALID, "null argument");
+  for (int i = 0; i < 4; ++i) counts[i] = plan->batch_counts[i];
+  return DMM_OK;
 }
 
 long long dmm_plan_num_graph_replays(const dmm_plan* plan, int which) {
@@ -1087,6 +1159,41 @@
   return pd;
 }
 
+static int thin_wgrad_setup(const dmm_conv_desc* d, const OneConv& g, const void* x, const void* dy, const float* scale, const float* shift,
+                            const void* yfwd, const float* q, const float* r, float* dw, void* scratch, hipStream_t st, WgradArgs& a,
+                            PackDesc*& dd, int*& dp, int& rows) {
+  const std::vector<Tap> taps = taps_conv_dgrad(d->R, d->S, d->pad);
+  const int cs = g.Cst;
+  const int npad = rup(cs, cs >= 384 || cs % 128 == 0 ? 128 : (cs >= 64 ? 64 : 32));
+  Scratch S{(uint8_t*)scratch};
+  dd = (PackDesc*)S.take(sizeof(PackDesc));
+  dp = (int*)S.take(sizeof(int));
+  float* zeros = (float*)S.take((size_t)rup(d->Cout, 8) * sizeof(float) + 64);
+  PackDesc pd = dgrad_pack_desc(d, g, taps, dw, npad);
+  const size_t elems = (size_t)pd.seg[0].nchunks * pd.Npad * g.BK;
+  pd.dpack = (float*)S.take(elems * sizeof(float));
+  pd.gw = dw;
+  if (S.off > dmm_conv_scratch_bytes(d)) return fail(DMM_ERR_INVALID, "scratch too small");
+  HIPCHK(hipMemsetAsync(scratch, 0, S.off, st));
+  int zero = 0;
+  HIPCHK(upload(dd, &pd, sizeof(pd), st));
+  HIPCHK(upload(dp, &zero, sizeof(int), st));
+  HIPCHK(hipStreamSynchronize(st));
+  memset(&a, 0, sizeof(a));
+  a.nseg = 1;
+  Seg& sq = a.seg[0];
+  sq.src = dy; sq.ld = d->Cout; sq.Hs = g.Hout; sq.Ws = g.Wout; sq.C = rup(d->Cout, 8); sq.Cpad = sq.C; sq.mode = G_PLAIN; sq.istride = 1;
+  set_eff_grad(sq, yfwd, d->Cout, q, r, zeros);
+  fill_seg_taps(sq, taps, g.BK);
+  a.B = d->B; a.Ho = g.Ho; a.Wo = g.Wo; a.M = d->B * g.Ho * g.Wo;
+  fill_one_seg(a.dy, d, g, x, scale, shift, taps_conv(1, 1, 0));
+  a.dy.istride = 1;
+  a.N = g.Cst; a.Npad = pd.Npad;
+  a.dpack = (float*)pd.dpack;
+  rows = pd.seg[0].nchunks * pd.Npad;
+  return DMM_OK;
+}
+
 int dmm_conv_wgrad_ex(const dmm_conv_desc* d, const void* x, const void* dy, const float* scale, const float* shift, const void* yfwd,
                       const float* q, const float* r, int transposed_form, float* dw, void* scratch, void* stream) {
   OneConv g;
@@ -1097,35 +1204,10 @@
   if (transposed_form) {
     if (d->transposed || d->mode != 0 || d->stride != 1 || d->R * d->S <= 1 || !d->bn_relu)
       return fail(DMM_ERR_INVALID, "the transposed form serves unit-stride multi-tap convolutions behind BN+ReLU");
-    const std::vector<Tap> taps = taps_conv_dgrad(d->R, d->S, d->pad);
-    const int cs = g.Cst;
-    const int npad = rup(cs, cs >= 384 || cs % 128 == 0 ? 128 : (cs >= 64 ? 64 : 32));
-    Scratch S{(uint8_t*)scratch};
-    PackDesc* dd = (PackDesc*)S.take(sizeof(PackDesc));
-    int* dp = (int*)S.take(sizeof(int));
-    float* zeros = (float*)S.take((size_t)rup(d->Cout, 8) * sizeof(float) + 64);
-    PackDesc pd = dgrad_pack_desc(d, g, taps, dw, npad);
-    const size_t elems = (size_t)pd.seg[0].nchunks * pd.Npad * g.BK;
-    pd.dpack = (float*)S.take(elems * sizeof(float));
-    pd.gw = dw;
-    if (S.off > dmm_conv_scratch_bytes(d)) return fail(DMM_ERR_INVALID, "scratch too small");
-    HIPCHK(hipMemsetAsync(scratch, 0, S.off, st));
-    int zero = 0;
-    HIPCHK(upload(dd, &pd, sizeof(pd), st));
-    HIPCHK(upload(dp, &zero, sizeof(int), st));
-    HIPCHK(hipStreamSynchronize(st));
     WgradArgs a;
-    memset(&a, 0, sizeof(a));
-    a.nseg = 1;
-    Seg& sq = a.seg[0];
-    sq.src = dy; sq.ld = d->Cout; sq.Hs = g.Hout; sq.Ws = g.Wout; sq.C = rup(d->Cout, 8); sq.Cpad = sq.C; sq.mode = G_PLAIN; sq.istride = 1;
-    set_eff_grad(sq, yfwd, d->Cout, q, r, zeros);
-    fill_seg_taps(sq, taps, g.BK);
-    a.B = d->B; a.Ho = g.Ho; a.Wo = g.Wo; a.M = d->B * g.Ho * g.Wo;
-    fill_one_seg(a.dy, d, g, x, scale, shift, taps_conv(1, 1, 0));
-    a.dy.istride = 1;
-    a.N = g.Cst; a.Npad = pd.Npad;
-    a.dpack = (float*)pd.dpack;
+    PackDesc* dd; int* dp; int rows;
+    const int rc = thin_wgrad_setup(d, g, x, dy, scale, shift, yfwd, q, r, dw, scratch, st, a, dd, dp, rows);
+    if (rc) return rc;
     void* part = nullptr;
     Resolved wg3;
     const unsigned deny = g_family_off;
@@ -1138,7 +1220,7 @@
     if (part != nullptr) hipFreeAsync(part, st);
     HIPCHK(e1);
     HIPCHK(hipMemsetAsync(dw, 0, wn * sizeof(float), st));
-    HIPCHK(launch_unpack(dd, dp, 1, pd.seg[0].nchunks * pd.Npad, d->dtype, 1.0f, st));
+    HIPCHK(launch_unpack(dd, dp, 1, rows, d->dtype, 1.0f, st));
     return DMM_OK;
   }
   std::vector<PackDesc> packs;
@@ -1340,4 +1422,74 @@
   return DMM_OK;
 }
 
-}
+int dmm_conv_wgrad_grouped(const dmm_conv_desc* descs, int n, const void* const* x, const void* const* dy, const float* const* scale,
+                           const float* const* shift, const void* const* yfwd, const float* const* q, const float* const* r,
+                           float* const* dw, void* const* scratch, int grouped, int* launches, void* stream) {
+  if (!descs || n < 1 || !x || !dy || !scale || !shift || !dw || !scratch) return fail(DMM_ERR_INVALID, "null argument");
+  hipStream_t st = (hipStream_t)stream;
+  struct One { WgradArgs a; PackDesc* dd; int* dp; int rows; };
+  std::vector<One> v((size_t)n);
+  for (int i = 0; i < n; ++i) {
+    const dmm_conv_desc* d = &descs[i];
+    OneConv g;
+    if (!geometry(d, g)) return fail(DMM_ERR_INVALID, "unsupported conv descriptor");
+    const void* yf = yfwd ? yfwd[i] : nullptr;
+    const float *qi = q ? q[i] : nullptr, *ri = r ? r[i] : nullptr;
+    if ((qi != nullptr) != (ri != nullptr) || (qi != nullptr && yf == nullptr)) return fail(DMM_ERR_INVALID, "q, r and yfwd come together");
+    if (d->transposed || d->mode != 0 || d->stride != 1 || d->R * d->S <= 1 || !d->bn_relu || !d->use_mfma)
+      return fail(DMM_ERR_INVALID, "the transposed form serves unit-stride multi-tap convolutions behind BN+ReLU");
+    const int rc = thin_wgrad_setup(d, g, x[i], dy[i], scale[i], shift[i], yf, qi, ri, dw[i], scratch[i], st, v[i].a, v[i].dd, v[i].dp, v[i].rows);
+    if (rc) return rc;
+    Resolved res;
+    if (!wg3_resolve(v[i].a, d->dtype, res)) return fail(DMM_ERR_INVALID, "not a launch wg3.hip takes (16-bit storage, 128 -> 32 channels, 3x3)");
+  }
+  void* part = nullptr;
+  HIPCHK(hipMallocAsync(&part, (size_t)W3_MAX_SLOTS * W3_SLOT_FLOATS * sizeof(float), st));
+  for (One& o : v) { o.a.part = (float*)part; o.a.part_slots = W3_MAX_SLOTS; }
+  hipError_t e = hipSuccess;
+  int nl = 0;
+  if (grouped) {
+    Wg3Group G;
+    for (int i = 0; i < n && e == hipSuccess; ++i) {
+      if (wg3_group_add(G, v[i].a, descs[i].dtype)) continue;
+      if (G.n > 0) { e = wg3_group_launch(G, st); ++nl; }
+      if (e == hipSuccess && !wg3_group_add(G, v[i].a, descs[i].dtype)) e = hipErrorNotSupported;
+    }
+    if (e == hipSuccess && G.n > 0) { e = wg3_group_launch(G, st); ++nl; }
+    if (e == hipSuccess) note_impl(IMPL_WG3);
+  } else {
+    for (int i = 0; i < n && e == hipSuccess; ++i, ++nl) e = launch_wgrad(v[i].a, descs[i].dtype, true, st, IMPL_WG3);
+  }
+  hipFreeAsync(part, st);
+  HIPCHK(e);
+  for (int i = 0; i < n; ++i) {
+    const dmm_conv_desc* d = &descs[i];
+    HIPCHK(hipMemsetAsync(dw[i], 0, (size_t)d->Cin * d->Cout * d->R * d->S * sizeof(float), st));
+    HIPCHK(launch_unpack(v[i].dd, v[i].dp, 1, v[i].rows, d->dtype, 1.0f, st));
+  }
+  if (launches) *launches = nl;
+  return DMM_OK;
+}
+
+int dmm_bw1_reduce_grouped(int n, const float* const* part, float* const* dpack, const int* nct, const int* nsplit, const int* wc,
+                           int grouped, int* launches, void* stream) {
+  if (n < 1 || !part || !dpack || !nct || !nsplit || !wc) return fail(DMM_ERR_INVALID, "null argument");
+  hipStream_t st = (hipStream_t)stream;
+  Bw1RedGroup G;
+  int nl = 0;
+  for (int i = 0; i < n; ++i) {
+    if (!part[i] || !dpack[i] || nct[i] < 1 || nsplit[i] < 1 || wc[i] < 1 || wc[i] > nct[i] * 128 || wc[i] <= (nct[i] - 1) * 128)
+      return fail(DMM_ERR_INVALID, "a member needs slots, a packed gradient, nct, nsplit >= 1 and (nct - 1) * 128 < wc <= nct * 128");
+    Bw1RedMember m;
+    m.part = part[i]; m.dpack = dpack[i]; m.nct = nct[i]; m.nsplit = nsplit[i];
+    m.nfloats = ((wc[i] + 31) / 32) * 128 * 32;
+    if (!grouped) { HIPCHK(launch_bw1_reduce_member(m, st)); ++nl; continue; }
+    if (G.n >= B1_RED_GROUP_MAX) { HIPCHK(bw1_reduce_group_launch(G, st)); ++nl; }
+    G.m[G.n++] = m;
+  }
+  if (G.n > 0) { HIPCHK(bw1_reduce_group_launch(G, st)); ++nl; }
+  if (launches) *launches = nl;
+  return DMM_OK;
+}
+
+}
diff --git a/dmmfods_amd/csrc/plan.h b/dmmfods_amd/csrc/plan.h
--- a/dmmfods_amd/csrc/plan.h
+++ b/dmmfods_amd/csrc/plan.h
@@ -141,4 +141,5 @@
   bool dp_used = false;
   unsigned long long graph_clock = 0;
   long long graph_replays[2] = {0, 0};
+  long long batch_counts[4] = {0, 0, 0, 0};
 };
diff --git a/dmmfods_amd/csrc/pointwise.h b/dmmfods_amd/csrc/pointwise.h
--- a/dmmfods_amd/csrc/pointwise.h
+++ b/dmmfods_amd/csrc/pointwise.h
@@ -204,6 +204,20 @@
 bool bw1_eligible(const WgradArgs& w, const ConvArgs& d, int dtype, unsigned deny);
 hipError_t launch_bw1(const Bw1Args& g, int dtype, hipStream_t st);
 hipError_t launch_bw1_reduce(const Bw1Args& g, hipStream_t st);
+constexpr int B1_RED_GROUP_MAX = 32;
+struct Bw1RedMember { const float* part; float* dpack; int nct, nsplit, nfloats; };
+struct Bw1RedGroup { int n = 0; Bw1RedMember m[B1_RED_GROUP_MAX]; };
+bool bw1_reduce_group_add(Bw1RedGroup& G, const Bw1Args& g);
+hipError_t bw1_reduce_group_launch(Bw1RedGroup& G, hipStream_t st);
+hipError_t launch_bw1_reduce_member(const Bw1RedMember& m, hipStream_t st);
+constexpr int W3_GROUP_MAX = 32;
+struct Wg3Group {
+  int n = 0, dtype = 0, pq = 0, part_slots = 0;
+  long long tiles = 0;
+  alignas(16) unsigned char block[4096];
+};
+bool wg3_group_add(Wg3Group& G, const WgradArgs& a, int dtype);
+hipError_t wg3_group_launch(Wg3Group& G, hipStream_t st);
 hipError_t launch_igemm(const ConvArgs& a, int dtype, int epi, bool mfma, hipStream_t st, int impl = IMPL_AUTO, unsigned deny = 0);
 hipError_t launch_wgrad(WgradArgs a, int dtype, bool mfma, hipStream_t st, int impl = IMPL_AUTO, unsigned deny = 0);
 int igemm_pick(const ConvArgs& a, int dtype, int epi, bool mfma, unsigned deny);
diff --git a/dmmfods_amd/csrc/wg3.hip b/dmmfods_amd/csrc/wg3.hip
--- a/dmmfods_amd/csrc/wg3.hip
+++ b/dmmfods_amd/csrc/wg3.hip
@@ -1,6 +1,8 @@
 #include <algorithm>
 #include <cmath>
+#include <cstddef>
 #include <cstdlib>
+#include <cstring>
 
 #include "common.h"
 #include "dispatch.h"
@@ -26,6 +28,14 @@
   int tiles_y, tiles_x, ntiles, tiles_per_wg;
   float* part;
 };
+
+struct W3View {
+  const void *asrc, *ysrc, *ysrc2;
+  const float *ascale, *ashift, *yq, *yr;
+  float* dpack;
+  int ald, yld, yld2, Ho, Wo, tiles_y, tiles_x;
+};
+struct W3Taps { short t[12]; };
 
 template <typename T, int NA, int NY, int PQ, int MODE>
 __device__ __forceinline__ void w3_sync(typename TT<T>::vec (&ra)[NA], typename TT<T>::vec (&ry)[NY], typename TT<T>::vec (&ry2)[PQ == 2 ? NY : 1]) {
@@ -40,20 +50,16 @@
 }
 
 template <typename T, int PQ>
-__global__ __launch_bounds__(W3_NT, 1) void wg3_kernel(const Wg3Args g) {
+__device__ __forceinline__ void wg3_walk(const W3View& a, const W3Taps& taps, const int t_beg, const int t_end, float* slot) {
   static_assert(sizeof(T) == 2, "16-bit storage");
   typedef typename TT<T>::vec V;
   constexpr int SLOT = 8;
   constexpr int NL = 256;
   constexpr int NA = BM * (W3_CA / SLOT) / NL;
   constexpr int NY = (W3_HH * W3_HW * (W3_CY / SLOT) + NL - 1) / NL;
-  const WgradArgs& a = g.w;
-  const Seg& sy_ = a.seg[0];
-  const Seg& sa = a.dy;
 
   extern __shared__ __attribute__((aligned(16))) unsigned char smem[];
   const int tid = threadIdx.x, lane = tid & 63, wave = tid >> 6;
-  const int t_beg = blockIdx.x * g.tiles_per_wg, t_end = min(g.ntiles, t_beg + g.tiles_per_wg);
   if (t_beg >= t_end) return;
   const int nt = t_end - t_beg;
 
@@ -62,12 +68,12 @@
     const int ca = lt & 15, pa0 = lt >> 4;
     const int cy = lt & 3, hy0 = lt >> 2;
     SlotK<SLOT> ka, ky;
-    ka.k0 = load_fv<SLOT>(sa.scale + ca * SLOT); ka.k1 = load_fv<SLOT>(sa.shift + ca * SLOT); ka.k2 = 0.f; ka.k3 = 0.f;
+    ka.k0 = load_fv<SLOT>(a.ascale + ca * SLOT); ka.k1 = load_fv<SLOT>(a.ashift + ca * SLOT); ka.k2 = 0.f; ka.k3 = 0.f;
     ky.k0 = 0.f; ky.k1 = 0.f; ky.k2 = 0.f; ky.k3 = 0.f;
-    if (PQ == 2) { ky.k0 = load_fv<SLOT>(sy_.q + cy * SLOT); ky.k1 = load_fv<SLOT>(sy_.r + cy * SLOT); }
-    const T* asrc = (const T*)sa.src + ca * SLOT;
-    const T* ysrc = (const T*)sy_.src + cy * SLOT;
-    const T* ysrc2 = (const T*)sy_.src2 + cy * SLOT;
+    if (PQ == 2) { ky.k0 = load_fv<SLOT>(a.yq + cy * SLOT); ky.k1 = load_fv<SLOT>(a.yr + cy * SLOT); }
+    const T* asrc = (const T*)a.asrc + ca * SLOT;
+    const T* ysrc = (const T*)a.ysrc + cy * SLOT;
+    const T* ysrc2 = (const T*)a.ysrc2 + cy * SLOT;
     int hyy[NY], hxx[NY];
 #pragma unroll
     for (int i = 0; i < NY; ++i) {
@@ -78,32 +84,32 @@
       V ra[NA], ry[NY], ry2[PQ == 2 ? NY : 1];
       unsigned oka, oky;
     };
-    const int tiles_img = g.tiles_y * g.tiles_x;
+    const int tiles_img = a.tiles_y * a.tiles_x;
     int cb = t_beg / tiles_img, cty, ctx, cleft = nt;
-    { const int tr = t_beg - cb * tiles_img; cty = tr / g.tiles_x; ctx = tr - cty * g.tiles_x; }
+    { const int tr = t_beg - cb * tiles_img; cty = tr / a.tiles_x; ctx = tr - cty * a.tiles_x; }
     auto issue = [&](LSet& R) {
       const int y0 = cty * W3_TH, x0 = ctx * W3_TW;
       R.oka = 0; R.oky = 0;
       const int xa = x0 + pa0;
-      const size_t arow = (size_t)cb * sa.Hs;
+      const size_t arow = (size_t)cb * a.Ho;
 #pragma unroll
       for (int i = 0; i < NA; ++i) {
         const int y = y0 + i;
         if (y < a.Ho && xa < a.Wo) R.oka |= 1u << i;
-        const size_t pix = (arow + min(y, sa.Hs - 1)) * sa.Ws + min(xa, sa.Ws - 1);
-        if (!(WG3_DBG & 4)) gload16(R.ra[i], asrc + pix * sa.ld);
-      }
-      const size_t yrow = (size_t)cb * sy_.Hs;
+        const size_t pix = (arow + min(y, a.Ho - 1)) * a.Wo + min(xa, a.Wo - 1);
+        if (!(WG3_DBG & 4)) gload16(R.ra[i], asrc + pix * a.ald);
+      }
+      const size_t yrow = (size_t)cb * a.Ho;
 #pragma unroll
       for (int i = 0; i < NY; ++i) {
         const int y = y0 + hyy[i], x = x0 + hxx[i];
-        if (hy0 + 64 * i < W3_HH * W3_HW && (unsigned)y < (unsigned)sy_.Hs && (unsigned)x < (unsigned)sy_.Ws) R.oky |= 1u << i;
-        const size_t pix = (yrow + min(max(y, 0), sy_.Hs - 1)) * sy_.Ws + min(max(x, 0), sy_.Ws - 1);
-        if (!(WG3_DBG & 4)) gload16(R.ry[i], ysrc + pix * sy_.ld);
-        if constexpr (PQ == 2) { if (!(WG3_DBG & 4)) gload16(R.ry2[i], ysrc2 + pix * sy_.ld2); }
+        if (hy0 + 64 * i < W3_HH * W3_HW && (unsigned)y < (unsigned)a.Ho && (unsigned)x < (unsigned)a.Wo) R.oky |= 1u << i;
+        const size_t pix = (yrow + min(max(y, 0), a.Ho - 1)) * a.Wo + min(max(x, 0), a.Wo - 1);
+        if (!(WG3_DBG & 4)) gload16(R.ry[i], ysrc + pix * a.yld);
+        if constexpr (PQ == 2) { if (!(WG3_DBG & 4)) gload16(R.ry2[i], ysrc2 + pix * a.yld2); }
       }
       if (--cleft > 0) {
-        if (++ctx == g.tiles_x) { ctx = 0; if (++cty == g.tiles_y) { cty = 0; ++cb; } }
+        if (++ctx == a.tiles_x) { ctx = 0; if (++cty == a.tiles_y) { cty = 0; ++cb; } }
       }
     };
     auto store = [&](LSet& R, int set, bool wait = true) {
@@ -169,7 +175,7 @@
   int yoff[9];
 #pragma unroll
   for (int t = 0; t < 9; ++t) {
-    const int tw = sy_.taps[t];
+    const int tw = taps.t[t];
     const int dy = (int)(signed char)(tw & 0xff), dx = (int)(signed char)((tw >> 8) & 0xff);
     yoff[t] = ((1 + dy) * W3_HW + (arow + 1 + dx)) * 64 + ycol;
   }
@@ -193,14 +199,14 @@
   }
 
   const int r = lane & 31, h = lane >> 5;
-  if (g.part != nullptr) {
-    f32x4* slot = (f32x4*)(g.part + (size_t)blockIdx.x * W3_SLOT_FLOATS);
+  if (slot != nullptr) {
+    f32x4* s4 = (f32x4*)slot;
 #pragma unroll
     for (int t = 0; t < 9; ++t)
 #pragma unroll
       for (int j = 0; j < 4; ++j) {
         const f32x4 v = {acc[t][4 * j], acc[t][4 * j + 1], acc[t][4 * j + 2], acc[t][4 * j + 3]};
-        if (!(WG3_DBG & 1) || v[0] == 1.2345e33f) slot[((t * 4 + wave) * 4 + j) * 64 + lane] = v;
+        if (!(WG3_DBG & 1) || v[0] == 1.2345e33f) s4[((t * 4 + wave) * 4 + j) * 64 + lane] = v;
       }
   } else {
 #pragma unroll
@@ -208,13 +214,51 @@
 #pragma unroll
       for (int i = 0; i < 16; ++i) {
         const int c = 32 * wave + (i & 3) + 8 * (i >> 2) + 4 * h;
-        if (!(WG3_DBG & 1) || acc[t][i] == 1.2345e33f) atomic_add_f32(a.dpack + ((size_t)t * a.Npad + c) * 32 + r, acc[t][i]);
-      }
-  }
+        if (!(WG3_DBG & 1) || acc[t][i] == 1.2345e33f) atomic_add_f32(a.dpack + ((size_t)t * W3_CA + c) * 32 + r, acc[t][i]);
+      }
+  }
+}
+
+template <typename T, int PQ>
+__global__ __launch_bounds__(W3_NT, 1) void wg3_kernel(const Wg3Args g) {
+  const Seg& sy_ = g.w.seg[0];
+  const Seg& sa = g.w.dy;
+  const W3View a = {sa.src, sy_.src, sy_.src2, sa.scale, sa.shift, sy_.q, sy_.r, g.w.dpack, sa.ld, sy_.ld, sy_.ld2, g.w.Ho, g.w.Wo, g.tiles_y, g.tiles_x};
+  W3Taps taps;
+#pragma unroll
+  for (int t = 0; t < 9; ++t) taps.t[t] = sy_.taps[t];
+  const int t_beg = blockIdx.x * g.tiles_per_wg;
+  wg3_walk<T, PQ>(a, taps, t_beg, min(g.ntiles, t_beg + g.tiles_per_wg), g.part ? g.part + (size_t)blockIdx.x * W3_SLOT_FLOATS : nullptr);
+}
+
+struct Wg3Member {
+  W3View v;
+  int ntiles, tiles_per_wg;
+};
+struct Wg3GroupArgs {
+  float* part;
+  int n;
+  int wg0[W3_GROUP_MAX + 1];
+  W3Taps taps;
+  Wg3Member m[W3_GROUP_MAX];
+};
+static_assert(sizeof(Wg3GroupArgs) <= 3840, "the table is a kernel argument: 4 KB with the hidden arguments");
+static_assert(sizeof(Wg3Member) % 8 == 0 && offsetof(Wg3GroupArgs, m) % 8 == 0, "members are read with aligned scalar loads");
+
+template <typename T, int PQ>
+__global__ __launch_bounds__(W3_NT, 1) void wg3_group_kernel(const Wg3GroupArgs g) {
+  const int bid = blockIdx.x;
+  int mi = 0;
+#pragma unroll
+  for (int i = 1; i < W3_GROUP_MAX; ++i)
+    if (i < g.n && bid >= g.wg0[i]) mi = i;
+  const Wg3Member& M = g.m[mi];
+  const int t_beg = (bid - g.wg0[mi]) * M.tiles_per_wg;
+  wg3_walk<T, PQ>(M.v, g.taps, t_beg, min(M.ntiles, t_beg + M.tiles_per_wg), g.part + (size_t)bid * W3_SLOT_FLOATS);
 }
 
 constexpr int W3_RG = 8;
-__global__ __launch_bounds__(256) void wg3_reduce_kernel(const float* __restrict__ part, float* __restrict__ dpack, int nslots) {
+__device__ __forceinline__ void wg3_reduce_slots(const float* __restrict__ part, float* __restrict__ dpack, int nslots) {
   __shared__ f32x4 red[W3_RG][32];
   const int o = threadIdx.x & 31, sg = threadIdx.x >> 5;
   const int f = blockIdx.x * 32 + o;
@@ -240,6 +284,19 @@
 #pragma unroll
     for (int q = 0; q < 4; ++q) d[q * 32] += t4[q];
   }
+}
+__global__ __launch_bounds__(256) void wg3_reduce_kernel(const float* __restrict__ part, float* __restrict__ dpack, int nslots) {
+  wg3_reduce_slots(part, dpack, nslots);
+}
+struct Wg3ReduceGroupArgs {
+  const float* part;
+  int wg0[W3_GROUP_MAX + 1];
+  float* dpack[W3_GROUP_MAX];
+};
+__global__ __launch_bounds__(256) void wg3_group_reduce_kernel(const Wg3ReduceGroupArgs g) {
+  const int mi = blockIdx.y;
+  const int s0 = g.wg0[mi];
+  wg3_reduce_slots(g.part + (size_t)s0 * W3_SLOT_FLOATS, g.dpack[mi], g.wg0[mi + 1] - s0);
 }
 
 struct Wg3Launch {
@@ -273,14 +330,25 @@
   return true;
 }
 
+static int wg3_slot_wgs(int part_slots) {
+  static const int cus = device_cus();
+  static const int wgs_cap = lab_int("DMM_WG3_WGS", 0);
+  int nwg = std::min(std::min(cus, W3_MAX_SLOTS), part_slots);
+  if (wgs_cap > 0) nwg = std::min(nwg, wgs_cap);
+  return std::max(1, nwg);
+}
+static bool wg3_use_slots() {
+  static const bool use_slots = lab_int("DMM_WG3_SLOTS", 1) != 0;
+  return use_slots;
+}
+
 hipError_t wg3_launch(const Resolved& r, hipStream_t st) {
   const Wg3Launch& l = r.get<Wg3Launch>();
   Wg3Args g = l.g;
   const WgradArgs& a = g.w;
   static const int cus = device_cus();
-  static const bool use_slots = lab_int("DMM_WG3_SLOTS", 1) != 0;
   static const int wgs_cap = lab_int("DMM_WG3_WGS", 0);
-  g.part = (use_slots && a.part != nullptr) ? a.part : nullptr;
+  g.part = (wg3_use_slots() && a.part != nullptr) ? a.part : nullptr;
   int nwg = g.part ? std::min(cus, a.part_slots) : (int)std::lround(std::sqrt(12.0 * g.ntiles));
   if (wgs_cap > 0) nwg = std::min(nwg, wgs_cap);
   nwg = std::max(1, std::min(std::min(nwg, cus), g.ntiles));
@@ -294,4 +362,83 @@
   return e;
 }
 
-}
+struct Wg3GroupLaunch {
+  Wg3GroupArgs g;
+  LdsLauncher<Wg3GroupArgs> run;
+};
+static_assert(sizeof(Wg3GroupLaunch) <= sizeof(Wg3Group::block) && alignof(Wg3GroupLaunch) <= 16, "Wg3Group::block is too small");
+
+template <typename T> static LdsLauncher<Wg3GroupArgs> wg3_group_runner(bool pq) {
+  return pq ? launch_lds<wg3_group_kernel<T, 2>, Wg3GroupArgs> : launch_lds<wg3_group_kernel<T, 0>, Wg3GroupArgs>;
+}
+
+bool wg3_group_add(Wg3Group& G, const WgradArgs& a, int dtype) {
+  if (!wg3_use_slots() || a.part == nullptr || a.part_slots < 1 || a.M <= 0) return false;
+  Resolved r;
+  if (!wg3_resolve(a, dtype, r)) return false;
+  const Wg3Launch& l = r.get<Wg3Launch>();
+  const Seg& sy_ = a.seg[0];
+  const Seg& sa = a.dy;
+  Wg3GroupLaunch& L = *reinterpret_cast<Wg3GroupLaunch*>(G.block);
+  const int pq = sy_.q ? 2 : 0;
+  W3Taps taps;
+  memset(&taps, 0, sizeof(taps));
+  for (int t = 0; t < 9; ++t) taps.t[t] = sy_.taps[t];
+  if (G.n == 0) {
+    memset(&L, 0, sizeof(L));
+    L.g.part = a.part;
+    L.g.taps = taps;
+    L.run = dtype == DT_F16 ? wg3_group_runner<f16>(pq != 0) : wg3_group_runner<bf16>(pq != 0);
+    G.dtype = dtype; G.pq = pq; G.part_slots = a.part_slots; G.tiles = 0;
+  } else {
+    if (G.dtype != dtype || G.pq != pq || L.g.part != a.part || G.part_slots != a.part_slots || memcmp(&L.g.taps, &taps, sizeof(taps)) != 0) return false;
+    if (G.n >= W3_GROUP_MAX || G.n >= wg3_slot_wgs(G.part_slots)) return false;
+  }
+  Wg3Member& m = L.g.m[G.n++];
+  m.v = {sa.src, sy_.src, sy_.src2, sa.scale, sa.shift, sy_.q, sy_.r, a.dpack, sa.ld, sy_.ld, sy_.ld2, a.Ho, a.Wo, l.g.tiles_y, l.g.tiles_x};
+  m.ntiles = l.g.ntiles;
+  m.tiles_per_wg = 0;
+  G.tiles += l.g.ntiles;
+  return true;
+}
+
+hipError_t wg3_group_launch(Wg3Group& G, hipStream_t st) {
+  if (G.n <= 0) return hipSuccess;
+  Wg3GroupLaunch& L = *reinterpret_cast<Wg3GroupLaunch*>(G.block);
+  Wg3GroupArgs& g = L.g;
+  const int n = G.n, W = wg3_slot_wgs(G.part_slots);
+  int w[W3_GROUP_MAX], sum = 0;
+  for (int i = 0; i < n; ++i) {
+    w[i] = (int)std::max<long long>(1, std::min<long long>(g.m[i].ntiles, (long long)W * g.m[i].ntiles / G.tiles));
+    sum += w[i];
+  }
+  while (sum > W) {
+    int k = -1;
+    for (int i = 0; i < n; ++i)
+      if (w[i] > 1 && (k < 0 || (long long)g.m[i].ntiles * w[k] < (long long)g.m[k].ntiles * w[i])) k = i;
+    --w[k]; --sum;
+  }
+  for (int i = 0; i < n && sum < W; ++i)
+    if (w[i] < g.m[i].ntiles) { ++w[i]; ++sum; }
+  int wg = 0;
+  Wg3ReduceGroupArgs rg;
+  memset(&rg, 0, sizeof(rg));
+  rg.part = g.part;
+  for (int i = 0; i < n; ++i) {
+    Wg3Member& m = g.m[i];
+    m.tiles_per_wg = (m.ntiles + w[i] - 1) / w[i];
+    g.wg0[i] = wg; rg.wg0[i] = wg;
+    rg.dpack[i] = m.v.dpack;
+    wg += (m.ntiles + m.tiles_per_wg - 1) / m.tiles_per_wg;
+  }
+  for (int i = n; i <= W3_GROUP_MAX; ++i) { g.wg0[i] = wg; rg.wg0[i] = wg; }
+  g.n = n;
+  G.n = 0; G.tiles = 0;
+  if (wg > G.part_slots) return hipErrorInvalidValue;
+  hipError_t e = L.run(W3_LDS, wg, W3_NT, W3_LDS, st, g);
+  if (e != hipSuccess) return e;
+  hipLaunchKernelGGL(wg3_group_reduce_kernel, dim3(W3_SLOT_FLOATS / 4 / 32, n), dim3(256), 0, st, rg);
+  return hipGetLastError();
+}
+
+}
diff --git a/include/dmmfods_hip.h b/include/dmmfods_hip.h
--- a/include/dmmfods_hip.h
+++ b/include/dmmfods_hip.h
@@ -88,6 +88,7 @@
 int dmm_plan_loss_metrics(dmm_plan* plan, const float* logits, const float* target, double* metrics_out, void* stream);
 
 long long dmm_plan_num_graph_replays(const dmm_plan* plan, int which);
+int dmm_plan_wgrad_batch_counts(const dmm_plan* plan, long long counts[4]);
 
 int dmm_adam_step(float* params, const float* grads, float* exp_avg, float* exp_avg_sq, int64_t n, float lr, float beta1,
                   float beta2, float eps, float weight_decay, int64_t step, float grad_scale, void* stream);
@@ -167,6 +168,12 @@
                                const float* shift, const void* yfwd, const float* q, const float* r, void* gx, int accumulate,
                                float* dw, double* red, void* scratch, void* stream);
 
+int dmm_conv_wgrad_grouped(const dmm_conv_desc* descs, int n, const void* const* x, const void* const* dy, const float* const* scale,
+                           const float* const* shift, const void* const* yfwd, const float* const* q, const float* const* r,
+                           float* const* dw, void* const* scratch, int grouped, int* launches, void* stream);
+int dmm_bw1_reduce_grouped(int n, const float* const* part, float* const* dpack, const int* nct, const int* nsplit, const int* wc,
+                           int grouped, int* launches, void* stream);
+
 int dmm_last_impl(void);
 const char* dmm_impl_name(int impl);
 unsigned dmm_impl_mask(int reset);
```

New measurement: 162.0 img/s (median of 6 runs). 1.1% higher.
